# pratyushkumar211/industrial_nnmpc_2021

Hardware: AMD Instinct MI355X
Metric: condensed-QP solves/sec (CDU offline datagen) (higher is better)
Workload: dtype f64; 1 GPU; cdu_offline_data: synthetic CDU-size plant (n=4480 vars, m=8960 box rows, n_aug=284), 100000 sampled x0 per GPU per step, whole sequences u* written out; batch_per_gpu=100000, total_batch=100000, method=auto, parallelism=dp1 (sharded samples, 1 RCCL gather of the first moves pe...

## Files before the change

include/nnmpc.h:

```cpp
#ifndef NNMPC_H
#define NNMPC_H
#include <stdint.h>
#ifdef __cplusplus
extern "C" {
#endif

#define NNMPC_OK 0
#define NNMPC_EINVAL (-1)
#define NNMPC_EHIP (-2)
#define NNMPC_ENOMEM (-3)
#define NNMPC_ENOTIMPL (-4)

#define NNMPC_HOST 0
#define NNMPC_DEVICE 1

#define NNMPC_ST_OPTIMAL 0
#define NNMPC_ST_MAXITER 1
#define NNMPC_ST_NUMERIC 2

typedef struct nnmpc_qp nnmpc_qp;
typedef struct nnmpc_nn nnmpc_nn;

typedef struct {
  int32_t max_batch;
  int32_t nb;
  int32_t max_ipm_iters;
  int32_t max_polish_rounds;
  int32_t max_refine;
  int32_t max_rounds;
  int32_t sub_steps;
  int32_t stale_max_changes;
  int32_t stale_cg_limit;
  int32_t method;
  int32_t asm_max_active;
  int32_t asm_max_rounds;
  int32_t asm_f32_rounds;
  int32_t seg_max;
  int32_t asm_tail_batch;
  int32_t asm_predict_iters;
  float ipm_tol;
  double refine_tol;
  double bound_tol;
} nnmpc_qp_opts;

typedef struct {
  int64_t problems;
  int64_t rounds;
  int64_t factorizations;
  int64_t ipm_iterations;
  int64_t panel_launches;
  double panel_ms;
  double diag_ms;
  double trsv_ms;
  double total_ms;
  double panel_flops;
  int64_t trsv_solves;
  int64_t asm_solved;
  int64_t asm_rounds;
  int64_t asm_gemm_launches;
  double asm_gemm_ms;
  double asm_gemm_flops;
  double asm_lambda_ms;
  double asm_update_ms;
  double asm_lambda_flops;
  double asm_lambda_bytes;
  double asm_e1max;
  double asm_e2max;
  int64_t asm_full_checks;
  double asm_lambda32_ms;
  double asm_lambda64_ms;
  double asm_lambda32_flops;
  int64_t asm_lambda32_launches, asm_lambda64_launches;
  int64_t asm_far_passes;
  double asm_side_ms;
  int64_t asm_small_passes;
  int64_t asm_predict_launches;
  double asm_predict_ms;
  double asm_predict_flops;
} nnmpc_qp_stats;

const char* nnmpc_last_error(void);

int nnmpc_qp_create(nnmpc_qp** out, int32_t n, int32_t nu, int32_t n_aug, const double* P,
                    const double* tq, const double* Kunc, const nnmpc_qp_opts* opts);
int nnmpc_qp_destroy(nnmpc_qp* h);

int nnmpc_qp_solve_batch(nnmpc_qp* h, int32_t B, const double* x0, const double* lb,
                         const double* ub, double* u, uint32_t* active, int32_t* status,
                         int32_t* iters, int32_t ptr_kind);

int nnmpc_qp_solve_batch_warm(nnmpc_qp* h, int32_t B, const double* x0, const double* lb,
                              const double* ub, const uint8_t* guess, double* u, uint32_t* active,
                              int32_t* status, int32_t* iters, int32_t ptr_kind);

#define NNMPC_OUT_SEQUENCE 0
#define NNMPC_OUT_FIRST_MOVE 1
int nnmpc_qp_solve_batch_ex(nnmpc_qp* h, int32_t B, const double* x0, const double* lb,
                            const double* ub, const uint8_t* guess, double* u, uint32_t* active,
                            int32_t* status, int32_t* iters, int32_t ptr_kind, int32_t out_kind);

int nnmpc_qp_set_inverse(nnmpc_qp* h, const double* Hinv, const double* Kunc);

int nnmpc_qp_set_farfield(nnmpc_qp* h, int32_t W, int32_t r, const double* U, const double* Vx, const double* Vl);
int nnmpc_qp_farfield_missing(nnmpc_qp* h, int32_t* W);

int nnmpc_qp_first_moves(const double* u, int64_t ldu, const double* us, int32_t B, int32_t nu, double* out);
int nnmpc_qp_dims(nnmpc_qp* h, int32_t* n, int32_t* nu, int32_t* n_aug);
int nnmpc_qp_set_profiling(nnmpc_qp* h, int32_t on);
int nnmpc_qp_get_stats(nnmpc_qp* h, nnmpc_qp_stats* out, int32_t reset);

int nnmpc_qp_debug_factor_solve(nnmpc_qp* h, int32_t B, const float* dvec, const float* mask,
                                const float* rhs, float* sol);

int nnmpc_nn_create(nnmpc_nn** out, int32_t nlayers, const int32_t* dims,
                    const double* const* W, const double* const* b, int32_t nx, int32_t nu,
                    int32_t with_uprev, const double* xscale, const double* ulb,
                    const double* uub, int32_t use_bf16, int32_t max_batch);
int nnmpc_nn_destroy(nnmpc_nn* h);
int nnmpc_nn_forward(nnmpc_nn* h, int32_t B, const double* x, const double* uprev,
                     const double* xs, const double* us, double* u, int32_t ptr_kind);
int nnmpc_nn_last_ms(nnmpc_nn* h, double* gemm_ms, double* total_ms);
int nnmpc_nn_last_hidden_ms(nnmpc_nn* h, double* hidden_ms, int32_t* launches);

typedef struct nnmpc_chain nnmpc_chain;
int nnmpc_chain_create(nnmpc_chain** out, nnmpc_qp* qp, int32_t nc, int32_t nx, int32_t nu, int32_t nd,
                       const double* A, const double* B, const double* Bd, const double* ulb,
                       const double* uub, const double* x0, const double* uprev0);
int nnmpc_chain_destroy(nnmpc_chain* c);
int nnmpc_chain_run(nnmpc_chain* c, int32_t T, const double* xs, const double* us, const double* d,
                    double* x_rec, double* uprev_rec, double* u_rec, int32_t* status,
                    int32_t warm_start, int32_t ptr_kind);
int nnmpc_chain_reset(nnmpc_chain* c);
int nnmpc_chain_last_ms(nnmpc_chain* c, double* total_ms, double* solve_ms);

typedef struct nnmpc_ts nnmpc_ts;
int nnmpc_ts_create(nnmpc_ts** out, int32_t nu, int32_t nz, const double* Pr, const double* E,
                    const double* lb, const double* ub);
int nnmpc_ts_destroy(nnmpc_ts* h);
int nnmpc_ts_solve_batch(nnmpc_ts* h, int32_t B, const double* q, const double* e, double* us,
                         double* lam_eq, uint8_t* active, int32_t* status, int32_t ptr_kind);

typedef struct nnmpc_cl nnmpc_cl;
#define NNMPC_CL_MPC 0
#define NNMPC_CL_NN 1
#define NNMPC_CL_SATDLQR 2
#define NNMPC_CL_US 3
typedef struct {
  int32_t nx, nu, ny, nd, nz;
  const double *A, *B, *C, *Bp;
  const double *Aaug, *Baug, *Caug, *L;
  const double *tb, *Qb, *Qy, *q0, *Cd, *Eb, *Xb, *Xu;
  const double *Qaug, *Raug, *Maug;
  const double *ulb, *uub, *x0, *xhat0, *uprev0;
} nnmpc_cl_model;
typedef struct {
  int32_t kind;
  nnmpc_qp* qp;
  int32_t nlayers;
  const int32_t* dims;
  const double* const* W;
  const double* const* b;
  int32_t with_uprev;
  const double* xscale;
  const double* Kaug;
} nnmpc_cl_slot;
int nnmpc_cl_create(nnmpc_cl** out, const nnmpc_cl_model* m, nnmpc_ts* ts, int32_t nslots, const nnmpc_cl_slot* slots,
                    int32_t nb, const int32_t* inst_slot);
int nnmpc_cl_destroy(nnmpc_cl* h);
int nnmpc_cl_run(nnmpc_cl* h, int32_t T, int32_t nscen, const double* setpoints, const double* dist, const int32_t* scen,
                 const double* v, const double* sigma, const double* y0, double* y_rec, double* x_rec, double* xhat_rec, double* u_rec,
                 double* xs_rec, double* us_rec, double* avg_rec, int32_t* ts_status, int32_t* reg_status, int32_t ptr_kind);
int nnmpc_cl_reset(nnmpc_cl* h);
int nnmpc_cl_last_ms(nnmpc_cl* h, double* total_ms, double* phase_ms, double* slot_step_ms);
#define NNMPC_CL_PLANT_LINEAR 0
#define NNMPC_CL_PLANT_CSTRS_FLASH 1
#define NNMPC_CSTRS_NPAR 51
int nnmpc_cl_set_plant(nnmpc_cl* h, int32_t kind, const double* par, int32_t npar, double sample_time, int32_t substeps);
int nnmpc_cl_last_plant_ms(nnmpc_cl* h, double* plant_ms);
int nnmpc_cstrs_flow(int32_t nb, const double* par, int32_t npar, double sample_time, int32_t substeps, const double* x,
                     const double* u, const double* p, double* x_out, int32_t ptr_kind);

int nnmpc_device_count(void);
int nnmpc_set_device(int32_t dev);
int nnmpc_device_synchronize(void);
int nnmpc_dev_mem_info(uint64_t* free_bytes, uint64_t* total_bytes);
int nnmpc_dev_malloc(void** out, uint64_t bytes);
int nnmpc_dev_free(void* p);
int nnmpc_dev_memset(void* p, int32_t value, uint64_t bytes);
int nnmpc_memcpy_h2d(void* dst, const void* src, uint64_t bytes);
int nnmpc_memcpy_d2h(void* dst, const void* src, uint64_t bytes);
int nnmpc_memcpy_d2d(void* dst, const void* src, uint64_t bytes);
int nnmpc_host_alloc_pinned(void** out, uint64_t bytes);
int nnmpc_host_free_pinned(void* p);

typedef struct nnmpc_comm nnmpc_comm;
int nnmpc_comm_unique_id(void* id128);
int nnmpc_comm_init(nnmpc_comm** out, const void* id128, int32_t rank, int32_t world);
int nnmpc_comm_destroy(nnmpc_comm* c);
int nnmpc_comm_rank(nnmpc_comm* c);
int nnmpc_comm_world(nnmpc_comm* c);
int nnmpc_comm_gather_rows(nnmpc_comm* c, const double* send, const int64_t* rows, int32_t row_doubles,
                           double* recv, int32_t root);
int nnmpc_comm_allreduce_max(nnmpc_comm* c, double* value);
int nnmpc_comm_barrier(nnmpc_comm* c);

#ifdef __cplusplus
}
#endif
#endif
```

industrial_nnmpc_2021_amd/_lib.py:

```python
import ctypes as C
import os

_HERE = os.path.dirname(os.path.abspath(__file__))
LIB_PATH = os.path.join(_HERE, "libnnmpc_hip.so")

HOST, DEVICE = 0, 1
ST_OPTIMAL, ST_MAXITER, ST_NUMERIC = 0, 1, 2
OUT_SEQUENCE, OUT_FIRST_MOVE = 0, 1
EINVAL, EHIP, ENOMEM, ENOTIMPL = -1, -2, -3, -4


class QpOpts(C.Structure):
    _fields_ = [("max_batch", C.c_int32), ("nb", C.c_int32), ("max_ipm_iters", C.c_int32),
                ("max_polish_rounds", C.c_int32), ("max_refine", C.c_int32),
                ("max_rounds", C.c_int32), ("sub_steps", C.c_int32), ("stale_max_changes", C.c_int32),
                ("stale_cg_limit", C.c_int32), ("method", C.c_int32), ("asm_max_active", C.c_int32),
                ("asm_max_rounds", C.c_int32), ("asm_f32_rounds", C.c_int32), ("seg_max", C.c_int32), ("asm_tail_batch", C.c_int32), ("asm_predict_iters", C.c_int32), ("ipm_tol", C.c_float), ("refine_tol", C.c_double),
                ("bound_tol", C.c_double)]


class QpStats(C.Structure):
    _fields_ = [("problems", C.c_int64), ("rounds", C.c_int64), ("factorizations", C.c_int64),
                ("ipm_iterations", C.c_int64), ("panel_launches", C.c_int64),
                ("panel_ms", C.c_double), ("diag_ms", C.c_double), ("trsv_ms", C.c_double),
                ("total_ms", C.c_double), ("panel_flops", C.c_double), ("trsv_solves", C.c_int64), ("asm_solved", C.c_int64),
                ("asm_rounds", C.c_int64), ("asm_gemm_launches", C.c_int64), ("asm_gemm_ms", C.c_double),
                ("asm_gemm_flops", C.c_double), ("asm_lambda_ms", C.c_double), ("asm_update_ms", C.c_double), ("asm_lambda_flops", C.c_double),
                ("asm_lambda_bytes", C.c_double), ("asm_e1max", C.c_double),
                ("asm_e2max", C.c_double), ("asm_full_checks", C.c_int64), ("asm_lambda32_ms", C.c_double),
                ("asm_lambda64_ms", C.c_double), ("asm_lambda32_flops", C.c_double),
                ("asm_lambda32_launches", C.c_int64), ("asm_lambda64_launches", C.c_int64), ("asm_far_passes", C.c_int64), ("asm_side_ms", C.c_double),
                ("asm_small_passes", C.c_int64), ("asm_predict_launches", C.c_int64), ("asm_predict_ms", C.c_double),
                ("asm_predict_flops", C.c_double)]


CL_MPC, CL_NN, CL_SATDLQR, CL_US = 0, 1, 2, 3
CL_PLANT_LINEAR, CL_PLANT_CSTRS_FLASH, CSTRS_NPAR = 0, 1, 51


class ClModel(C.Structure):
    _fields_ = [(k, C.c_int32) for k in ("nx", "nu", "ny", "nd", "nz")] + \
               [(k, C.c_void_p) for k in ("A", "B", "C", "Bp", "Aaug", "Baug", "Caug", "L", "tb", "Qb", "Qy", "q0", "Cd",
                                          "Eb", "Xb", "Xu", "Qaug", "Raug", "Maug", "ulb", "uub", "x0", "xhat0", "uprev0")]


class ClSlot(C.Structure):
    _fields_ = [("kind", C.c_int32), ("qp", C.c_void_p), ("nlayers", C.c_int32), ("dims", C.c_void_p), ("W", C.c_void_p),
                ("b", C.c_void_p), ("with_uprev", C.c_int32), ("xscale", C.c_void_p), ("Kaug", C.c_void_p)]


EXPORTS = ["nnmpc_last_error", "nnmpc_qp_create", "nnmpc_qp_destroy", "nnmpc_qp_solve_batch",
           "nnmpc_qp_solve_batch_warm", "nnmpc_qp_solve_batch_ex", "nnmpc_qp_set_inverse", "nnmpc_qp_dims",
           "nnmpc_qp_first_moves", "nnmpc_qp_set_farfield", "nnmpc_qp_farfield_missing",
           "nnmpc_qp_set_profiling", "nnmpc_qp_get_stats", "nnmpc_qp_debug_factor_solve",
           "nnmpc_nn_create", "nnmpc_nn_destroy", "nnmpc_nn_forward", "nnmpc_nn_last_ms", "nnmpc_nn_last_hidden_ms",
           "nnmpc_chain_create", "nnmpc_chain_destroy", "nnmpc_chain_run", "nnmpc_chain_reset", "nnmpc_chain_last_ms",
           "nnmpc_ts_create", "nnmpc_ts_destroy", "nnmpc_ts_solve_batch",
           "nnmpc_cl_create", "nnmpc_cl_destroy", "nnmpc_cl_run", "nnmpc_cl_reset", "nnmpc_cl_last_ms",
           "nnmpc_cl_set_plant", "nnmpc_cl_last_plant_ms", "nnmpc_cstrs_flow",
           "nnmpc_device_count", "nnmpc_set_device", "nnmpc_device_synchronize", "nnmpc_dev_mem_info",
           "nnmpc_dev_malloc", "nnmpc_dev_free", "nnmpc_dev_memset", "nnmpc_memcpy_h2d", "nnmpc_memcpy_d2h",
           "nnmpc_memcpy_d2d", "nnmpc_host_alloc_pinned", "nnmpc_host_free_pinned",
           "nnmpc_comm_unique_id", "nnmpc_comm_init", "nnmpc_comm_destroy", "nnmpc_comm_rank", "nnmpc_comm_world",
           "nnmpc_comm_gather_rows", "nnmpc_comm_allreduce_max", "nnmpc_comm_barrier"]

_lib = None


class NnmpcError(RuntimeError):
    pass


def load():
    global _lib
    if _lib is not None:
        return _lib
    if not os.path.exists(LIB_PATH):
        raise NnmpcError(
            f"{LIB_PATH} not found: build it with `python -c 'import __graft_entry__ as g; g.build()'` "
            "(hipcc --offload-arch=gfx950).  There is no CPU fallback.")
    lib = C.CDLL(LIB_PATH)
    vp, i32, dp = C.c_void_p, C.c_int32, C.c_void_p
    lib.nnmpc_last_error.restype = C.c_char_p
    lib.nnmpc_last_error.argtypes = []
    lib.nnmpc_qp_create.restype = i32
    lib.nnmpc_qp_create.argtypes = [C.POINTER(vp), i32, i32, i32, dp, dp, dp, C.POINTER(QpOpts)]
    lib.nnmpc_qp_destroy.restype = i32
    lib.nnmpc_qp_destroy.argtypes = [vp]
    lib.nnmpc_qp_solve_batch.restype = i32
    lib.nnmpc_qp_solve_batch.argtypes = [vp, i32, dp, dp, dp, dp, dp, dp, dp, i32]
    lib.nnmpc_qp_solve_batch_warm.restype = i32
    lib.nnmpc_qp_solve_batch_warm.argtypes = [vp, i32, dp, dp, dp, dp, dp, dp, dp, dp, i32]
    lib.nnmpc_qp_set_inverse.restype = i32
    lib.nnmpc_qp_set_inverse.argtypes = [vp, dp, dp]
    lib.nnmpc_qp_set_farfield.restype = i32
    lib.nnmpc_qp_set_farfield.argtypes = [vp, i32, i32, dp, dp, dp]
    lib.nnmpc_qp_farfield_missing.restype = i32
    lib.nnmpc_qp_farfield_missing.argtypes = [vp, C.POINTER(i32)]
    lib.nnmpc_qp_set_profiling.restype = i32
    lib.nnmpc_qp_set_profiling.argtypes = [vp, i32]
    lib.nnmpc_qp_get_stats.restype = i32
    lib.nnmpc_qp_get_stats.argtypes = [vp, C.POINTER(QpStats), i32]
    lib.nnmpc_qp_debug_factor_solve.restype = i32
    lib.nnmpc_qp_debug_factor_solve.argtypes = [vp, i32, dp, dp, dp, dp]
    lib.nnmpc_nn_create.restype = i32
    lib.nnmpc_nn_create.argtypes = [C.POINTER(vp), i32, C.POINTER(i32), C.POINTER(dp), C.POINTER(dp),
                                    i32, i32, i32, dp, dp, dp, i32, i32]
    lib.nnmpc_nn_destroy.restype = i32
    lib.nnmpc_nn_destroy.argtypes = [vp]
    lib.nnmpc_nn_forward.restype = i32
    lib.nnmpc_nn_forward.argtypes = [vp, i32, dp, dp, dp, dp, dp, i32]
    lib.nnmpc_nn_last_ms.restype = i32
    lib.nnmpc_nn_last_ms.argtypes = [vp, C.POINTER(C.c_double), C.POINTER(C.c_double)]
    lib.nnmpc_nn_last_hidden_ms.restype = i32
    lib.nnmpc_nn_last_hidden_ms.argtypes = [vp, C.POINTER(C.c_double), C.POINTER(C.c_int32)]
    u64 = C.c_uint64
    lib.nnmpc_qp_solve_batch_ex.restype = i32
    lib.nnmpc_qp_solve_batch_ex.argtypes = [vp, i32, dp, dp, dp, dp, dp, dp, dp, dp, i32, i32]
    lib.nnmpc_qp_first_moves.restype = i32
    lib.nnmpc_qp_first_moves.argtypes = [dp, C.c_int64, dp, i32, i32, dp]
    lib.nnmpc_qp_dims.restype = i32
    lib.nnmpc_qp_dims.argtypes = [vp, C.POINTER(i32), C.POINTER(i32), C.POINTER(i32)]
    lib.nnmpc_chain_create.restype = i32
    lib.nnmpc_chain_create.argtypes = [C.POINTER(vp), vp, i32, i32, i32, i32, dp, dp, dp, dp, dp, dp, dp]
    lib.nnmpc_chain_destroy.restype = i32
    lib.nnmpc_chain_destroy.argtypes = [vp]
    lib.nnmpc_chain_run.restype = i32
    lib.nnmpc_chain_run.argtypes = [vp, i32, dp, dp, dp, dp, dp, dp, dp, i32, i32]
    lib.nnmpc_chain_reset.restype = i32
    lib.nnmpc_chain_reset.argtypes = [vp]
    lib.nnmpc_chain_last_ms.restype = i32
    lib.nnmpc_chain_last_ms.argtypes = [vp, C.POINTER(C.c_double), C.POINTER(C.c_double)]
    lib.nnmpc_ts_create.restype = i32
    lib.nnmpc_ts_create.argtypes = [C.POINTER(vp), i32, i32, dp, dp, dp, dp]
    lib.nnmpc_ts_destroy.restype = i32
    lib.nnmpc_ts_destroy.argtypes = [vp]
    lib.nnmpc_ts_solve_batch.restype = i32
    lib.nnmpc_ts_solve_batch.argtypes = [vp, i32, dp, dp, dp, dp, dp, dp, i32]
    lib.nnmpc_cl_create.restype = i32
    lib.nnmpc_cl_create.argtypes = [C.POINTER(vp), C.POINTER(ClModel), vp, i32, C.POINTER(ClSlot), i32, C.POINTER(i32)]
    lib.nnmpc_cl_destroy.restype = i32
    lib.nnmpc_cl_destroy.argtypes = [vp]
    lib.nnmpc_cl_run.restype = i32
    lib.nnmpc_cl_run.argtypes = [vp, i32, i32, dp, dp, dp, dp, dp, dp] + [dp] * 9 + [i32]
    lib.nnmpc_cl_reset.restype = i32
    lib.nnmpc_cl_reset.argtypes = [vp]
    lib.nnmpc_cl_last_ms.restype = i32
    lib.nnmpc_cl_last_ms.argtypes = [vp, C.POINTER(C.c_double), dp, dp]
    lib.nnmpc_cl_set_plant.restype = i32
    lib.nnmpc_cl_set_plant.argtypes = [vp, i32, dp, i32, C.c_double, i32]
    lib.nnmpc_cl_last_plant_ms.restype = i32
    lib.nnmpc_cl_last_plant_ms.argtypes = [vp, C.POINTER(C.c_double)]
    lib.nnmpc_cstrs_flow.restype = i32
    lib.nnmpc_cstrs_flow.argtypes = [i32, dp, i32, C.c_double, i32, dp, dp, dp, dp, i32]
    lib.nnmpc_device_count.restype = i32
    lib.nnmpc_device_count.argtypes = []
    lib.nnmpc_set_device.restype = i32
    lib.nnmpc_set_device.argtypes = [i32]
    lib.nnmpc_device_synchronize.restype = i32
    lib.nnmpc_device_synchronize.argtypes = []
    lib.nnmpc_dev_mem_info.restype = i32
    lib.nnmpc_dev_mem_info.argtypes = [C.POINTER(u64), C.POINTER(u64)]
    lib.nnmpc_dev_malloc.restype = i32
    lib.nnmpc_dev_malloc.argtypes = [C.POINTER(vp), u64]
    lib.nnmpc_dev_free.restype = i32
    lib.nnmpc_dev_free.argtypes = [vp]
    lib.nnmpc_dev_memset.restype = i32
    lib.nnmpc_dev_memset.argtypes = [vp, i32, u64]
    for name in ("nnmpc_memcpy_h2d", "nnmpc_memcpy_d2h", "nnmpc_memcpy_d2d"):
        getattr(lib, name).restype = i32
        getattr(lib, name).argtypes = [vp, vp, u64]
    lib.nnmpc_host_alloc_pinned.restype = i32
    lib.nnmpc_host_alloc_pinned.argtypes = [C.POINTER(vp), u64]
    lib.nnmpc_host_free_pinned.restype = i32
    lib.nnmpc_host_free_pinned.argtypes = [vp]
    lib.nnmpc_comm_unique_id.restype = i32
    lib.nnmpc_comm_unique_id.argtypes = [vp]
    lib.nnmpc_comm_init.restype = i32
    lib.nnmpc_comm_init.argtypes = [C.POINTER(vp), vp, i32, i32]
    lib.nnmpc_comm_destroy.restype = i32
    lib.nnmpc_comm_destroy.argtypes = [vp]
    lib.nnmpc_comm_rank.restype = i32
    lib.nnmpc_comm_rank.argtypes = [vp]
    lib.nnmpc_comm_world.restype = i32
    lib.nnmpc_comm_world.argtypes = [vp]
    lib.nnmpc_comm_gather_rows.restype = i32
    lib.nnmpc_comm_gather_rows.argtypes = [vp, dp, C.POINTER(C.c_int64), i32, dp, i32]
    lib.nnmpc_comm_allreduce_max.restype = i32
    lib.nnmpc_comm_allreduce_max.argtypes = [vp, C.POINTER(C.c_double)]
    lib.nnmpc_comm_barrier.restype = i32
    lib.nnmpc_comm_barrier.argtypes = [vp]
    _lib = lib
    return lib


def check(rc, what):
    if rc != 0:
        msg = load().nnmpc_last_error().decode(errors="replace")
        raise NnmpcError(f"{what} failed (code {rc}): {msg}")


class DeviceArray:

    def __init__(self, shape, dtype):
        import numpy as np
        self.shape = tuple(int(v) for v in (shape if hasattr(shape, "__len__") else (shape,)))
        self.dtype = np.dtype(dtype)
        self.nbytes = int(np.prod(self.shape, dtype=np.int64)) * self.dtype.itemsize
        self._p = C.c_void_p()
        check(load().nnmpc_dev_malloc(C.byref(self._p), self.nbytes), "nnmpc_dev_malloc")

    @classmethod
    def from_host(cls, a):
        import numpy as np
        a = np.ascontiguousarray(a)
        d = cls(a.shape, a.dtype)
        d.upload(a)
        return d

    def data_ptr(self):
        return self._p.value or 0

    def upload(self, a):
        import numpy as np
        a = np.ascontiguousarray(a, dtype=self.dtype)
        if a.nbytes != self.nbytes:
            raise ValueError("upload: size mismatch")
        check(load().nnmpc_memcpy_h2d(self._p, a.ctypes.data_as(C.c_void_p), self.nbytes), "nnmpc_memcpy_h2d")

    def to_host(self, rows=None):
        import numpy as np
        shape = self.shape if rows is None else (int(rows),) + self.shape[1:]
        out = np.empty(shape, self.dtype)
        check(load().nnmpc_memcpy_d2h(out.ctypes.data_as(C.c_void_p), self._p, out.nbytes), "nnmpc_memcpy_d2h")
        return out

    def row_ptr(self, row):
        import numpy as np
        stride = int(np.prod(self.shape[1:], dtype=np.int64)) * self.dtype.itemsize
        return C.c_void_p((self._p.value or 0) + int(row) * stride)

    def free(self):
        if getattr(self, "_p", None) is not None and self._p.value:
            load().nnmpc_dev_free(self._p)
            self._p = C.c_void_p()

    __del__ = free


def set_device(dev):
    check(load().nnmpc_set_device(int(dev)), "nnmpc_set_device")


def synchronize():
    check(load().nnmpc_device_synchronize(), "nnmpc_device_synchronize")


def device_count():
    return int(load().nnmpc_device_count())
```

industrial_nnmpc_2021_amd/csrc/qp_solver.hip:

```cpp
#include <hip/hip_runtime.h>
#include <stdint.h>
#include <stdio.h>
#include <stdarg.h>
#include <string.h>
#include <vector>
#include <algorithm>
#include <cmath>
#include <cstdlib>
#include "../../include/nnmpc.h"
#define ASM_WG_TU (-1)
#include "chol_kernels.h"
#include "gemm_kernels.h"
#include "qp_asm.h"
#include "qp_wide.h"
#include "qp_small.h"
#include "qp_predict.h"
#include "common.h"
static constexpr int ASM_SMALL9_LDS_MAX = 100 * 1024;

using namespace nnmpc;

namespace {

enum { PH_INIT = 0, PH_IPM = 1, PH_POLISH = 2, PH_DONE = 3 };
enum { PS_START = 0, PS_CG = 1, PS_CHECK = 2 };
enum { CNT_ACTIVE = 0, CNT_FACTOR = 1, CNT_IPM = 2, CNT_POLISH = 3, CNT_SOLVE = 4 };

constexpr int POLISH_GRACE = 10;
struct QpDev {
  int n, np, nu, slots;
  int max_ipm, max_polish, max_refine, stale_max_changes, stale_cg_limit;
  float ipm_tol, delta;
  double refine_tol, bound_tol, stat_tol, pscale;
  const float* pdiag;
  float *u, *zu, *zl, *lbv, *ubv, *q, *PU, *rd, *rhs, *sol, *dua, *dvec, *mask, *uunc;
  double *x, *q64, *PX, *r64, *p64, *v64;
  unsigned char* st;
  double *lb64, *ub64;
  const double *q64_all, *lb_all, *ub_all;
  const float* uunc_all;
  const unsigned char* guess_all;
  int *slot_prob, *age, *next_prob;
  int seg_count, max_rounds;
  int *phase, *f_factor, *f_solve, *istep, *ipm_it, *nfac, *prounds, *rcnt, *psub, *fail, *stale;
  int *pninf, *pgrace;
  int* ptie;
  float *mu, *gap, *smu, *qscale;
  double* rz;
  int* counters;
  double* u_out;
  int ldu, nout;
  uint32_t* act_out;
  int* status_out;
  int* iters_out;
  int words;
};

__device__ __forceinline__ float wave_max(float v) {
  for (int o = 32; o > 0; o >>= 1) v = fmaxf(v, __shfl_xor(v, o));
  return v;
}
__device__ __forceinline__ float wave_sum(float v) {
  for (int o = 32; o > 0; o >>= 1) v += __shfl_xor(v, o);
  return v;
}
__device__ __forceinline__ double wave_maxd(double v) {
  for (int o = 32; o > 0; o >>= 1) v = fmax(v, __shfl_xor(v, o));
  return v;
}
__device__ float block_max(float v, float* sh) {
  v = wave_max(v);
  __syncthreads();
  if ((threadIdx.x & 63) == 0) sh[threadIdx.x >> 6] = v;
  __syncthreads();
  return fmaxf(fmaxf(sh[0], sh[1]), fmaxf(sh[2], sh[3]));
}
__device__ float block_sum(float v, float* sh) {
  v = wave_sum(v);
  __syncthreads();
  if ((threadIdx.x & 63) == 0) sh[threadIdx.x >> 6] = v;
  __syncthreads();
  return (sh[0] + sh[1]) + (sh[2] + sh[3]);
}
__device__ double block_maxd(double v, double* sh) {
  v = wave_maxd(v);
  __syncthreads();
  if ((threadIdx.x & 63) == 0) sh[threadIdx.x >> 6] = v;
  __syncthreads();
  return fmax(fmax(sh[0], sh[1]), fmax(sh[2], sh[3]));
}
__device__ double block_sumd(double v, double* sh) {
  for (int o = 32; o > 0; o >>= 1) v += __shfl_xor(v, o);
  __syncthreads();
  if ((threadIdx.x & 63) == 0) sh[threadIdx.x >> 6] = v;
  __syncthreads();
  return (sh[0] + sh[1]) + (sh[2] + sh[3]);
}
__device__ int block_sum_i(int v, int* sh) {
  for (int o = 32; o > 0; o >>= 1) v += __shfl_xor(v, o);
  __syncthreads();
  if ((threadIdx.x & 63) == 0) sh[threadIdx.x >> 6] = v;
  __syncthreads();
  return sh[0] + sh[1] + sh[2] + sh[3];
}

#define SLACK_MIN 1e-12f

__device__ void write_outputs(const QpDev& d, int p, int status);

__global__ __launch_bounds__(256) void refill_k(QpDev d) {
  __shared__ float shf[4];
  __shared__ int s_idx;
  const int p = blockIdx.x, tid = threadIdx.x;
  const size_t o = (size_t)p * d.np;
  if (d.phase[p] != PH_DONE) return;
  if (tid == 0) s_idx = atomicAdd(d.next_prob, 1);
  __syncthreads();
  const int idx = s_idx;
  if (idx >= d.seg_count) {
    if (tid == 0) d.slot_prob[p] = -1;
    return;
  }
  const size_t oi = (size_t)idx * d.np;
  if (tid < d.nu) {
    d.lb64[(size_t)p * d.nu + tid] = d.lb_all[(size_t)idx * d.nu + tid];
    d.ub64[(size_t)p * d.nu + tid] = d.ub_all[(size_t)idx * d.nu + tid];
  }
  float qm = 0.f;
  int invalid = 0;
  for (int r = tid; r < d.np; r += 256) {
    if (r < d.n) {
      const int c = r % d.nu;
      invalid |= !(fabs(d.q64_all[oi + r]) <= 1.79e308);
      const float lb = (float)d.lb_all[(size_t)idx * d.nu + c], ub = (float)d.ub_all[(size_t)idx * d.nu + c];
      const double q64 = d.q64_all[oi + r];
      const float q = (float)(q64 / d.pscale);
      const float w = ub - lb;
      float u0 = d.uunc_all[oi + r];
      u0 = fminf(fmaxf(u0, lb + 0.05f * w), ub - 0.05f * w);
      d.lbv[o + r] = lb; d.ubv[o + r] = ub; d.q[o + r] = q; d.u[o + r] = u0; d.q64[o + r] = q64;
      qm = fmaxf(qm, fabsf(q));
    } else {
      d.lbv[o + r] = -1.f; d.ubv[o + r] = 1.f; d.q[o + r] = 0.f; d.u[o + r] = 0.f; d.q64[o + r] = 0.0;
    }
    d.zu[o + r] = 0.f; d.zl[o + r] = 0.f;
    d.mask[o + r] = 1.f; d.dvec[o + r] = 0.f; d.rhs[o + r] = 0.f; d.sol[o + r] = 0.f;
    d.dua[o + r] = 0.f; d.rd[o + r] = 0.f; d.x[o + r] = 0.0; d.st[o + r] = 0;
    d.r64[o + r] = 0.0; d.p64[o + r] = 0.0; d.v64[o + r] = 0.0;
  }
  qm = block_max(qm, shf);
  {
    invalid |= !(qm <= 3.0e38f);
    if (tid < d.nu) invalid |= !(d.lb_all[(size_t)idx * d.nu + tid] <= d.ub_all[(size_t)idx * d.nu + tid]);
    invalid = __syncthreads_or(invalid);
    if (invalid) {
      const double qnan = __longlong_as_double(0x7ff8000000000000ll);
      for (int r = tid; r < d.np; r += 256) d.x[o + r] = qnan;
      if (tid == 0) { d.slot_prob[p] = idx; d.fail[p] = 1; d.ipm_it[p] = d.nfac[p] = 0; }
      __syncthreads();
      write_outputs(d, p, NNMPC_ST_NUMERIC);
      return;
    }
  }
  const bool warm = d.guess_all != nullptr && d.guess_all[(size_t)idx * d.n] != 255;
  if (warm) {
    for (int r = tid; r < d.n; r += 256) {
      const int c = r % d.nu;
      int s = d.guess_all[(size_t)idx * d.n + r];
      if (s > 2) s = 0;
      const double xv = s == 1 ? d.ub_all[(size_t)idx * d.nu + c]
                      : s == 2 ? d.lb_all[(size_t)idx * d.nu + c] : (double)d.u[o + r];
      d.st[o + r] = (unsigned char)s;
      d.x[o + r] = xv;
      d.v64[o + r] = xv;
    }
  }
  if (tid == 0) {
    d.slot_prob[p] = idx;
    d.age[p] = 0;
    d.qscale[p] = fmaxf(1.f, qm);
    d.phase[p] = warm ? PH_POLISH : PH_INIT;
    d.f_factor[p] = d.f_solve[p] = 0;
    d.ipm_it[p] = d.nfac[p] = d.prounds[p] = d.rcnt[p] = d.psub[p] = d.fail[p] = d.stale[p] = 0;
    d.pninf[p] = 0x7fffffff; d.pgrace[p] = POLISH_GRACE; d.ptie[p] = 0;
    d.mu[p] = d.gap[p] = d.smu[p] = 0.f; d.rz[p] = 0.0;
  }
}
__global__ void reset_slots_k(QpDev d) {
  const int p = blockIdx.x * blockDim.x + threadIdx.x;
  if (p < d.slots) {
    d.phase[p] = PH_DONE; d.slot_prob[p] = -1; d.age[p] = 0;
    d.f_factor[p] = d.f_solve[p] = 0;
  }
  if (p == 0) *d.next_prob = 0;
}

__device__ void write_outputs(const QpDev& d, int p, int status) {
  const int tid = threadIdx.x;
  const size_t o = (size_t)p * d.np;
  const size_t pi = (size_t)d.slot_prob[p];
  for (int r = tid; r < d.nout; r += 256) d.u_out[pi * d.ldu + r] = d.x[o + r];
  const int m = 2 * d.n;
  for (int w = tid; w < d.words; w += 256) {
    uint32_t bits = 0;
    for (int b = 0; b < 32; ++b) {
      const int idx = 32 * w + b;
      if (idx < m) {
        const int k = idx / (2 * d.nu), c = idx % (2 * d.nu);
        const int hit = (c < d.nu) ? (d.st[o + k * d.nu + c] == 1) : (d.st[o + k * d.nu + c - d.nu] == 2);
        bits |= (uint32_t)hit << b;
      }
    }
    if (d.act_out) d.act_out[pi * d.words + w] = bits;
  }
  if (tid == 0) {
    if (d.status_out) d.status_out[pi] = d.fail[p] ? NNMPC_ST_NUMERIC : status;
    if (d.iters_out) { d.iters_out[2 * pi] = d.ipm_it[p]; d.iters_out[2 * pi + 1] = d.nfac[p]; }
  }
}

__device__ int cg_alpha(const QpDev& d, int p, double* shd) {
  const int tid = threadIdx.x;
  const size_t o = (size_t)p * d.np;
  double pap = 0.0;
  for (int r = tid; r < d.n; r += 256)
    if (d.st[o + r] == 0) pap += d.p64[o + r] * d.PX[o + r];
  pap = block_sumd(pap, shd);
  const double rz = d.rz[p];
  const bool ok = (pap > 0.0) && (rz > 0.0);
  const double a = ok ? rz / pap : 0.0;
  double pm = 0.0, xm = 0.0;
  for (int r = tid; r < d.n; r += 256) {
    if (d.st[o + r] == 0) {
      const double pv = d.p64[o + r];
      const double x = d.x[o + r] + a * pv;
      d.x[o + r] = x;
      d.r64[o + r] -= a * d.PX[o + r];
      pm = fmax(pm, fabs(pv));
      xm = fmax(xm, fabs(x));
    } else {
      xm = fmax(xm, fabs(d.x[o + r]));
    }
  }
  pm = block_maxd(pm, shd);
  xm = block_maxd(xm, shd);
  const int rc = d.rcnt[p] + 1;
  const bool nan = !(a == a) || !(xm == xm);
  const bool conv = !ok || nan || (fabs(a) * pm <= d.refine_tol * fmax(1.0, xm)) || rc >= d.max_refine;
  if (conv) {
    for (int r = tid; r < d.n; r += 256) d.v64[o + r] = d.x[o + r];
  } else {
    for (int r = tid; r < d.n; r += 256) d.rhs[o + r] = d.st[o + r] ? 0.f : (float)d.r64[o + r];
  }
  const bool refac = !conv && d.stale[p] && rc >= d.stale_cg_limit;
  if (refac) for (int r = tid; r < d.n; r += 256) d.v64[o + r] = d.x[o + r];
  __syncthreads();
  if (tid == 0) {
    d.rcnt[p] = refac ? 0 : rc;
    if (nan) d.fail[p] = 1;
    if (conv) d.psub[p] = PS_CHECK;
    if (refac) { d.psub[p] = PS_START; d.stale[p] = 0; }
  }
  return (conv || refac) ? 0 : 1;
}
__device__ void cg_beta(const QpDev& d, int p, double* shd) {
  const int tid = threadIdx.x;
  const size_t o = (size_t)p * d.np;
  double rzn = 0.0;
  for (int r = tid; r < d.n; r += 256)
    if (d.st[o + r] == 0) rzn += d.r64[o + r] * (double)d.sol[o + r];
  rzn = block_sumd(rzn, shd);
  const bool first = d.psub[p] == PS_START;
  const double rz = d.rz[p];
  const double beta = (first || !(rz > 0.0)) ? 0.0 : rzn / rz;
  for (int r = tid; r < d.n; r += 256) {
    double pv = 0.0;
    if (d.st[o + r] == 0) pv = (double)d.sol[o + r] + beta * d.p64[o + r];
    d.p64[o + r] = pv;
    d.v64[o + r] = pv;
  }
  __syncthreads();
  if (tid == 0) { d.rz[p] = rzn; d.psub[p] = PS_CG; }
}

__device__ int kkt_check(const QpDev& d, int p, int* shi, double* shd) {
  const int tid = threadIdx.x, n = d.n;
  const size_t o = (size_t)p * d.np;
  int bad = 0;
  double gfree = 0.0;
  for (int r = tid; r < n; r += 256) {
    const int c = r % d.nu;
    const double g = d.PX[o + r] + d.q64[o + r], x = d.x[o + r];
    const double lb = d.lb64[(size_t)p * d.nu + c], ub = d.ub64[(size_t)p * d.nu + c];
    const int s = d.st[o + r];
    if (s == 0) { bad += !(x <= ub + d.bound_tol) || !(x >= lb - d.bound_tol) || !(fabs(g) <= 1.79e308); gfree = fmax(gfree, fabs(g)); }
    else if (s == 1) bad += !(g < 0.0);
    else bad += !(g > 0.0);
  }
  bad = block_sum_i(bad, shi);
  gfree = block_maxd(gfree, shd);
  const int pr = d.prounds[p] + 1;
  if (bad == 0 && pr <= d.max_polish && !d.ptie[p]) {
    int ties = 0;
    for (int r = tid; r < n; r += 256) {
      if (d.st[o + r] != 0) continue;
      const int c = r % d.nu;
      const double x = d.x[o + r];
      const double lb = d.lb64[(size_t)p * d.nu + c], ub = d.ub64[(size_t)p * d.nu + c];
      if (x > ub) { d.st[o + r] = 1; d.x[o + r] = ub; ++ties; }
      else if (x < lb) { d.st[o + r] = 2; d.x[o + r] = lb; ++ties; }
    }
    ties = block_sum_i(ties, shi);
    __syncthreads();
    if (tid == 0) d.ptie[p] = 1;
    if (ties > 0) {
      for (int r = tid; r < n; r += 256) d.v64[o + r] = d.x[o + r];
      if (tid == 0) {
        d.stale[p] = ties <= d.stale_max_changes;
        d.prounds[p] = pr; d.psub[p] = PS_START; d.rcnt[p] = 0;
        d.f_factor[p] = d.f_solve[p] = 0;
      }
      return 0;
    }
  }
  if (bad == 0 || pr > d.max_polish) {
    const double gs = d.pscale * (double)d.qscale[p];
    const int ok = bad == 0 && gfree <= d.stat_tol * gs;
    write_outputs(d, p, ok ? NNMPC_ST_OPTIMAL : NNMPC_ST_MAXITER);
    if (tid == 0) { d.phase[p] = PH_DONE; d.f_factor[p] = d.f_solve[p] = 0; }
    return 1;
  }
  int single = 0, rsel = -1;
  {
    const int best = d.pninf[p], grace = d.pgrace[p];
    __syncthreads();
    if (bad < best) { if (tid == 0) { d.pninf[p] = bad; d.pgrace[p] = POLISH_GRACE; } }
    else if (grace > 0) { if (tid == 0) d.pgrace[p] = grace - 1; }
    else single = 1;
  }
  if (single) {
    double rm = -1e300;
    for (int r = tid; r < n; r += 256) {
      const int c = r % d.nu;
      const double g = d.PX[o + r] + d.q64[o + r], x = d.x[o + r];
      const double lb = d.lb64[(size_t)p * d.nu + c], ub = d.ub64[(size_t)p * d.nu + c];
      const int s = d.st[o + r];
      const bool inf = s == 0 ? ((x > ub + d.bound_tol) || (x < lb - d.bound_tol)) : (s == 1 ? g >= 0.0 : g <= 0.0);
      if (inf && -(double)r > rm) rm = -(double)r;
    }
    rm = block_maxd(rm, shd);
    rsel = rm > -1e299 ? (int)(-rm) : -1;
  }
  for (int r = tid; r < n; r += 256) {
    const int c = r % d.nu;
    const double g = d.PX[o + r] + d.q64[o + r], x = d.x[o + r];
    const double lb = d.lb64[(size_t)p * d.nu + c], ub = d.ub64[(size_t)p * d.nu + c];
    const int s = d.st[o + r];
    double xn = x;
    if (single && r != rsel) { d.v64[o + r] = xn; continue; }
    if (s == 0) {
      if (x > ub + d.bound_tol) { d.st[o + r] = 1; xn = ub; }
      else if (x < lb - d.bound_tol) { d.st[o + r] = 2; xn = lb; }
    } else if ((s == 1 && g >= 0.0) || (s == 2 && g <= 0.0)) {
      d.st[o + r] = 0;
    }
    d.x[o + r] = xn;
    d.v64[o + r] = xn;
  }
  if (tid == 0) {
    d.stale[p] = bad <= d.stale_max_changes;
    d.prounds[p] = pr; d.psub[p] = PS_START; d.rcnt[p] = 0;
    d.f_factor[p] = d.f_solve[p] = 0;
  }
  return 0;
}

__global__ __launch_bounds__(256) void stage_pre_k(QpDev d) {
  __shared__ float shf[4];
  __shared__ int shi[4];
  __shared__ double shd[4];
  const int p = blockIdx.x, tid = threadIdx.x;
  const size_t o = (size_t)p * d.np;
  int ph = d.phase[p];
  if (ph == PH_DONE) return;
  const int n = d.n;
  {
    const int age = d.age[p] + 1;
    __syncthreads();
    if (tid == 0) d.age[p] = age;
    if (age > d.max_rounds) {
      if (ph != PH_POLISH) {
        for (int r = tid; r < n; r += 256) { d.x[o + r] = (double)d.u[o + r]; d.st[o + r] = 0; }
        __syncthreads();
      }
      write_outputs(d, p, NNMPC_ST_MAXITER);
      if (tid == 0) { d.phase[p] = PH_DONE; d.f_factor[p] = d.f_solve[p] = 0; }
      return;
    }
  }

  if (ph == PH_INIT) {
    float s = 0.f;
    for (int r = tid; r < n; r += 256) s += fabsf(d.PU[o + r] + d.q[o + r]);
    s = block_sum(s, shf);
    const float mu0 = 0.1f * s / n + 1e-3f;
    for (int r = tid; r < n; r += 256) {
      const float g = d.PU[o + r] + d.q[o + r];
      const float u = d.u[o + r];
      const float su = fmaxf(d.ubv[o + r] - u, SLACK_MIN), sl = fmaxf(u - d.lbv[o + r], SLACK_MIN);
      d.zu[o + r] = fmaxf(-g, 0.f) + mu0 / su;
      d.zl[o + r] = fmaxf(g, 0.f) + mu0 / sl;
    }
    ph = PH_IPM;
  }

  if (ph == PH_IPM) {
    float rdm = 0.f, gs = 0.f;
    for (int r = tid; r < n; r += 256) {
      const float g = d.PU[o + r] + d.q[o + r];
      const float u = d.u[o + r], zu = d.zu[o + r], zl = d.zl[o + r];
      const float su = fmaxf(d.ubv[o + r] - u, SLACK_MIN), sl = fmaxf(u - d.lbv[o + r], SLACK_MIN);
      const float rdv = g + zu - zl;
      d.rd[o + r] = rdv;
      rdm = fmaxf(rdm, fabsf(rdv));
      gs += su * zu + sl * zl;
    }
    rdm = block_max(rdm, shf);
    gs = block_sum(gs, shf);
    const float mu = gs / (2.f * n);
    const int it = d.ipm_it[p];
    const bool nan = !(rdm == rdm) || !(gs == gs);
    const bool conv = (rdm <= d.ipm_tol * d.qscale[p] && mu <= d.ipm_tol * d.qscale[p]) || it >= d.max_ipm || nan;
    if (!conv) {
      for (int r = tid; r < n; r += 256) {
        const float u = d.u[o + r], zu = d.zu[o + r], zl = d.zl[o + r];
        const float su = fmaxf(d.ubv[o + r] - u, SLACK_MIN), sl = fmaxf(u - d.lbv[o + r], SLACK_MIN);
        d.dvec[o + r] = zu / su + zl / sl + d.delta;
        d.mask[o + r] = 1.f;
        d.rhs[o + r] = -(d.PU[o + r] + d.q[o + r]);
      }
      if (tid == 0) {
        d.phase[p] = PH_IPM;
        d.gap[p] = gs; d.mu[p] = mu;
        d.ipm_it[p] = it + 1; d.nfac[p] += 1;
        d.f_factor[p] = 1; d.f_solve[p] = 1; d.istep[p] = 0;
        atomicAdd(&d.counters[CNT_ACTIVE], 1); atomicAdd(&d.counters[CNT_FACTOR], 1);
        atomicAdd(&d.counters[CNT_IPM], 1); atomicAdd(&d.counters[CNT_SOLVE], 1);
      }
      return;
    }
    for (int r = tid; r < n; r += 256) {
      const float u = d.u[o + r], zu = d.zu[o + r], zl = d.zl[o + r];
      const float su = fmaxf(d.ubv[o + r] - u, SLACK_MIN), sl = fmaxf(u - d.lbv[o + r], SLACK_MIN);
      const int c = r % d.nu;
      int s = 0;
      if (!nan) {
        const float pd = d.pdiag[r];
        const bool au = zu > pd * su, al = zl > pd * sl;
        if (au && al) s = (zu * sl > zl * su) ? 1 : 2; else if (au) s = 1; else if (al) s = 2;
      }
      d.st[o + r] = (unsigned char)s;
      const double xv = s == 1 ? d.ub64[(size_t)p * d.nu + c]
                      : s == 2 ? d.lb64[(size_t)p * d.nu + c]
                               : (nan ? 0.0 : (double)u);
      d.x[o + r] = xv;
      d.v64[o + r] = xv;
    }
    if (tid == 0) {
      if (nan) d.fail[p] = 1;
      d.phase[p] = PH_POLISH; d.psub[p] = PS_START; d.rcnt[p] = 0; d.prounds[p] = 0;
      d.f_factor[p] = d.f_solve[p] = 0;
      atomicAdd(&d.counters[CNT_ACTIVE], 1); atomicAdd(&d.counters[CNT_POLISH], 1);
    }
    return;
  }

  int sub = d.psub[p];
  if (sub == PS_CHECK) {
    if (kkt_check(d, p, shi, shd)) return;
    if (tid == 0) { atomicAdd(&d.counters[CNT_ACTIVE], 1); atomicAdd(&d.counters[CNT_POLISH], 1); }
    return;
  }
  if (sub == PS_START) {
    const int keep = d.stale[p];
    for (int r = tid; r < n; r += 256) {
      const int s = d.st[o + r];
      const double rr = s ? 0.0 : -(d.PX[o + r] + d.q64[o + r]);
      d.r64[o + r] = rr;
      d.rhs[o + r] = (float)rr;
      if (!keep) { d.mask[o + r] = s ? 0.f : 1.f; d.dvec[o + r] = s ? 1.f : d.delta; }
    }
    if (tid == 0) {
      d.f_factor[p] = !keep; d.f_solve[p] = 1;
      if (!keep) { d.nfac[p] += 1; atomicAdd(&d.counters[CNT_FACTOR], 1); }
      atomicAdd(&d.counters[CNT_ACTIVE], 1); atomicAdd(&d.counters[CNT_POLISH], 1);
      atomicAdd(&d.counters[CNT_SOLVE], 1);
    }
    return;
  }
  if (tid == 0) {
    d.f_factor[p] = 0; d.f_solve[p] = 1;
    atomicAdd(&d.counters[CNT_ACTIVE], 1); atomicAdd(&d.counters[CNT_POLISH], 1);
    atomicAdd(&d.counters[CNT_SOLVE], 1);
  }
}

__global__ __launch_bounds__(256) void stage_sub_a_k(QpDev d) {
  __shared__ float shf[4];
  __shared__ double shd[4];
  const int p = blockIdx.x, tid = threadIdx.x;
  const size_t o = (size_t)p * d.np;
  if (!d.f_solve[p]) return;
  const int ph = d.phase[p], n = d.n;
  if (ph == PH_POLISH) { cg_beta(d, p, shd); return; }
  if (ph != PH_IPM) return;
  if (d.istep[p] == 0) {
  float t = 0.f;
  for (int r = tid; r < n; r += 256) {
    const float du = d.sol[o + r], u = d.u[o + r], zu = d.zu[o + r], zl = d.zl[o + r];
    const float su = fmaxf(d.ubv[o + r] - u, SLACK_MIN), sl = fmaxf(u - d.lbv[o + r], SLACK_MIN);
    const float dzu = -zu + zu * du / su, dzl = -zl - zl * du / sl;
    t = fmaxf(t, fmaxf(fmaxf(du / su, -du / sl), fmaxf(-dzu / zu, -dzl / zl)));
  }
  t = block_max(t, shf);
  const float a = t > 0.f ? fminf(1.f, 1.f / t) : 1.f;
  float ga = 0.f;
  for (int r = tid; r < n; r += 256) {
    const float du = d.sol[o + r], u = d.u[o + r], zu = d.zu[o + r], zl = d.zl[o + r];
    const float su = fmaxf(d.ubv[o + r] - u, SLACK_MIN), sl = fmaxf(u - d.lbv[o + r], SLACK_MIN);
    const float dzu = -zu + zu * du / su, dzl = -zl - zl * du / sl;
    ga += (su - a * du) * (zu + a * dzu) + (sl + a * du) * (zl + a * dzl);
  }
  ga = block_sum(ga, shf);
  float sg = ga / d.gap[p];
  sg = fminf(1.f, fmaxf(0.f, sg));
  const float smu = sg * sg * sg * d.mu[p];
  for (int r = tid; r < n; r += 256) {
    const float du = d.sol[o + r], u = d.u[o + r], zu = d.zu[o + r], zl = d.zl[o + r];
    const float su = fmaxf(d.ubv[o + r] - u, SLACK_MIN), sl = fmaxf(u - d.lbv[o + r], SLACK_MIN);
    const float dzu = -zu + zu * du / su, dzl = -zl - zl * du / sl;
    d.rhs[o + r] = -d.rd[o + r] + zu - smu / su - du * dzu / su - zl + smu / sl - du * dzl / sl;
    d.dua[o + r] = du;
  }
  if (tid == 0) { d.smu[p] = smu; d.istep[p] = 1; }
    return;
  }
  const float smu = d.smu[p];
  float t = 0.f;
  for (int r = tid; r < n; r += 256) {
    const float du = d.sol[o + r], da = d.dua[o + r], u = d.u[o + r], zu = d.zu[o + r], zl = d.zl[o + r];
    const float su = fmaxf(d.ubv[o + r] - u, SLACK_MIN), sl = fmaxf(u - d.lbv[o + r], SLACK_MIN);
    const float dzua = -zu + zu * da / su, dzla = -zl - zl * da / sl;
    const float rcu = -su * zu + smu + da * dzua, rcl = -sl * zl + smu - da * dzla;
    const float dzu = (rcu + zu * du) / su, dzl = (rcl - zl * du) / sl;
    t = fmaxf(t, fmaxf(fmaxf(du / su, -du / sl), fmaxf(-dzu / zu, -dzl / zl)));
  }
  t = block_max(t, shf);
  const float a = t > 0.f ? fminf(1.f, 0.99f / t) : 1.f;
  for (int r = tid; r < n; r += 256) {
    const float du = d.sol[o + r], da = d.dua[o + r], u = d.u[o + r], zu = d.zu[o + r], zl = d.zl[o + r];
    const float su = fmaxf(d.ubv[o + r] - u, SLACK_MIN), sl = fmaxf(u - d.lbv[o + r], SLACK_MIN);
    const float dzua = -zu + zu * da / su, dzla = -zl - zl * da / sl;
    const float rcu = -su * zu + smu + da * dzua, rcl = -sl * zl + smu - da * dzla;
    const float dzu = (rcu + zu * du) / su, dzl = (rcl - zl * du) / sl;
    d.u[o + r] = u + a * du;
    d.zu[o + r] = fmaxf(zu + a * dzu, 1e-30f);
    d.zl[o + r] = fmaxf(zl + a * dzl, 1e-30f);
  }
  if (tid == 0) d.f_solve[p] = 0;
}

__global__ __launch_bounds__(256) void stage_sub_b_k(QpDev d) {
  __shared__ int shi[4];
  __shared__ double shd[4];
  const int p = blockIdx.x, tid = threadIdx.x;
  if (d.phase[p] != PH_POLISH) return;
  const int sub = d.psub[p];
  if (sub == PS_CG && d.f_solve[p]) {
    const int go = cg_alpha(d, p, shd);
    if (tid == 0) d.f_solve[p] = go;
  } else if (sub == PS_CHECK) {
    kkt_check(d, p, shi, shd);
  }
}

__global__ void f64_to_f32_k(float* dst, const double* src, size_t count) {
  size_t i = (size_t)blockIdx.x * blockDim.x + threadIdx.x;
  const size_t stride = (size_t)gridDim.x * blockDim.x;
  for (; i < count; i += stride) dst[i] = (float)src[i];
}
__global__ void pad_x0_k(double* d64, float* d32, const double* src, int nprob, int n_aug, int ka,
                         int rows) {
  size_t i = (size_t)blockIdx.x * blockDim.x + threadIdx.x;
  const size_t total = (size_t)rows * ka;
  const size_t stride = (size_t)gridDim.x * blockDim.x;
  for (; i < total; i += stride) {
    const int p = (int)(i / ka), k = (int)(i % ka);
    const double v = (p < nprob && k < n_aug) ? src[(size_t)p * n_aug + k] : 0.0;
    d64[i] = v;
    d32[i] = (float)v;
  }
}

}

struct nnmpc_qp {
  int device;
  int n, np, nu, n_aug, ka, NB, T, tiles, slots, words;
  nnmpc_qp_opts opts;
  bool have_kunc;
  float* Pt;
  float* P32;
  double* P64;
  double* tq64;
  float* Kunc32;
  float* pdiag;
  double pscale;
  float* L;
  float* Y;
  float* Dacc;
  unsigned long long* trsv_count;
  QpDev d;
  bool have_inverse;
  double* H64;
  double* Kunc64;
  double *asm_xunc, *asm_x, *asm_lam, *asm_xh, *asm_scratch, *asm_xhw;
  int *asm_rowprob, *asm_wflag;
  unsigned char* asm_wmark;
  unsigned char* asm_st;
  int *asm_state, *asm_rounds, *asm_counters, *asm_biglist, *asm_status, *asm_binlist, *asm_idxg, *asm_mg, *asm_row, *asm_lrank, *asm_ctot;
  unsigned char *asm_prec, *asm_redo, *asm_alpha, *asm_rowk;
  float *asm_lam32, *asm_xh32, *H32;
  int *asm_ninf, *asm_hi, *asm_kblk;
  double tqmax;
  int asm_pool;
  double asm_e1max, asm_e2max;
  struct Far { int W, r, rp; double *U, *Vx, *Vl, *cu; int* kt; double ksum; double efar; };
  std::vector<Far> far;
  std::vector<int> far_missing;
  double p_inf = 0.0;
  double *asm_tnorm = nullptr, *asm_tslack = nullptr;
  struct PredWin { pu32x4* Hf = nullptr; double L = 0.0; int W = 0; };
  PredWin pred[2];
  int* pred_cnt = nullptr;
  double* asm_work;
  int seg_max;
  double* x0_64;
  float* x0_32;
  double* q64_all;
  float* uunc_all;
  double *lb_d, *ub_d;
  double* in_stage;
  hipStream_t stream;
  hipStream_t stream2 = nullptr;
  hipStream_t stream3 = nullptr, stream4 = nullptr;
  int asm_tail_budget = 50000;
  hipEvent_t ev_fork = nullptr, ev_join = nullptr, ev_join3 = nullptr, ev_join4 = nullptr;
  int* pin_cnt = nullptr;
  int* pin_st = nullptr;
  bool profiling;
  bool gemm_error = false;
  std::vector<hipEvent_t> ev_pool;
  size_t ev_used;
  struct EvRec { int kind; size_t e0, e1; double flops; };
  std::vector<EvRec> ev_recs;
  nnmpc_qp_stats stats;
  std::vector<void*> allocs;
  struct Scratch { void* p = nullptr; size_t cap = 0; };
  enum { SC_U = 0, SC_ACT, SC_ST, SC_IT, SC_GUESS, SC_FB_GUESS, SC_FB_LIST, SC_FB_X0, SC_FB_LB, SC_FB_UB, SC_FB_U, SC_FB_ACT, SC_FB_ST, SC_FB_IT, SC_COUNT };
  Scratch sc[SC_COUNT];
  int ldu, nout;
};

namespace {

template <class T>
int dev_alloc(nnmpc_qp* h, T** p, size_t count) {
  void* q = nullptr;
  hipError_t e = hipMalloc(&q, count * sizeof(T));
  if (e != hipSuccess) { set_error("hipMalloc(%zu bytes): %s", count * sizeof(T), hipGetErrorString(e)); return NNMPC_ENOMEM; }
  e = hipMemset(q, 0, count * sizeof(T));
  if (e != hipSuccess) { set_error("hipMemset: %s", hipGetErrorString(e)); return NNMPC_EHIP; }
  h->allocs.push_back(q);
  *p = (T*)q;
  return 0;
}

template <class T>
int scratch_get(nnmpc_qp* h, int which, T** out, size_t bytes) {
  nnmpc_qp::Scratch& s = h->sc[which];
  if (s.cap < bytes) {
    if (s.p) { hipFree(s.p); s.p = nullptr; s.cap = 0; }
    const size_t want = bytes + bytes / 4 + 256;
    const hipError_t e = hipMalloc(&s.p, want);
    if (e != hipSuccess) { s.p = nullptr; set_error("hipMalloc(%zu bytes of scratch): %s", want, hipGetErrorString(e)); return NNMPC_ENOMEM; }
    s.cap = want;
  }
  *out = (T*)s.p;
  return 0;
}

size_t ev_get(nnmpc_qp* h) {
  if (h->ev_used == h->ev_pool.size()) {
    hipEvent_t e;
    hipEventCreate(&e);
    h->ev_pool.push_back(e);
  }
  return h->ev_used++;
}
struct EvScope {
  nnmpc_qp* h; int kind; double flops; size_t e0; hipStream_t st;
  EvScope(nnmpc_qp* h_, int kind_, double flops_, hipStream_t st_ = nullptr) : h(h_), kind(kind_), flops(flops_), e0(0), st(st_ ? st_ : h_->stream) {
    if (h->profiling) { e0 = ev_get(h); hipEventRecord(h->ev_pool[e0], st); }
  }
  ~EvScope() {
    if (h->profiling) {
      size_t e1 = ev_get(h);
      hipEventRecord(h->ev_pool[e1], st);
      h->ev_recs.push_back({kind, e0, e1, flops});
    }
  }
};
void ev_collect(nnmpc_qp* h) {
  for (auto& r : h->ev_recs) {
    float ms = 0.f;
    hipEventElapsedTime(&ms, h->ev_pool[r.e0], h->ev_pool[r.e1]);
    if (r.kind == 0) { h->stats.panel_ms += ms; h->stats.panel_launches += 1; h->stats.panel_flops += r.flops; }
    else if (r.kind == 1) h->stats.diag_ms += ms;
    else if (r.kind == 2) h->stats.trsv_ms += ms;
    else if (r.kind == 3) h->stats.total_ms += ms;
    else if (r.kind == 4) h->stats.asm_lambda_ms += ms;
    else if (r.kind == 5) { h->stats.asm_gemm_ms += ms; h->stats.asm_gemm_flops += r.flops; h->stats.asm_gemm_launches += 1; }
    else if (r.kind == 6) h->stats.asm_update_ms += ms;
    else if (r.kind == 7) { h->stats.asm_lambda32_ms += ms; h->stats.asm_lambda32_launches += 1; }
    else if (r.kind == 8) { h->stats.asm_lambda64_ms += ms; h->stats.asm_lambda64_launches += 1; }
    else if (r.kind == 9) h->stats.asm_side_ms += ms;
    else if (r.kind == 10) { h->stats.asm_predict_ms += ms; h->stats.asm_predict_flops += r.flops; }
  }
  h->ev_recs.clear();
  h->ev_used = 0;
}

template <int NB>
void launch_gemm32(hipStream_t s, float* C, size_t ldc, const float* A, size_t lda, const float* B,
                   size_t ldb, int M, int N, int K) {
  dim3 grid(N / NB, M / NB);
  hipLaunchKernelGGL((gemm_nt_f32_k<NB, false, false>), grid, dim3(256), TileCfg<NB>::LDS_FLOATS * 4, s,
                     C, ldc, A, lda, B, ldb, K, (const float*)nullptr);
}
void gemm32(nnmpc_qp* h, float* C, size_t ldc, const float* A, size_t lda, const float* B, size_t ldb,
            int M, int N, int K) {
  if (N % 128 == 0 && M % 128 == 0) launch_gemm32<128>(h->stream, C, ldc, A, lda, B, ldb, M, N, K);
  else launch_gemm32<64>(h->stream, C, ldc, A, lda, B, ldb, M, N, K);
}
void gemm64(nnmpc_qp* h, double* C, size_t ldc, const double* A, size_t lda, const double* B,
            size_t ldb, int M, int N, int K, const int* rowphase = nullptr, int want = 0,
            const int* kdyn = nullptr, const int* mdyn = nullptr, bool kblocks = false, const int* rowmap = nullptr) {
  static const bool small64 = getenv("NNMPC_NO_SMALL_GEMM") == nullptr;
  const bool few = small64 && !rowmap && (M / 128) * (N / 128) < 200;
  if (M % 128 == 0 && N % 128 == 0 && K % G64_KC == 0 && !few) {
    const int ntm = M / 128, ntn = N / 128;
    hipLaunchKernelGGL(gemm_nt_f64_t128_k, dim3(g64_grid(ntm, ntn)), dim3(256), G64_LDS, h->stream, C, ldc, A, lda, B, ldb, K, ntm, ntn,
                       rowphase, want, kdyn, kblocks ? 2 : 0, mdyn, rowmap);
    return;
  }
  if (rowmap) {
    set_error("gemm64: rowmap with a shape off the 128 x 128 / K %% 16 grid (M = %d, N = %d, K = %d)", M, N, K);
    h->gemm_error = true;
    return;
  }
  dim3 grid(N / 64, M / 64);
  hipLaunchKernelGGL(gemm_nt_f64_k, grid, dim3(256), 0, h->stream, C, ldc, A, lda, B, ldb, K, rowphase, want, kdyn, mdyn, kblocks ? 1 : 0);
}

template <int NB>
int set_lds_attrs() {
  hipError_t e;
  e = hipFuncSetAttribute((const void*)chol_diag_k<NB>, hipFuncAttributeMaxDynamicSharedMemorySize, chol_diag_lds_bytes<NB>());
  if (e != hipSuccess) return -1;
  e = hipFuncSetAttribute((const void*)chol_panel_k<NB>, hipFuncAttributeMaxDynamicSharedMemorySize, chol_panel_lds_bytes<NB>());
  if (e != hipSuccess) return -1;
  e = hipFuncSetAttribute((const void*)trsv_k<NB>, hipFuncAttributeMaxDynamicSharedMemorySize, 96 * 1024);
  if (e != hipSuccess) return -1;
  e = hipFuncSetAttribute((const void*)gemm_nt_f32_k<NB, false, false>, hipFuncAttributeMaxDynamicSharedMemorySize, TileCfg<NB>::LDS_FLOATS * 4);
  if (e != hipSuccess) return -1;
  return 0;
}

template <int NB>
void factor_all(nnmpc_qp* h, int nslots, int nfactor) {
  CholArgs a;
  a.n = h->n; a.np = h->np; a.T = h->T; a.tiles = h->tiles;
  a.Pt = h->Pt; a.L = h->L; a.Y = h->Y; a.Dacc = h->Dacc; a.dvec = h->d.dvec; a.mask = h->d.mask;
  a.flag = h->d.f_factor; a.fail = h->d.fail;
  const double nb = NB;
  for (int j = 0; j < h->T; ++j) {
    {
      EvScope es(h, 1, 0.0);
      hipLaunchKernelGGL((chol_diag_k<NB>), dim3(nslots), dim3(256), chol_diag_lds_bytes<NB>(), h->stream, a, j);
    }
    const int below = h->T - 1 - j;
    if (below > 0) {
      const double fl = (double)nfactor * below * (2.0 * nb * nb * (j * nb) + nb * nb * nb + nb * nb * nb);
      EvScope es(h, 0, fl);
      hipLaunchKernelGGL((chol_panel_k<NB>), dim3(below, nslots), dim3(256), chol_panel_lds_bytes<NB>(), h->stream, a, j);
    }
  }
}
template <int NB>
void solve_all(nnmpc_qp* h, int nslots, const int* flag) {
  TrsvArgs a;
  a.n = h->n; a.np = h->np; a.T = h->T; a.tiles = h->tiles;
  a.L = h->L; a.Y = h->Y; a.rhs = h->d.rhs; a.sol = h->d.sol; a.flag = flag; a.count = h->trsv_count;
  EvScope es(h, 2, 0.0);
  hipLaunchKernelGGL((trsv_k<NB>), dim3(nslots), dim3(256), (h->np + 5 * NB) * 4, h->stream, a);
}
void factor_dispatch(nnmpc_qp* h, int nslots, int nfactor) {
  if (h->NB == 128) factor_all<128>(h, nslots, nfactor); else factor_all<64>(h, nslots, nfactor);
}
void solve_dispatch(nnmpc_qp* h, int nslots, const int* flag) {
  if (h->NB == 128) solve_all<128>(h, nslots, flag); else solve_all<64>(h, nslots, flag);
}

#define HIPCHK(x) do { hipError_t e_ = (x); if (e_ != hipSuccess) { set_error("%s: %s", #x, hipGetErrorString(e_)); return NNMPC_EHIP; } } while (0)

int solve_segment(nnmpc_qp* h, int nprob, const double* x0_dev, const double* lb_dev, const double* ub_dev,
                  const unsigned char* guess_dev, double* u_dev, uint32_t* act_dev, int32_t* st_dev, int32_t* it_dev) {
  QpDev& d = h->d;
  hipStream_t s = h->stream;
  const int rows = h->slots;
  const int segp = ((nprob + 127) / 128) * 128;
  hipLaunchKernelGGL(pad_x0_k, dim3(512), dim3(256), 0, s, h->x0_64, h->x0_32, x0_dev, nprob, h->n_aug, h->ka, segp);
  gemm64(h, h->q64_all, h->np, h->x0_64, h->ka, h->tq64, h->ka, segp, h->np, h->ka);
  if (h->have_kunc) gemm32(h, h->uunc_all, h->np, h->x0_32, h->ka, h->Kunc32, h->ka, segp, h->np, h->ka);
  else HIPCHK(hipMemsetAsync(h->uunc_all, 0, (size_t)segp * h->np * sizeof(float), s));
  d.q64_all = h->q64_all; d.uunc_all = h->uunc_all; d.lb_all = lb_dev; d.ub_all = ub_dev;
  d.seg_count = nprob;
  d.guess_all = guess_dev;
  d.u_out = u_dev; d.act_out = act_dev; d.status_out = st_dev; d.iters_out = it_dev;
  d.ldu = h->ldu; d.nout = h->nout;
  hipLaunchKernelGGL(reset_slots_k, dim3((rows + 255) / 256), dim3(256), 0, s, d);

  int cnt[8];
  bool any_ipm = true, any_polish = guess_dev != nullptr;
  int issued = 0;
  const int hard_cap = 1000000;
  for (int round = 0; round < hard_cap; ++round) {
    HIPCHK(hipMemsetAsync(d.counters, 0, 8 * sizeof(int), s));
    if (issued < nprob) {
      hipLaunchKernelGGL(refill_k, dim3(rows), dim3(256), 0, s, d);
      any_ipm = true;
      if (guess_dev) any_polish = true;
    }
    if (any_ipm) gemm32(h, d.PU, h->np, d.u, h->np, h->P32, h->np, rows, h->np, h->np);
    if (any_polish) gemm64(h, d.PX, h->np, d.v64, h->np, h->P64, h->np, rows, h->np, h->np, d.phase, PH_POLISH);
    hipLaunchKernelGGL(stage_pre_k, dim3(rows), dim3(256), 0, s, d);
    HIPCHK(hipMemcpyAsync(cnt, d.counters, 8 * sizeof(int), hipMemcpyDeviceToHost, s));
    HIPCHK(hipMemcpyAsync(&issued, d.next_prob, sizeof(int), hipMemcpyDeviceToHost, s));
    HIPCHK(stream_sync(s));
    if (cnt[CNT_ACTIVE] == 0 && issued >= nprob) break;
    any_ipm = cnt[CNT_IPM] > 0;
    any_polish = cnt[CNT_POLISH] > 0;
    h->stats.rounds += 1;
    h->stats.factorizations += cnt[CNT_FACTOR];
    h->stats.ipm_iterations += cnt[CNT_IPM];
    if (cnt[CNT_FACTOR] > 0) factor_dispatch(h, rows, cnt[CNT_FACTOR]);
    if (cnt[CNT_SOLVE] > 0) {
      const int nsub = cnt[CNT_POLISH] > 0 ? h->opts.sub_steps : 2;
      for (int k = 0; k < nsub; ++k) {
        solve_dispatch(h, rows, d.f_solve);
        hipLaunchKernelGGL(stage_sub_a_k, dim3(rows), dim3(256), 0, s, d);
        if (cnt[CNT_POLISH] > 0) {
          gemm64(h, d.PX, h->np, d.v64, h->np, h->P64, h->np, rows, h->np, h->np, d.phase, PH_POLISH);
          hipLaunchKernelGGL(stage_sub_b_k, dim3(rows), dim3(256), 0, s, d);
        }
      }
    }
  }
  HIPCHK(stream_sync(s));
  HIPCHK(hipGetLastError());
  h->stats.problems += nprob;
  return 0;
}


template <int NT>
int build_predictor(nnmpc_qp* h, const std::vector<double>& hh, int np, nnmpc_qp::PredWin& pw) {
  constexpr int W = PredCfg<NT>::W, KS = PredCfg<NT>::KS;
  pw.L = 0.0; pw.W = W;
  std::vector<double> dg(W);
  for (int j = 0; j < W; ++j) { dg[j] = hh[(size_t)j * np + j]; if (!(dg[j] > 0.0)) return 0; }
  std::vector<double> v(W, 1.0), u(W), isd(W);
  for (int j = 0; j < W; ++j) isd[j] = 1.0 / std::sqrt(dg[j]);
  double lam = 0.0;
  for (int itp = 0; itp < 200; ++itp) {
    double nv = 0.0;
    for (int i = 0; i < W; ++i) nv += v[i] * v[i];
    nv = std::sqrt(nv);
    for (int i = 0; i < W; ++i) v[i] *= isd[i] / nv;
    for (int i = 0; i < W; ++i) {
      double sacc = 0.0;
      const double* hr = &hh[(size_t)i * np];
      for (int j = 0; j < W; ++j) sacc += hr[j] * v[j];
      u[i] = sacc * isd[i];
    }
    double num = 0.0;
    for (int i = 0; i < W; ++i) num += u[i] * v[i] / isd[i];
    const bool conv = std::fabs(num - lam) <= 1e-6 * std::fabs(num);
    lam = num;
    v = u;
    if (conv && itp > 8) break;
  }
  if (!(lam > 0.0)) return 0;
  const double L = 1.05 * lam;
  std::vector<unsigned short> hf((size_t)W * W);
  auto bf = [](double x) { float f = (float)x; unsigned u32; memcpy(&u32, &f, 4); return (unsigned short)((u32 + 0x7fffu + ((u32 >> 16) & 1u)) >> 16); };
  for (int jt = 0; jt < W / 16; ++jt)
    for (int ks = 0; ks < KS; ++ks)
      for (int lane = 0; lane < 64; ++lane) {
        const int li = lane & 15, lq = lane >> 4;
        for (int e = 0; e < 8; ++e) {
          const int k = 32 * ks + 8 * lq + e;
          hf[pred_frag_index<NT>(jt, ks, lane) * 8 + e] = bf(hh[(size_t)(16 * jt + li) * np + k] / (L * dg[k]));
        }
      }
  if (!pw.Hf) { int rc = dev_alloc(h, (unsigned short**)&pw.Hf, hf.size()); if (rc) return rc; }
  HIPCHK(hipMemcpy(pw.Hf, hf.data(), hf.size() * 2, hipMemcpyHostToDevice));
  pw.L = L;
  return 0;
}

int solve_segment_asm(nnmpc_qp* h, int nprob, const double* x0_dev, const double* lb_dev, const double* ub_dev,
                      const unsigned char* guess_dev, double* u_dev, uint32_t* act_dev, int32_t* st_dev, int32_t* it_dev) {
  hipStream_t s = h->stream;
  const int segp = ((nprob + 127) / 128) * 128;
  hipLaunchKernelGGL(pad_x0_k, dim3(512), dim3(256), 0, s, h->x0_64, h->x0_32, x0_dev, nprob, h->n_aug, h->ka, segp);
  static const bool no_fuse = getenv("NNMPC_NO_FUSED_WIDE") != nullptr;
  static const bool no_lazy = getenv("NNMPC_NO_LAZY_XUNC") != nullptr;
  const bool tail_only = h->opts.asm_tail_batch >= 0 && nprob <= std::min(std::min(h->asm_pool, 256), h->opts.asm_tail_batch ? h->opts.asm_tail_batch : 256);
  const bool small = getenv("NNMPC_NO_SMALL") == nullptr && (size_t)h->np * h->np * 8 <= (4u << 20) && h->n <= ASM_SM_NMAX && h->np % 4 == 0;
  const bool lazy = h->np % 128 == 0 && !no_fuse && !no_lazy && !tail_only && !small && (uint64_t)h->seg_max * h->ka * 8 < (1ull << 32);
  const int winit = std::min(h->n, std::max(512, ((h->n / 8 + 127) / 128) * 128));
  int Wx = h->np;
  if (lazy) Wx = std::min(h->np, guess_dev ? 512 : ((winit + 127) / 128) * 128);

  {
    EvScope es(h, 5, 2.0 * Wx * (double)h->ka * nprob);
    gemm64(h, h->asm_xunc, h->np, h->x0_64, h->ka, h->Kunc64, h->ka, segp, Wx, h->ka);
  }
  AsmDev a;
  a.Kunc = h->Kunc64; a.Wx = Wx; a.winit = winit;
  a.ffU = a.ffVx = a.ffVl = a.ffcu = nullptr; a.ffk = nullptr; a.ffr = a.ffW = 0; a.T = h->asm_xhw; a.tnorm = h->asm_tnorm; a.tslack = h->asm_tslack;
  a.ff_skip = 0; a.ff_err = 0.0; a.ff_efar = 0.0;
  static const bool no_far = getenv("NNMPC_NO_FARFIELD") != nullptr;
  int wide_far_rp = 0, fft_prev = 0;
  double wide_far_ksum = 0.0;
  a.n = h->n; a.np = h->np; a.nu = h->nu; a.nseg = nprob;
  a.max_active = h->opts.asm_max_active; a.max_rounds = h->opts.asm_max_rounds;
  a.bound_tol = h->opts.bound_tol; a.stat_tol = 1e-8; a.pscale = h->pscale;
  a.e1max = h->asm_e1max; a.e2max = h->asm_e2max; a.x0 = h->x0_64; a.ka = h->ka;
  a.H = h->H64; a.lb = lb_dev; a.ub = ub_dev; a.xunc = h->asm_xunc; a.q64 = h->q64_all;
  a.x = h->asm_x; a.lam = h->asm_lam; a.xh = h->asm_xh; a.px = h->asm_xh;
  a.st = h->asm_st; a.guess = guess_dev; a.state = h->asm_state; a.rounds = h->asm_rounds; a.counters = h->asm_counters;
  a.biglist = h->asm_biglist; a.binlist = h->asm_binlist; a.idxg = h->asm_idxg; a.mg = h->asm_mg; a.row = h->asm_row; a.tqmax = h->tqmax; a.lrank = h->asm_lrank; a.ctot = h->asm_ctot; a.prec = h->asm_prec; a.redo = h->asm_redo; a.rowk = h->asm_rowk; a.lam32 = h->asm_lam32; a.H32 = h->H32; a.xh32 = h->asm_xh32; a.alpha = h->asm_alpha; a.ninf_best = h->asm_ninf; a.hi = h->asm_hi; a.kblk = h->asm_kblk; a.nkblk = 2 * (h->seg_max / 64 + 2); a.kref = 0; a.use_f32 = h->opts.asm_f32_rounds >= 0; a.xhw = h->asm_xhw; a.rowprob = h->asm_rowprob; a.wrows = 0; a.wmark = h->asm_wmark; a.wflag = h->asm_wflag; a.W = h->np; a.scratch = h->asm_scratch; a.work = h->asm_work;
  a.u_out = u_dev; a.ldu = h->ldu; a.nout = h->nout; a.act_out = act_dev; a.status_out = h->asm_status; a.iters_out = it_dev; a.words = h->words;
  a.nseg = nprob;
  { static const int tgi = getenv("NNMPC_TAIL_GI") ? 1 : 0; a.tail_gi = tgi; }
  { static const int wg = getenv("NNMPC_NO_WG") ? 0 : 1; a.use_wg = wg; }
  { static const int rfn = getenv("NNMPC_REFINE") ? atoi(getenv("NNMPC_REFINE")) : 1; a.refine = 0; a.refine_later = rfn && a.use_f32;
    static const double rtol = getenv("NNMPC_REFINE_TOL") ? atof(getenv("NNMPC_REFINE_TOL")) : ASM_REFINE_TOL; a.refine_tol = rtol; }
  { static const int e64 = getenv("NNMPC_EARLY64") ? atoi(getenv("NNMPC_EARLY64")) : 4; a.early64 = e64; }
  if (!guess_dev) HIPCHK(hipMemsetAsync(h->asm_st, 0, (size_t)nprob * h->n, s));
  a.pred_w = 0; a.pred_f64 = 0;
  double pred_flops_per_it = 0.0;
  {
    static const int env_it = getenv("NNMPC_PRED_ITERS") ? atoi(getenv("NNMPC_PRED_ITERS")) : -1;
    const int iters_req = env_it >= 0 ? (env_it == 0 ? -1 : std::min(env_it, (int)PRED_MAXIT)) : h->opts.asm_predict_iters;
    const int iters = iters_req == 0 ? (int)PRED_MAXIT : iters_req;
    if (iters > 0 && h->pred[0].L > 0.0 && !guess_dev && !small && !tail_only && Wx >= PRED_W) {
      PredArgs pa;
      { static const int f10 = getenv("NNMPC_PRED_FACTOR") ? atoi(getenv("NNMPC_PRED_FACTOR")) : 3; pa.fac10 = f10; }
      pa.iters = iters; pa.adaptive = iters_req == 0; pa.itsum = h->profiling ? h->pred_cnt + 1 : nullptr;
      if (h->profiling) HIPCHK(hipMemsetAsync(h->pred_cnt + 1, 0, 4, s));
      double t = 1.0;
      for (int k = 0; k < iters; ++k) { const double tn = 0.5 * (1.0 + std::sqrt(1.0 + 4.0 * t * t)); pa.beta[k] = (float)((t - 1.0) / tn); t = tn; }
      for (int k = iters; k < PRED_MAXIT; ++k) pa.beta[k] = 0.f;
      int wide = 0;
      static const int force_w = getenv("NNMPC_PRED_WIDE") ? atoi(getenv("NNMPC_PRED_WIDE")) : -1;
      if (h->pred[1].L > 0.0 && lazy) {
        if (force_w >= 0) wide = force_w;
        else {
          HIPCHK(hipMemsetAsync(h->pred_cnt, 0, 4, s));
          hipLaunchKernelGGL(asm_extent_k, dim3((nprob + 63) / 64), dim3(256), 0, s, a, PRED_W - PRED_W / 4, PRED_W, h->pred_cnt);
          HIPCHK(hipMemcpyAsync(h->pin_cnt, h->pred_cnt, 4, hipMemcpyDeviceToHost, s));
          HIPCHK(stream_sync(s));
          wide = h->pin_cnt[0] * 4 > nprob;
          h->pin_cnt[0] = 0;
        }
      }
      if (wide && Wx < PRED_W2) {
        EvScope es(h, 5, 2.0 * (PRED_W2 - Wx) * (double)h->ka * nprob);
        gemm64(h, h->asm_xunc + Wx, h->np, h->x0_64, h->ka, h->Kunc64 + (size_t)Wx * h->ka, h->ka, segp, PRED_W2 - Wx, h->ka);
        Wx = PRED_W2; a.Wx = Wx;
      }
      const bool nu4 = h->nu % 4 == 0;
      const int W = wide ? PRED_W2 : PRED_W, MR = (wide || !nu4) ? 32 : 64;
      pa.Hf = h->pred[wide].Hf;
      pred_flops_per_it = 2.0 * W * (double)W * MR;
      h->stats.asm_predict_launches += 1;
      EvScope es(h, 10, 0.0);
      if (wide) hipLaunchKernelGGL((asm_predict_k<8, 2>), dim3((nprob + 31) / 32), dim3(64 * PRED_NW), (pred_lds_bytes<8, 2>(h->nu)), s, a, pa);
      else if (nu4) hipLaunchKernelGGL((asm_predict_k<4, 4>), dim3((nprob + 63) / 64), dim3(64 * PRED_NW), (pred_lds_bytes<4, 4>(h->nu)), s, a, pa);
      else hipLaunchKernelGGL((asm_predict_k<4, 2, false>), dim3((nprob + 31) / 32), dim3(64 * PRED_NW), (pred_lds_bytes<4, 2>(h->nu)), s, a, pa);
      a.pred_w = W;
      { static const int pf = getenv("NNMPC_PRED_F64") ? atoi(getenv("NNMPC_PRED_F64")) : 0; a.pred_f64 = pf; }
    }
  }
  hipLaunchKernelGGL(asm_init_k, dim3((segp + 3) / 4), dim3(256), 0, s, a, segp);
  const int lds_big = (a.max_active + ASM_TS) * 8;
  int* cnt = h->pin_cnt;
  memset(cnt, 0, ASM_NCNT * sizeof(int));
  int rounds = 0;
  int prev_rows = 0;
  int kprev = 0, wide_cols = 0, fused_c0 = -1;
  HIPCHK(hipMemsetAsync(h->asm_counters, 0, ASM_NCNT * sizeof(int), s));
  if (small) {
    EvScope es(h, 4, 0.0);
    static const int g0 = getenv("NNMPC_SMALL_GRACE") ? atoi(getenv("NNMPC_SMALL_GRACE")) : ASM_SM_GRACE;
    hipLaunchKernelGGL((asm_small_k<2, 3, 4>), dim3(nprob), dim3(64), asm_small_lds_bytes(2, h->n, h->nu), s, a, a.max_rounds, g0);
    hipLaunchKernelGGL((asm_small_k<7, 1, 8>), dim3(nprob), dim3(64), asm_small_lds_bytes(7, h->n, h->nu), s, a, a.max_rounds, g0);
    if (asm_small_lds_bytes(9, h->n, h->nu) <= ASM_SMALL9_LDS_MAX)
      hipLaunchKernelGGL((asm_small_k<9, 1, 8>), dim3(nprob), dim3(64), asm_small_lds_bytes(9, h->n, h->nu), s, a, a.max_rounds, g0);
    h->stats.asm_rounds += 1;
    h->stats.asm_small_passes += 1;
    static const bool trace = getenv("NNMPC_TRACE_ROUNDS") != nullptr;
    if (trace) {
      std::vector<int> rd(nprob), mg(nprob), stt(nprob);
      HIPCHK(stream_sync(s));
      hipMemcpy(rd.data(), h->asm_rounds, nprob * sizeof(int), hipMemcpyDeviceToHost);
      hipMemcpy(mg.data(), h->asm_mg, nprob * sizeof(int), hipMemcpyDeviceToHost);
      hipMemcpy(stt.data(), h->asm_state, nprob * sizeof(int), hipMemcpyDeviceToHost);
      long sum = 0, sm = 0, big = 0, bigit = 0, left = 0; int mx = 0, mm = 0, mxbig = 0, hist[8] = {0};
      for (int i = 0; i < nprob; ++i) {
        sum += rd[i]; mx = std::max(mx, rd[i]); sm += mg[i]; mm = std::max(mm, mg[i]); left += stt[i] == ASM_RUN;
        if (mg[i] > 32) { ++big; bigit += rd[i]; mxbig = std::max(mxbig, rd[i]); }
        hist[std::min(7, rd[i] / 8)]++;
      }
      fprintf(stderr, "asm small: %d problems, iterations mean %.2f max %d, final sets mean %.1f max %d; sets > 32: %ld (iterations mean %.1f max %d); handed on %ld; iterations/8 histogram",
              nprob, (double)sum / nprob, mx, (double)sm / nprob, mm, big, big ? (double)bigit / big : 0.0, mxbig, left);
      for (int b = 0; b < 8; ++b) fprintf(stderr, " %d", hist[b]);
      fprintf(stderr, "\n");
#ifdef ASM_SM_PROF
      unsigned long long tp[2][8];
      hipMemcpyFromSymbol(tp, HIP_SYMBOL(asm_small_prof), sizeof tp);
      for (int k = 0; k < 2; ++k)
        fprintf(stderr, "  small instance %d clock sums: list %llu, rhs + solve %llu, x window %llu, signs %llu, exchange / loop %llu; iterations %llu\n", k, tp[k][0], tp[k][1], tp[k][2], tp[k][3], tp[k][5], tp[k][6]);
      memset(tp, 0, sizeof tp); hipMemcpyToSymbol(HIP_SYMBOL(asm_small_prof), tp, sizeof tp);
#endif
    }
  }
  static const bool trace_tail = getenv("NNMPC_TRACE_ROUNDS") != nullptr;
  const bool defer_cnt = tail_only && !trace_tail;
  if (tail_only) {
    EvScope es(h, 4, 0.0);
    hipLaunchKernelGGL(asm_taillist_k, dim3((nprob + 255) / 256), dim3(256), 0, s, a);
    const int lds_tail = (a.max_active + ASM_TS + ASM_TAIL_AREA) * 8 + ((h->n + 15) / 16) * 16 + ASM_TAIL_EXTRA;
    hipLaunchKernelGGL(asm_tail_k, dim3(nprob), dim3(256), lds_tail, s, a, h->asm_tail_budget);
    if (!defer_cnt) {
      HIPCHK(hipMemcpyAsync(cnt, h->asm_counters, ASM_NCNT * sizeof(int), hipMemcpyDeviceToHost, s));
      HIPCHK(stream_sync(s));
    }
    h->stats.asm_rounds += 1;
    if (trace_tail) {
      std::vector<int> rd(nprob), mg(nprob);
      hipMemcpy(rd.data(), h->asm_rounds, nprob * sizeof(int), hipMemcpyDeviceToHost);
      hipMemcpy(mg.data(), h->asm_mg, nprob * sizeof(int), hipMemcpyDeviceToHost);
      long sum = 0, sm = 0; int mx = 0, mm = 0;
      for (int i = 0; i < nprob; ++i) { sum += rd[i]; mx = std::max(mx, rd[i]); sm += mg[i]; mm = std::max(mm, mg[i]); }
      fprintf(stderr, "asm tail only: %d problems, iterations mean %.2f max %d, active bounds mean %.1f max %d\n", nprob, (double)sum / nprob, mx, (double)sm / nprob, mm);
    }
  }
  for (; !tail_only && rounds < 2 * a.max_rounds + 2; ++rounds) {
    if (prev_rows) {
      {
        EvScope es(h, 5, 0.0);
        const int c0 = (a.W < h->np && (h->np - a.W) % 128 == 0) ? a.W : 0;
        fused_c0 = ((h->np - c0) % 128 == 0 && !no_fuse) ? c0 : -1;
        const int ntm = (prev_rows + 127) / 128, ntn = (h->np - c0) / 128;
        a.wrows = prev_rows;
        const nnmpc_qp::Far* ff = nullptr;
        if (lazy && fused_c0 > 0 && !no_far) {
          for (const auto& f : h->far) if (f.W == c0) ff = &f;
          if (!ff && h->far_missing.size() < 16 && std::find(h->far_missing.begin(), h->far_missing.end(), c0) == h->far_missing.end())
            h->far_missing.push_back(c0);
        }
        a.ff_err = 0.0; a.ff_efar = 0.0; a.ff_skip = 0; wide_far_rp = 0;
        if (ff) {
          a.ffU = ff->U; a.ffVx = ff->Vx; a.ffVl = ff->Vl; a.ffcu = ff->cu; a.ffk = ff->kt; a.ffr = ff->rp; a.ffW = ff->W;
          a.ff_err = h->p_inf * ff->efar; a.ff_efar = ff->efar;
          a.ff_skip = h->nout <= c0 && h->nout < h->n;
          wide_far_rp = ff->rp; wide_far_ksum = ff->ksum;
          h->stats.asm_far_passes += 1;
          hipLaunchKernelGGL(asm_wide_t_k, dim3(g64_grid(ntm, ff->rp / 128)), dim3(256), G64_LDS, s, a, ntm, ff->rp / 128);
          if (a.ff_skip) hipLaunchKernelGGL(asm_wide_tnorm_k, dim3((ntm * 128 + 3) / 4), dim3(256), 0, s, a, ntm);
          hipLaunchKernelGGL(asm_wide_gemm_k<WIDE_FAR>, dim3(g64_grid(ntm, ntn)), dim3(256), G64_LDS, s, a, c0, ntm, ntn);
        } else if (fused_c0 >= 0 && lazy) {
          hipLaunchKernelGGL(asm_wide_gemm_k<WIDE_LAZY>, dim3(g64_grid(ntm, ntn)), dim3(256), G64_LDS, s, a, c0, ntm, ntn);
        } else if (fused_c0 >= 0) {
          hipLaunchKernelGGL(asm_wide_gemm_k<WIDE_XUNC>, dim3(g64_grid(ntm, ntn)), dim3(256), G64_LDS, s, a, c0, ntm, ntn);
        } else {
          gemm64(h, h->asm_xhw + c0, h->np, h->asm_lam, h->np, h->H64 + (size_t)c0 * h->np, h->np, ((prev_rows + 127) / 128) * 128,
                 h->np - c0, h->np, nullptr, 0, h->asm_kblk, nullptr, true);
        }
        wide_cols = h->np - c0;
      }
      EvScope es(h, 6, 0.0);
      hipLaunchKernelGGL(asm_wide_k, dim3((prev_rows + 3) / 4), dim3(256), 0, s, a, fused_c0);
    }
    a.kref = kprev;
    if (!a.pred_w) a.refine_later = 0;
    a.refine = a.refine_later && rounds >= 1;
    {
      EvScope es(h, 6, 0.0);
      hipLaunchKernelGGL(asm_count_k, dim3((nprob + 3) / 4), dim3(256), 0, s, a);
      hipLaunchKernelGGL(asm_bins_a_k, dim3((nprob + 1023) / 1024), dim3(1024), 0, s, a);
      hipLaunchKernelGGL(asm_bins_b_k, dim3((nprob + 1023) / 1024), dim3(1024), 0, s, a);
    }
    HIPCHK(hipMemcpyAsync(cnt, h->asm_counters, ASM_NCNT * sizeof(int), hipMemcpyDeviceToHost, s));
    HIPCHK(stream_sync(s));
    const int n64 = cnt[2], n32 = cnt[ASM_CNT_ROWS32], nrun = n64 + n32;
    if (h->profiling)
    {
        const double nw = cnt[ASM_CNT_WIDE + 1], ksum = cnt[ASM_CNT_WKSUM];
        if (wide_far_rp) {
          const double chunks = cnt[ASM_CNT_FFTILES] - fft_prev;
          h->stats.asm_gemm_flops += 2.0 * wide_far_rp * (ksum + nw * h->ka) +
                                     (a.ff_skip ? 2.0 * G64_KC * 128.0 * 128.0 * chunks : 2.0 * 128.0 * wide_far_ksum * nw);
        } else {
          h->stats.asm_gemm_flops += 2.0 * wide_cols * (ksum + (lazy ? nw * h->ka : 0.0));
        }
        fft_prev = cnt[ASM_CNT_FFTILES];
    }
    kprev = cnt[3];
    {
      static const bool trace = getenv("NNMPC_TRACE_ROUNDS") != nullptr;
      if (trace) {
        fprintf(stderr, "asm round %d: fp64 %d f32 %d last-active %d wide-checked %d big %d big32 %d | fp64 classes", rounds, n64, n32, cnt[3],
                cnt[ASM_CNT_WIDE + 1], cnt[1], cnt[ASM_CNT_BIG32] + cnt[ASM_CNT_BIG32B]);
        for (int b = 0; b < ASM_NBIN; ++b) fprintf(stderr, " %d", cnt[4 + b]);
        fprintf(stderr, " | f32 classes");
        for (int b = 0; b < ASM_NBIN; ++b) fprintf(stderr, " %d", cnt[ASM_CNT_F32 + b]);
        fprintf(stderr, "\n");
      }
    }
    if (nrun == 0) break;
    static const int tail_max = getenv("NNMPC_TAIL_MAX") ? atoi(getenv("NNMPC_TAIL_MAX")) : 256;
    if (nrun <= std::min(h->asm_pool, tail_max) && (rounds >= (a.pred_w ? 2 : 6) || small)) {
      EvScope es(h, 4, 0.0);
      hipLaunchKernelGGL(asm_taillist_k, dim3((nprob + 255) / 256), dim3(256), 0, s, a);
      if (Wx < h->np) {
        gemm64(h, h->asm_xunc + Wx, h->np, h->x0_64, h->ka, h->Kunc64 + (size_t)Wx * h->ka, h->ka, ((nrun + 127) / 128) * 128, h->np - Wx, h->ka,
               nullptr, 0, nullptr, h->asm_counters + ASM_CNT_TAIL, false, h->asm_biglist);
        a.Wx = h->np;
      }
      const int lds_tail = (a.max_active + ASM_TS + ASM_TAIL_AREA) * 8 + ((h->n + 15) / 16) * 16 + ASM_TAIL_EXTRA;
      hipLaunchKernelGGL(asm_tail_k, dim3(nrun), dim3(256), lds_tail, s, a, h->asm_tail_budget);
      HIPCHK(hipMemcpyAsync(cnt, h->asm_counters, ASM_NCNT * sizeof(int), hipMemcpyDeviceToHost, s));
      HIPCHK(stream_sync(s));
      {
        static const bool trace = getenv("NNMPC_TRACE_ROUNDS") != nullptr;
        if (trace) {
          std::vector<int> rd(nprob), bl(nrun);
          hipMemcpy(rd.data(), h->asm_rounds, nprob * sizeof(int), hipMemcpyDeviceToHost);
          hipMemcpy(bl.data(), h->asm_biglist, nrun * sizeof(int), hipMemcpyDeviceToHost);
          long sum = 0; int mx = 0;
          for (int i = 0; i < nrun; ++i) { const int r = rd[bl[i]] - rounds; sum += r; mx = std::max(mx, r); }
          fprintf(stderr, "asm tail after round %d: %d problems, iterations mean %.1f max %d\n", rounds, nrun, (double)sum / nrun, mx);
#ifdef ASM_TAIL_PROF
          unsigned long long tp[8];
          hipMemcpyFromSymbol(tp, HIP_SYMBOL(asm_tail_prof), sizeof tp);
          fprintf(stderr, "  tail clock sums (all workgroups): count/factor/solve %llu, substitutions %llu, x loop %llu, tests %llu, exchange %llu; iterations on the dense factor %llu, on a fresh factorisation %llu\n",
                  tp[0], tp[1], tp[2], tp[3], tp[4], tp[5], tp[6]);
          memset(tp, 0, sizeof tp); hipMemcpyToSymbol(HIP_SYMBOL(asm_tail_prof), tp, sizeof tp);
#endif
        }
      }
      h->stats.asm_rounds += 1;
      rounds = 0;
      break;
    }
    h->stats.asm_rounds += 1;
    a.W = std::min(h->np, ((cnt[3] + 1 + h->nu + 127) / 128) * 128);
    if (a.W > Wx) {
      EvScope es(h, 5, 2.0 * (a.W - Wx) * (double)h->ka * nprob);
      gemm64(h, h->asm_xunc + Wx, h->np, h->x0_64, h->ka, h->Kunc64 + (size_t)Wx * h->ka, h->ka, segp, a.W - Wx, h->ka);
      Wx = a.W; a.Wx = Wx;
    }
    {
      EvScope es(h, 4, 0.0);
      const int nreg2_wg = (cnt[4 + 6] + 1) / 2 + (cnt[4 + 7] + 1) / 2;
      const int nreg32b_wg = (cnt[ASM_CNT_F32 + 6] + 3) / 4 + (cnt[ASM_CNT_F32 + 7] + 3) / 4;
      const int nwg64 = a.use_wg ? cnt[ASM_CNT_BIG64] : 0;
      const int nwg32 = a.use_wg ? cnt[ASM_CNT_BIG32] : 0;
      const int nwg32b = a.use_wg ? cnt[ASM_CNT_BIG32B] : 0;
      const int nwg64r = a.use_wg ? cnt[ASM_CNT_BIG64R] : 0;
      int nbig = cnt[1] + cnt[ASM_CNT_BIG32] + nreg2_wg + nreg32b_wg + nwg64 + nwg32b + nwg64r, nreg_wg = 0, nreg32_wg = 0;
      for (int b = 0; b < ASM_NREG; ++b) { nreg_wg += (cnt[4 + b] + 3) / 4; nreg32_wg += (cnt[ASM_CNT_F32 + b] + 3) / 4; }
      const bool side4 = cnt[1] > 0, side2 = nwg64 + nwg32 + nwg32b + nwg64r > 0 || (cnt[ASM_CNT_BIG32] && !a.use_wg), side3 = nreg2_wg + nreg32b_wg > 0;
      if (nbig) {
        HIPCHK(hipEventRecord(h->ev_fork, s));
        if (side4) {
          HIPCHK(hipStreamWaitEvent(h->stream4, h->ev_fork, 0));
          { EvScope e9(h, 9, 0.0, h->stream4); hipLaunchKernelGGL((asm_lambda_tile_k<1>), dim3(std::min(cnt[1], h->asm_pool)), dim3(256), lds_big, h->stream4, a, 0); }
          HIPCHK(hipEventRecord(h->ev_join4, h->stream4));
        }
        if (side2) {
          HIPCHK(hipStreamWaitEvent(h->stream2, h->ev_fork, 0));
          EvScope e9(h, 9, 0.0, h->stream2);
          if (nwg64) hipLaunchKernelGGL(asm_lambda_wg64_k, dim3(nwg64), dim3(256), asm_wg_lds_bytes<double>(), h->stream2, a);
          if (nwg64r) hipLaunchKernelGGL(asm_lambda_wg64r_k, dim3(nwg64r), dim3(512), (asm_wg_lds_bytes_refine<float, ASM_WG_MB8>()), h->stream2, a);
          if (nwg32b) hipLaunchKernelGGL(asm_lambda_wg32b_k, dim3(nwg32b), dim3(512), (asm_wg_lds_bytes<float, ASM_WG_MB8>()), h->stream2, a);
          if (nwg32) hipLaunchKernelGGL(asm_lambda_wg32_k, dim3(nwg32), dim3(256), asm_wg_lds_bytes<float>(), h->stream2, a);
          if (cnt[ASM_CNT_BIG32] && !a.use_wg) hipLaunchKernelGGL(asm_lambda_tile32_k, dim3(std::min(cnt[ASM_CNT_BIG32], 4096)), dim3(512), ASM_TILE32_LDS, h->stream2, a);
          HIPCHK(hipEventRecord(h->ev_join, h->stream2));
        }
        if (side3) {
          HIPCHK(hipStreamWaitEvent(h->stream3, h->ev_fork, 0));
          EvScope e9(h, 9, 0.0, h->stream3);
          if (nreg2_wg && a.use_wg) hipLaunchKernelGGL(asm_lambda_wg64s_k, dim3(cnt[4 + 6] + cnt[4 + 7]), dim3(128), asm_wg_lds_bytes<double>(), h->stream3, a);
          else if (nreg2_wg) hipLaunchKernelGGL(asm_lambda_reg2_k, dim3(nreg2_wg), dim3(128), ASM_REG2_LDS, h->stream3, a);
          if (nreg32b_wg) hipLaunchKernelGGL(asm_lambda_reg32b_k, dim3(nreg32b_wg), dim3(256), ASM_REG32B_LDS, h->stream3, a);
          HIPCHK(hipEventRecord(h->ev_join3, h->stream3));
        }
      }
      if (nreg_wg) { EvScope e8(h, 8, 0.0); hipLaunchKernelGGL(asm_lambda_reg_k, dim3(nreg_wg), dim3(256), ASM_REG_LDS, s, a); }
      if (nreg32_wg) { EvScope e7(h, 7, 0.0); hipLaunchKernelGGL(asm_lambda_reg32_k, dim3(nreg32_wg), dim3(256), ASM_REG32_LDS, s, a); }
      if (side2) HIPCHK(hipStreamWaitEvent(s, h->ev_join, 0));
      if (side3) HIPCHK(hipStreamWaitEvent(s, h->ev_join3, 0));
      if (side4) HIPCHK(hipStreamWaitEvent(s, h->ev_join4, 0));
    }
    {
      EvScope es(h, 5, 2.0 * a.W * (double)cnt[0]);
      if (n64)
        gemm64(h, h->asm_xh, h->np, h->asm_lam, h->np, h->H64, h->np, ((n64 + 127) / 128) * 128, a.W, h->np, nullptr, 0,
               h->asm_kblk, nullptr, true);
      if (n32 && a.W % 128 == 0)
        hipLaunchKernelGGL((gemm_nt_f32_kdyn_k<128>), dim3(a.W / 128, (n32 + 127) / 128), dim3(256), TileCfg<128>::LDS_FLOATS * 4, s,
                           h->asm_xh32, (size_t)h->np, h->asm_lam32, (size_t)h->np, h->H32, (size_t)h->np, h->np, h->asm_kblk + a.nkblk / 2, 2);
      else if (n32)
        hipLaunchKernelGGL((gemm_nt_f32_kdyn_k<64>), dim3(a.W / 64, (n32 + 63) / 64), dim3(256), TileCfg<64>::LDS_FLOATS * 4, s,
                           h->asm_xh32, (size_t)h->np, h->asm_lam32, (size_t)h->np, h->H32, (size_t)h->np, h->np, h->asm_kblk + a.nkblk / 2, 1);
    }
    {
      EvScope es(h, 6, 0.0);
      if (n64) HIPCHK(hipMemsetAsync(h->asm_rowprob, 0xFF, (size_t)((n64 + 127) / 128) * 128 * sizeof(int), s));
      hipLaunchKernelGGL(asm_update_k, dim3((nprob + 3) / 4), dim3(256), 0, s, a);
    }
    prev_rows = a.W < h->n ? n64 : 0;
  }
  if (rounds >= 2 * a.max_rounds + 2) {
    HIPCHK(hipMemcpyAsync(cnt, h->asm_counters, ASM_NCNT * sizeof(int), hipMemcpyDeviceToHost, s));
    HIPCHK(stream_sync(s));
  }
  if (h->gemm_error) { h->gemm_error = false; return NNMPC_EINVAL; }
  if (!defer_cnt) h->stats.asm_full_checks += cnt[ASM_CNT_DONE];
  if (defer_cnt || cnt[ASM_CNT_DONE] > 0) {
    gemm64(h, h->q64_all, h->np, h->x0_64, h->ka, h->tq64, h->ka, segp, h->np, h->ka, h->asm_state, ASM_DONE);
    gemm64(h, h->asm_xh, h->np, h->asm_x, h->np, h->P64, h->np, segp, h->np, h->np, h->asm_state, ASM_DONE);
  }
  hipLaunchKernelGGL(asm_certify_k, dim3(nprob), dim3(256), 0, s, a, h->pscale);
  int* st = h->pin_st;
  HIPCHK(hipMemcpyAsync(st, h->asm_status, (size_t)nprob * sizeof(int), hipMemcpyDeviceToHost, s));
  int* pin_its = h->pin_cnt + ASM_NCNT;
  if (h->profiling && pred_flops_per_it > 0.0) HIPCHK(hipMemcpyAsync(pin_its, h->pred_cnt + 1, 4, hipMemcpyDeviceToHost, s));
  if (defer_cnt) HIPCHK(hipMemcpyAsync(cnt, h->asm_counters, ASM_NCNT * sizeof(int), hipMemcpyDeviceToHost, s));
  HIPCHK(stream_sync(s));
  if (defer_cnt) h->stats.asm_full_checks += cnt[ASM_CNT_DONE];
  if (h->profiling && pred_flops_per_it > 0.0) h->stats.asm_predict_flops += pred_flops_per_it * (double)*pin_its;
  HIPCHK(hipGetLastError());
  std::vector<int> fb;
  int ninvalid = 0;
  for (int p = 0; p < nprob; ++p) { if (st[p] == 3) fb.push_back(p); else if (st[p] != 0) ++ninvalid; }
  h->stats.asm_solved += nprob - (int64_t)fb.size() - ninvalid;
  if (st_dev) HIPCHK(hipMemcpyAsync(st_dev, h->asm_status, (size_t)nprob * sizeof(int), hipMemcpyDeviceToDevice, s));
  if (fb.empty()) { h->stats.problems += nprob; return 0; }
  if (h->opts.method == 2) {
    for (int p = 0; p < nprob; ++p) st[p] = st[p] == 3 ? NNMPC_ST_MAXITER : st[p];
    if (st_dev) HIPCHK(hipMemcpy(st_dev, st, (size_t)nprob * sizeof(int), hipMemcpyHostToDevice));
    h->stats.problems += nprob;
    return 0;
  }
  const int cntf = (int)fb.size();
  int* list = nullptr; double *x0c = nullptr, *lbc = nullptr, *ubc = nullptr, *uc = nullptr;
  uint32_t* actc = nullptr; int *stc = nullptr, *itc = nullptr;
  unsigned char* guessc = nullptr;
  int rc = 0;
  if (!rc) rc = scratch_get(h, nnmpc_qp::SC_FB_GUESS, &guessc, (size_t)cntf * h->n);
  if (!rc) rc = scratch_get(h, nnmpc_qp::SC_FB_LIST, &list, cntf * sizeof(int));
  if (!rc) rc = scratch_get(h, nnmpc_qp::SC_FB_X0, &x0c, (size_t)cntf * h->n_aug * 8);
  if (!rc) rc = scratch_get(h, nnmpc_qp::SC_FB_LB, &lbc, (size_t)cntf * h->nu * 8);
  if (!rc) rc = scratch_get(h, nnmpc_qp::SC_FB_UB, &ubc, (size_t)cntf * h->nu * 8);
  if (!rc) rc = scratch_get(h, nnmpc_qp::SC_FB_U, &uc, (size_t)cntf * h->n * 8);
  if (!rc) rc = scratch_get(h, nnmpc_qp::SC_FB_ACT, &actc, (size_t)cntf * h->words * 4);
  if (!rc) rc = scratch_get(h, nnmpc_qp::SC_FB_ST, &stc, (size_t)cntf * 4);
  if (!rc) rc = scratch_get(h, nnmpc_qp::SC_FB_IT, &itc, (size_t)cntf * 8);
  if (rc) return rc;
  HIPCHK(hipMemcpy(list, fb.data(), cntf * sizeof(int), hipMemcpyHostToDevice));
  hipLaunchKernelGGL(asm_gather_k, dim3(cntf), dim3(128), 0, s, x0c, lbc, ubc, x0_dev, lb_dev, ub_dev, list, cntf, h->n_aug, h->nu);
  hipLaunchKernelGGL(asm_gather_guess_k, dim3(cntf), dim3(128), 0, s, guessc, h->asm_st, h->asm_state, list, cntf, h->n);
  const int ldu_caller = h->ldu, nout_caller = h->nout;
  h->ldu = h->n; h->nout = h->n;
  for (int b0 = 0; b0 < cntf && !rc; b0 += h->seg_max) {
    const int nb = std::min(h->seg_max, cntf - b0);
    rc = solve_segment(h, nb, x0c + (size_t)b0 * h->n_aug, lbc + (size_t)b0 * h->nu, ubc + (size_t)b0 * h->nu, guessc + (size_t)b0 * h->n,
                       uc + (size_t)b0 * h->n, actc + (size_t)b0 * h->words, stc + b0, itc + 2 * (size_t)b0);
  }
  h->ldu = ldu_caller; h->nout = nout_caller;
  if (!rc) {
    hipLaunchKernelGGL(asm_scatter_k, dim3(cntf), dim3(128), 0, s, u_dev, act_dev, st_dev, it_dev, uc, actc, stc, itc,
                       list, cntf, h->n, h->words, h->ldu, h->nout);
    HIPCHK(stream_sync(s));
  }
  h->stats.problems += nprob - cntf;
  return rc;
}

}

hipStream_t nnmpc_qp_stream_internal(nnmpc_qp* h) { return h->stream; }

extern "C" {

int nnmpc_qp_create(nnmpc_qp** out, int32_t n, int32_t nu, int32_t n_aug, const double* P,
                    const double* tq, const double* Kunc, const nnmpc_qp_opts* opts) {
  if (!out || !P || !tq || n <= 0 || nu <= 0 || nu > 256 || n_aug <= 0 || n % nu != 0) {
    set_error("nnmpc_qp_create: bad arguments (n=%d nu=%d n_aug=%d)", n, nu, n_aug);
    return NNMPC_EINVAL;
  }
  int ndev = 0;
  if (hipGetDeviceCount(&ndev) != hipSuccess || ndev == 0) {
    set_error("nnmpc_qp_create: no HIP device available (this library has no CPU fallback)");
    return NNMPC_EHIP;
  }
  nnmpc_qp* h = new nnmpc_qp();
  memset(&h->stats, 0, sizeof(h->stats));
  memset(&h->d, 0, sizeof(h->d));
  h->profiling = false; h->ev_used = 0; h->have_inverse = false;
  h->ldu = n; h->nout = n;
  if (opts) h->opts = *opts; else memset(&h->opts, 0, sizeof(h->opts));
  nnmpc_qp_opts& o = h->opts;
  if (o.max_batch <= 0) o.max_batch = 1024;
  if (o.nb == 0) o.nb = (n <= 1024) ? 64 : 128;
  if (o.nb != 64 && o.nb != 128) { set_error("nb must be 64 or 128"); delete h; return NNMPC_EINVAL; }
  if (o.max_ipm_iters <= 0) o.max_ipm_iters = 40;
  if (o.max_polish_rounds <= 0) o.max_polish_rounds = 150;
  if (o.max_refine <= 0) o.max_refine = 60;
  if (o.max_rounds <= 0) o.max_rounds = 1000;
  if (o.sub_steps <= 0) o.sub_steps = 8;
  if (o.stale_max_changes == 0) o.stale_max_changes = 4;
  if (o.stale_cg_limit <= 0) o.stale_cg_limit = 16;
  if (o.asm_max_active <= 0) o.asm_max_active = 768;
  if (o.asm_max_active > 768) o.asm_max_active = 768;
  o.asm_max_active = std::max(16, (o.asm_max_active / 16) * 16);
  h->asm_tail_budget = o.asm_max_rounds <= 0 ? 50000 : o.asm_max_rounds;
  if (o.asm_max_rounds <= 0) o.asm_max_rounds = 200;
  if (o.asm_predict_iters > PRED_MAXIT) o.asm_predict_iters = PRED_MAXIT;
  if (o.sub_steps < 2) o.sub_steps = 2;
  if (o.ipm_tol <= 0.f) o.ipm_tol = 1e-2f;
  if (o.refine_tol <= 0.0) o.refine_tol = 1e-10;
  if (o.bound_tol <= 0.0) o.bound_tol = 1e-9;
  hipGetDevice(&h->device);
  h->n = n; h->nu = nu; h->n_aug = n_aug;
  h->NB = o.nb;
  h->np = ((n + h->NB - 1) / h->NB) * h->NB;
  h->T = h->np / h->NB;
  h->tiles = h->T * (h->T + 1) / 2;
  h->ka = ((n_aug + 31) / 32) * 32;
  h->slots = ((o.max_batch + 127) / 128) * 128;
  h->words = (2 * n + 31) / 32;
  h->have_kunc = Kunc != nullptr;
  if ((size_t)(h->np + 5 * h->NB) * 4 > 96 * 1024) { set_error("n too large for the LDS-resident solve vector"); delete h; return NNMPC_EINVAL; }
  if (hipStreamCreate(&h->stream) != hipSuccess) { set_error("hipStreamCreate failed"); delete h; return NNMPC_EHIP; }
  if (hipStreamCreate(&h->stream2) != hipSuccess || hipStreamCreate(&h->stream3) != hipSuccess || hipStreamCreate(&h->stream4) != hipSuccess ||
      hipEventCreateWithFlags(&h->ev_fork, hipEventDisableTiming) != hipSuccess ||
      hipEventCreateWithFlags(&h->ev_join3, hipEventDisableTiming) != hipSuccess || hipEventCreateWithFlags(&h->ev_join4, hipEventDisableTiming) != hipSuccess ||
      hipEventCreateWithFlags(&h->ev_join, hipEventDisableTiming) != hipSuccess) {
    set_error("hipStreamCreate / hipEventCreate failed"); nnmpc_qp_destroy(h); return NNMPC_EHIP;
  }
  {
    hipError_t e = hipSuccess;
    if (e == hipSuccess) e = hipFuncSetAttribute((const void*)asm_lambda_reg_k, hipFuncAttributeMaxDynamicSharedMemorySize, ASM_REG_LDS);
    if (e == hipSuccess) e = hipFuncSetAttribute((const void*)asm_lambda_reg2_k, hipFuncAttributeMaxDynamicSharedMemorySize, ASM_REG2_LDS);
    if (e == hipSuccess) e = hipFuncSetAttribute((const void*)asm_lambda_reg32_k, hipFuncAttributeMaxDynamicSharedMemorySize, ASM_REG32_LDS);
    if (e == hipSuccess) e = hipFuncSetAttribute((const void*)asm_tail_k, hipFuncAttributeMaxDynamicSharedMemorySize, 150 * 1024);
    if (e == hipSuccess) e = hipFuncSetAttribute((const void*)asm_lambda_reg32b_k, hipFuncAttributeMaxDynamicSharedMemorySize, ASM_REG32B_LDS);
    if (e == hipSuccess) e = hipFuncSetAttribute((const void*)asm_lambda_tile32_k, hipFuncAttributeMaxDynamicSharedMemorySize, ASM_TILE32_LDS);
    if (e == hipSuccess) e = hipFuncSetAttribute((const void*)gemm_nt_f64_t128_k, hipFuncAttributeMaxDynamicSharedMemorySize, G64_LDS);
    if (e == hipSuccess) e = hipFuncSetAttribute((const void*)asm_wide_gemm_k<WIDE_XUNC>, hipFuncAttributeMaxDynamicSharedMemorySize, G64_LDS);
    if (e == hipSuccess) e = hipFuncSetAttribute((const void*)asm_wide_gemm_k<WIDE_LAZY>, hipFuncAttributeMaxDynamicSharedMemorySize, G64_LDS);
    if (e == hipSuccess) e = hipFuncSetAttribute((const void*)asm_wide_gemm_k<WIDE_FAR>, hipFuncAttributeMaxDynamicSharedMemorySize, G64_LDS);
    if (e == hipSuccess) e = hipFuncSetAttribute((const void*)asm_wide_t_k, hipFuncAttributeMaxDynamicSharedMemorySize, G64_LDS);
    if (e == hipSuccess) e = hipFuncSetAttribute((const void*)asm_small_k<9, 1, 8>, hipFuncAttributeMaxDynamicSharedMemorySize, ASM_SMALL9_LDS_MAX);
    if (e == hipSuccess) e = hipFuncSetAttribute((const void*)gemm_nt_f32_kdyn_k<128>, hipFuncAttributeMaxDynamicSharedMemorySize, TileCfg<128>::LDS_FLOATS * 4);
    if (e != hipSuccess) { set_error("hipFuncSetAttribute(MaxDynamicSharedMemorySize) failed"); nnmpc_qp_destroy(h); return NNMPC_EHIP; }
  }
  if (set_lds_attrs<128>() != 0 || set_lds_attrs<64>() != 0) {
    set_error("hipFuncSetAttribute(MaxDynamicSharedMemorySize) failed"); nnmpc_qp_destroy(h); return NNMPC_EHIP;
  }

  const int np = h->np, NB = h->NB, ka = h->ka, S = h->slots;
  const size_t nb2 = (size_t)NB * NB;
  int rc = 0;
#define A_(ptr, cnt) if (!rc) rc = dev_alloc(h, &(ptr), (size_t)(cnt))
  A_(h->Pt, h->tiles * nb2); A_(h->P32, (size_t)np * np); A_(h->P64, (size_t)np * np);
  A_(h->tq64, (size_t)np * ka); A_(h->Kunc32, (size_t)np * ka); A_(h->pdiag, np);
  A_(h->L, (size_t)S * h->tiles * nb2); A_(h->Y, (size_t)S * h->T * nb2); A_(h->Dacc, (size_t)S * h->T * nb2); A_(h->trsv_count, 1);
  QpDev& d = h->d;
  const size_t V = (size_t)S * np;
  A_(d.u, V); A_(d.zu, V); A_(d.zl, V); A_(d.lbv, V); A_(d.ubv, V); A_(d.q, V); A_(d.PU, V);
  A_(d.rd, V); A_(d.rhs, V); A_(d.sol, V); A_(d.dua, V); A_(d.dvec, V); A_(d.mask, V); A_(d.uunc, V);
  A_(d.x, V); A_(d.q64, V); A_(d.PX, V); A_(d.r64, V); A_(d.p64, V); A_(d.v64, V); A_(d.st, V);
  A_(d.phase, S); A_(d.f_factor, S); A_(d.f_solve, S); A_(d.istep, S); A_(d.ipm_it, S);
  A_(d.nfac, S); A_(d.prounds, S); A_(d.pninf, S); A_(d.pgrace, S); A_(d.ptie, S); A_(d.rcnt, S); A_(d.psub, S); A_(d.fail, S); A_(d.stale, S); A_(d.rz, S);
  A_(d.mu, S); A_(d.gap, S); A_(d.smu, S); A_(d.qscale, S); A_(d.counters, 8);
  {
    size_t free_b = 0, total_b = 0;
    if (hipMemGetInfo(&free_b, &total_b) != hipSuccess) free_b = (size_t)12e9;
    long long cap = (long long)(0.25 * (double)free_b / (12.0 * np + 88.0 * np + n + 4.0 * o.asm_max_active + 64.0));
    if (o.seg_max > 0) cap = std::min<long long>(cap, o.seg_max);
    cap = std::max<long long>(cap, S);
    cap = std::min<long long>(cap, 1 << 20);
    h->seg_max = (int)((cap / 128) * 128);
  }
  const size_t G = h->seg_max;
  A_(h->x0_64, G * ka); A_(h->x0_32, G * ka);
  A_(h->q64_all, G * np); A_(h->uunc_all, G * np);
  A_(h->lb_d, G * nu); A_(h->ub_d, G * nu);
  A_(h->in_stage, G * n_aug);
  if (!rc && hipHostMalloc((void**)&h->pin_cnt, (ASM_NCNT + 4) * sizeof(int)) != hipSuccess) { set_error("nnmpc_qp_create: hipHostMalloc failed"); rc = NNMPC_EHIP; }
  if (!rc && hipHostMalloc((void**)&h->pin_st, G * sizeof(int)) != hipSuccess) { set_error("nnmpc_qp_create: hipHostMalloc failed"); rc = NNMPC_EHIP; }
  A_(d.lb64, (size_t)S * nu); A_(d.ub64, (size_t)S * nu);
  A_(d.slot_prob, S); A_(d.age, S); A_(d.next_prob, 1);
  h->asm_pool = h->seg_max >= 4096 ? (getenv("NNMPC_TAIL_MAX") && atoi(getenv("NNMPC_TAIL_MAX")) > 1024 ? 2048 : 1024) : 256;
  A_(h->H64, (size_t)np * np); A_(h->Kunc64, (size_t)np * ka); A_(h->H32, (size_t)np * np);
  A_(h->asm_xunc, G * np); A_(h->asm_x, G * np); A_(h->asm_lam, G * np); A_(h->asm_xh, G * np);
  A_(h->asm_xhw, (G + 256) * np); A_(h->asm_rowprob, G + 256); A_(h->asm_wflag, G); A_(h->asm_wmark, G);
  A_(h->asm_tnorm, G + 128 * (ASM_NKG + 1)); A_(h->asm_tslack, G + 128 * (ASM_NKG + 1));
  A_(h->asm_st, G * n); A_(h->asm_state, G); A_(h->asm_rounds, G); A_(h->asm_counters, ASM_NCNT);
  A_(h->asm_biglist, G); A_(h->asm_status, G); A_(h->asm_binlist, (size_t)(ASM_NLIST + 4) * G);
  A_(h->asm_idxg, G * o.asm_max_active); A_(h->asm_mg, G); A_(h->asm_row, G); A_(h->asm_lrank, G); A_(h->asm_ctot, ((G + 1023) / 1024) * ASM_NSCAN); A_(h->asm_prec, G); A_(h->asm_redo, G); A_(h->asm_rowk, G); A_(h->asm_lam32, G * np); A_(h->asm_xh32, G * np); A_(h->asm_alpha, G); A_(h->asm_ninf, G); A_(h->asm_hi, G); A_(h->asm_kblk, 2 * (G / 64 + 2)); A_(h->asm_work, 3 * G);
  A_(h->asm_scratch, (size_t)h->asm_pool * ((size_t)(o.asm_max_active / 16) * (o.asm_max_active / 16 + 1) / 2 * ASM_TS));
#undef A_
  if (rc) { nnmpc_qp_destroy(h); return rc; }
  d.n = n; d.np = np; d.nu = nu; d.slots = S; d.words = h->words;
  d.max_ipm = o.max_ipm_iters; d.max_polish = o.max_polish_rounds; d.max_refine = o.max_refine;
  d.max_rounds = o.max_rounds; d.stale_max_changes = o.stale_max_changes; d.stale_cg_limit = o.stale_cg_limit;
  d.ipm_tol = o.ipm_tol; d.refine_tol = o.refine_tol; d.bound_tol = o.bound_tol; d.stat_tol = 1e-8;

  std::vector<float> pt(h->tiles * nb2, 0.f), p32((size_t)np * np, 0.f), k32((size_t)np * ka, 0.f), pdg(np, 1.f);
  std::vector<double> p64((size_t)np * np, 0.0), t64((size_t)np * ka, 0.0);
  {
    std::vector<double> dg(n);
    for (int r = 0; r < n; ++r) dg[r] = P[(size_t)r * n + r];
    std::nth_element(dg.begin(), dg.begin() + n / 2, dg.end());
    h->pscale = dg[n / 2];
    if (!(h->pscale > 0.0)) { set_error("P has a non-positive diagonal"); nnmpc_qp_destroy(h); return NNMPC_EINVAL; }
  }
  const double ips = 1.0 / h->pscale;
  float pdmax = 0.f;
  for (int r = 0; r < n; ++r) {
    pdg[r] = (float)(P[(size_t)r * n + r] * ips);
    pdmax = std::max(pdmax, pdg[r]);
    for (int c = 0; c <= r; ++c) {
      const double v = P[(size_t)r * n + c];
      p64[(size_t)r * np + c] = v; p64[(size_t)c * np + r] = v;
      p32[(size_t)r * np + c] = (float)(v * ips); p32[(size_t)c * np + r] = (float)(v * ips);
    }
  }
  d.pscale = h->pscale;
  for (int r = 0; r < n; ++r) {
    double rs = 0.0;
    for (int c = 0; c < n; ++c) rs += std::fabs(p64[(size_t)r * np + c]);
    h->p_inf = std::max(h->p_inf, rs);
  }
  d.delta = 16.f * 5.96e-8f * pdmax;
  d.pdiag = h->pdiag;
  for (int i = 0; i < h->T; ++i)
    for (int j = 0; j <= i; ++j) {
      float* t = pt.data() + ((size_t)i * (i + 1) / 2 + j) * nb2;
      for (int r = 0; r < NB; ++r)
        for (int c = 0; c < NB; ++c) {
          const int gr = i * NB + r, gc = j * NB + c;
          float v = 0.f;
          if (gr < n && gc < n) v = (float)((gc <= gr ? P[(size_t)gr * n + gc] : P[(size_t)gc * n + gr]) * ips);
          else if (gr == gc) v = 1.f;
          t[(size_t)r * NB + c] = v;
        }
    }
  h->tqmax = 0.0;
  for (int r = 0; r < n; ++r)
    for (int k = 0; k < n_aug; ++k) {
      t64[(size_t)r * ka + k] = tq[(size_t)r * n_aug + k];
      h->tqmax = std::max(h->tqmax, std::fabs(tq[(size_t)r * n_aug + k]));
      if (Kunc) k32[(size_t)r * ka + k] = (float)Kunc[(size_t)r * n_aug + k];
    }
  hipError_t e = hipSuccess;
  if (e == hipSuccess) e = hipMemcpy(h->Pt, pt.data(), pt.size() * 4, hipMemcpyHostToDevice);
  if (e == hipSuccess) e = hipMemcpy(h->P32, p32.data(), p32.size() * 4, hipMemcpyHostToDevice);
  if (e == hipSuccess) e = hipMemcpy(h->P64, p64.data(), p64.size() * 8, hipMemcpyHostToDevice);
  if (e == hipSuccess) e = hipMemcpy(h->tq64, t64.data(), t64.size() * 8, hipMemcpyHostToDevice);
  if (e == hipSuccess) e = hipMemcpy(h->Kunc32, k32.data(), k32.size() * 4, hipMemcpyHostToDevice);
  if (e == hipSuccess) e = hipMemcpy(h->pdiag, pdg.data(), pdg.size() * 4, hipMemcpyHostToDevice);
  if (e != hipSuccess) { set_error("upload of P/tq failed: %s", hipGetErrorString(e)); nnmpc_qp_destroy(h); return NNMPC_EHIP; }
  *out = h;
  return NNMPC_OK;
}

int nnmpc_qp_destroy(nnmpc_qp* h) {
  if (!h) return NNMPC_OK;
  hipDeviceSynchronize();
  for (void* p : h->allocs) hipFree(p);
  for (auto& g : h->far) { hipFree(g.U); hipFree(g.Vx); hipFree(g.Vl); hipFree(g.cu); hipFree(g.kt); }
  for (auto& sc : h->sc) if (sc.p) hipFree(sc.p);
  for (hipEvent_t e : h->ev_pool) hipEventDestroy(e);
  if (h->ev_fork) hipEventDestroy(h->ev_fork);
  if (h->ev_join) hipEventDestroy(h->ev_join);
  if (h->ev_join3) hipEventDestroy(h->ev_join3);
  if (h->ev_join4) hipEventDestroy(h->ev_join4);
  if (h->pin_cnt) hipHostFree(h->pin_cnt);
  if (h->pin_st) hipHostFree(h->pin_st);
  if (h->stream2) hipStreamDestroy(h->stream2);
  if (h->stream3) hipStreamDestroy(h->stream3);
  if (h->stream4) hipStreamDestroy(h->stream4);
  if (h->stream) hipStreamDestroy(h->stream);
  delete h;
  return NNMPC_OK;
}

int nnmpc_qp_set_inverse(nnmpc_qp* h, const double* Hinv, const double* Kunc) {
  if (!h || !Hinv || !Kunc) { set_error("nnmpc_qp_set_inverse: bad arguments"); return NNMPC_EINVAL; }
  HIPCHK(hipSetDevice(h->device));
  const int n = h->n, np = h->np, ka = h->ka, n_aug = h->n_aug;
  if ((uint64_t)np * np * 8 >= (1ull << 32)) {
    set_error("nnmpc_qp_set_inverse: n = %d is too large for the active-set pass (n < 23168)", n);
    return NNMPC_EINVAL;
  }
  std::vector<double> hh((size_t)np * np, 0.0), kk((size_t)np * ka, 0.0);
  for (int r = 0; r < n; ++r) {
    for (int c = 0; c < n; ++c) hh[(size_t)r * np + c] = 0.5 * (Hinv[(size_t)r * n + c] + Hinv[(size_t)c * n + r]);
    for (int k = 0; k < n_aug; ++k) kk[(size_t)r * ka + k] = Kunc[(size_t)r * n_aug + k];
  }
  HIPCHK(hipMemcpy(h->H64, hh.data(), hh.size() * 8, hipMemcpyHostToDevice));
  {
    std::vector<float> h32(hh.size());
    for (size_t i = 0; i < hh.size(); ++i) h32[i] = (float)hh[i];
    HIPCHK(hipMemcpy(h->H32, h32.data(), h32.size() * 4, hipMemcpyHostToDevice));
  }
  HIPCHK(hipMemcpy(h->Kunc64, kk.data(), kk.size() * 8, hipMemcpyHostToDevice));
  h->pred[0].L = h->pred[1].L = 0.0;
  if (h->nu <= 64 && h->nu >= 4 && h->opts.asm_predict_iters >= 0) {
    if (np >= PRED_W && n >= PRED_W) {
      const int rc = build_predictor<4>(h, hh, np, h->pred[0]);
      if (rc) return rc;
      if (!h->pred_cnt) { const int rc2 = dev_alloc(h, &h->pred_cnt, 4); if (rc2) return rc2; }
      HIPCHK(hipFuncSetAttribute((const void*)asm_predict_k<4, 4>, hipFuncAttributeMaxDynamicSharedMemorySize, pred_lds_bytes<4, 4>(h->nu)));
      HIPCHK(hipFuncSetAttribute((const void*)asm_predict_k<4, 2, false>, hipFuncAttributeMaxDynamicSharedMemorySize, pred_lds_bytes<4, 2>(h->nu)));
    }
    if (np >= PRED_W2 && n >= PRED_W2 && h->pred[0].L > 0.0 && h->nu % 4 == 0) {
      const int rc = build_predictor<8>(h, hh, np, h->pred[1]);
      if (rc) return rc;
      HIPCHK(hipFuncSetAttribute((const void*)asm_predict_k<8, 2>, hipFuncAttributeMaxDynamicSharedMemorySize, pred_lds_bytes<8, 2>(h->nu)));
    }
  }
  {
    const int kap = ((n_aug + 63) / 64) * 64;
    double *tmp = nullptr, *kt = nullptr;
    HIPCHK(hipMalloc((void**)&tmp, (size_t)np * np * 8));
    HIPCHK(hipMalloc((void**)&kt, (size_t)kap * np * 8));
    std::vector<double> ktr((size_t)kap * np, 0.0);
    for (int r = 0; r < n; ++r)
      for (int k = 0; k < n_aug; ++k) ktr[(size_t)k * np + r] = Kunc[(size_t)r * n_aug + k];
    HIPCHK(hipMemcpy(kt, ktr.data(), ktr.size() * 8, hipMemcpyHostToDevice));
    gemm64(h, tmp, np, h->P64, np, h->H64, np, np, np, np);
    HIPCHK(stream_sync(h->stream));
    std::vector<double> c((size_t)np * np);
    HIPCHK(hipMemcpy(c.data(), tmp, c.size() * 8, hipMemcpyDeviceToHost));
    double e2 = 0.0;
    for (int r = 0; r < n; ++r)
      for (int cc = 0; cc < n; ++cc) e2 = std::max(e2, std::fabs(c[(size_t)r * np + cc] - (r == cc ? 1.0 : 0.0)));
    gemm64(h, tmp, kap, h->P64, np, kt, np, np, kap, np);
    HIPCHK(stream_sync(h->stream));
    HIPCHK(hipMemcpy(c.data(), tmp, (size_t)np * kap * 8, hipMemcpyDeviceToHost));
    std::vector<double> tqh((size_t)np * ka);
    HIPCHK(hipMemcpy(tqh.data(), h->tq64, tqh.size() * 8, hipMemcpyDeviceToHost));
    double e1 = 0.0;
    for (int r = 0; r < n; ++r)
      for (int k = 0; k < n_aug; ++k) e1 = std::max(e1, std::fabs(c[(size_t)r * kap + k] + tqh[(size_t)r * ka + k]));
    hipFree(tmp); hipFree(kt);
    h->asm_e1max = e1; h->asm_e2max = e2;
    if (!(e2 < 1e-6) || !(e1 == e1)) {
      set_error("nnmpc_qp_set_inverse: |P Pinv - I|_max = %.3e: the supplied inverse is not usable", e2);
      return NNMPC_EINVAL;
    }
  }
  h->have_inverse = true;
  return NNMPC_OK;
}

int nnmpc_qp_set_farfield(nnmpc_qp* h, int32_t W, int32_t r, const double* U, const double* Vx, const double* Vl) {
  if (!h || !U || !Vx || !Vl || r <= 0) { set_error("nnmpc_qp_set_farfield: bad arguments"); return NNMPC_EINVAL; }
  if (!h->have_inverse) { set_error("nnmpc_qp_set_farfield: needs nnmpc_qp_set_inverse first"); return NNMPC_EINVAL; }
  HIPCHK(hipSetDevice(h->device));
  const int n = h->n, np = h->np, ka = h->ka, n_aug = h->n_aug;
  const int rp = ((r + 127) / 128) * 128;
  if (W <= 0 || W % 128 != 0 || W >= n || np % 128 != 0) { set_error("nnmpc_qp_set_farfield: W = %d must be a multiple of 128 below n = %d (padded %d)", W, n, np); return NNMPC_EINVAL; }
  if ((double)rp * (ka + W + (np - W)) > 0.8 * (double)(ka + W) * (np - W)) {
    set_error("nnmpc_qp_set_farfield: rank %d does not pay against the dense form at W = %d (n = %d, n_aug = %d)", r, W, n, n_aug);
    return NNMPC_EINVAL;
  }
  if (rp > np) { set_error("nnmpc_qp_set_farfield: rank %d too large for the workspace", r); return NNMPC_EINVAL; }
  const int nf = np - W;
  std::vector<double> u((size_t)nf * rp, 0.0), vx((size_t)rp * ka, 0.0), vl((size_t)rp * W, 0.0), cu(nf / 128, 0.0);
  for (int j = 0; j < n - W; ++j)
    for (int i = 0; i < r; ++i) u[(size_t)j * rp + i] = U[(size_t)j * r + i];
  for (int i = 0; i < r; ++i) {
    for (int k = 0; k < n_aug; ++k) vx[(size_t)i * ka + k] = Vx[(size_t)i * n_aug + k];
    for (int k = 0; k < W; ++k) vl[(size_t)i * W + k] = Vl[(size_t)i * W + k];
  }
  {
    double run = 0.0;
    for (int t = nf / 128 - 1; t >= 0; --t) {
      for (int j = 128 * t; j < 128 * (t + 1); ++j) {
        double s2 = 0.0;
        for (int i = 0; i < rp; ++i) s2 += u[(size_t)j * rp + i] * u[(size_t)j * rp + i];
        run = std::max(run, std::sqrt(s2) * (1.0 + 1e-12));
      }
      cu[t] = run;
    }
  }
  std::vector<int> kt(nf / 128, 0);
  double ksum = 0.0;
  for (int t = 0; t < nf / 128; ++t) {
    int last = 0;
    for (int j = 128 * t; j < 128 * (t + 1); ++j)
      for (int i = rp - 1; i >= last; --i)
        if (u[(size_t)j * rp + i] != 0.0) { last = i + 1; break; }
    kt[t] = ((last + G64_KC - 1) / G64_KC) * G64_KC;
    ksum += kt[t];
  }
  nnmpc_qp::Far f;
  f.W = W; f.r = r; f.rp = rp; f.U = f.Vx = f.Vl = f.cu = nullptr; f.kt = nullptr; f.ksum = ksum; f.efar = 0.0;
  unsigned long long* em = nullptr;
  auto release = [&](nnmpc_qp::Far& g) {
    hipFree(g.U); hipFree(g.Vx); hipFree(g.Vl); hipFree(g.cu); hipFree(g.kt);
    g.U = g.Vx = g.Vl = g.cu = nullptr; g.kt = nullptr;
  };
  auto fail = [&](int code) { release(f); if (em) hipFree(em); return code; };
#define FFCHK(x) do { hipError_t e_ = (x); if (e_ != hipSuccess) { set_error("%s: %s", #x, hipGetErrorString(e_)); return fail(e_ == hipErrorOutOfMemory ? NNMPC_ENOMEM : NNMPC_EHIP); } } while (0)
  FFCHK(hipMalloc((void**)&f.U, u.size() * 8));
  FFCHK(hipMalloc((void**)&f.Vx, vx.size() * 8));
  FFCHK(hipMalloc((void**)&f.Vl, vl.size() * 8));
  FFCHK(hipMalloc((void**)&f.cu, cu.size() * 8));
  FFCHK(hipMalloc((void**)&f.kt, kt.size() * sizeof(int)));
  FFCHK(hipMemcpy(f.kt, kt.data(), kt.size() * sizeof(int), hipMemcpyHostToDevice));
  FFCHK(hipMemcpy(f.U, u.data(), u.size() * 8, hipMemcpyHostToDevice));
  FFCHK(hipMemcpy(f.Vx, vx.data(), vx.size() * 8, hipMemcpyHostToDevice));
  FFCHK(hipMemcpy(f.Vl, vl.data(), vl.size() * 8, hipMemcpyHostToDevice));
  FFCHK(hipMemcpy(f.cu, cu.data(), cu.size() * 8, hipMemcpyHostToDevice));
  {
    FFCHK(hipMalloc((void**)&em, 8));
    FFCHK(hipMemset(em, 0, 8));
    hipLaunchKernelGGL(far_verify_k, dim3(nf), dim3(256), rp * sizeof(double), h->stream, f.U, f.Vx, f.Vl, h->Kunc64, h->H64, W, rp, ka, np, em);
    unsigned long long bits = 0;
    FFCHK(hipMemcpyAsync(&bits, em, 8, hipMemcpyDeviceToHost, h->stream));
    FFCHK(stream_sync(h->stream));
    hipFree(em); em = nullptr;
    double e;
    memcpy(&e, &bits, 8);
    f.efar = e;
    if (!(e < 1e-9)) { set_error("nnmpc_qp_set_farfield: max |U V' - M| = %.3e: the factors are not usable", e); return fail(NNMPC_EINVAL); }
  }
#undef FFCHK
  h->far_missing.erase(std::remove(h->far_missing.begin(), h->far_missing.end(), W), h->far_missing.end());
  for (auto& g : h->far) if (g.W == W) { HIPCHK(stream_sync(h->stream)); release(g); g = f; return NNMPC_OK; }
  h->far.push_back(f);
  return NNMPC_OK;
}

int nnmpc_qp_farfield_missing(nnmpc_qp* h, int32_t* W) {
  if (!h || !W) { set_error("nnmpc_qp_farfield_missing: bad arguments"); return NNMPC_EINVAL; }
  *W = 0;
  if (!h->far_missing.empty()) { *W = h->far_missing.back(); h->far_missing.pop_back(); }
  return NNMPC_OK;
}

int nnmpc_qp_dims(nnmpc_qp* h, int32_t* n, int32_t* nu, int32_t* n_aug) {
  if (!h) { set_error("nnmpc_qp_dims: null handle"); return NNMPC_EINVAL; }
  if (n) *n = h->n;
  if (nu) *nu = h->nu;
  if (n_aug) *n_aug = h->n_aug;
  return NNMPC_OK;
}

int nnmpc_qp_set_profiling(nnmpc_qp* h, int32_t on) {
  if (!h) return NNMPC_EINVAL;
  h->profiling = on != 0;
  return NNMPC_OK;
}

int nnmpc_qp_get_stats(nnmpc_qp* h, nnmpc_qp_stats* out, int32_t reset) {
  if (!h || !out) return NNMPC_EINVAL;
  *out = h->stats;
  out->asm_e1max = h->asm_e1max; out->asm_e2max = h->asm_e2max;
  {
    std::vector<double> w(3 * (size_t)h->seg_max, 0.0);
    hipMemcpy(w.data(), h->asm_work, w.size() * sizeof(double), hipMemcpyDeviceToHost);
    double f = 0.0, b = 0.0, f32 = 0.0;
    for (size_t i = 0; i < w.size(); i += 3) { f += w[i]; b += w[i + 1]; f32 += w[i + 2]; }
    out->asm_lambda_flops = f; out->asm_lambda_bytes = b; out->asm_lambda32_flops = f32;
    if (reset) hipMemset(h->asm_work, 0, w.size() * sizeof(double));
  }
  {
    unsigned long long c = 0;
    hipMemcpy(&c, h->trsv_count, sizeof(c), hipMemcpyDeviceToHost);
    out->trsv_solves = (int64_t)c;
    if (reset) hipMemset(h->trsv_count, 0, sizeof(c));
  }
  if (reset) memset(&h->stats, 0, sizeof(h->stats));
  return NNMPC_OK;
}

int nnmpc_qp_solve_batch(nnmpc_qp* h, int32_t B, const double* x0, const double* lb, const double* ub,
                         double* u, uint32_t* active, int32_t* status, int32_t* iters, int32_t ptr_kind) {
  return nnmpc_qp_solve_batch_ex(h, B, x0, lb, ub, nullptr, u, active, status, iters, ptr_kind, NNMPC_OUT_SEQUENCE);
}

int nnmpc_qp_solve_batch_warm(nnmpc_qp* h, int32_t B, const double* x0, const double* lb, const double* ub,
                              const uint8_t* guess, double* u, uint32_t* active, int32_t* status,
                              int32_t* iters, int32_t ptr_kind) {
  return nnmpc_qp_solve_batch_ex(h, B, x0, lb, ub, guess, u, active, status, iters, ptr_kind, NNMPC_OUT_SEQUENCE);
}

int nnmpc_qp_solve_batch_ex(nnmpc_qp* h, int32_t B, const double* x0, const double* lb, const double* ub,
                            const uint8_t* guess, double* u, uint32_t* active, int32_t* status,
                            int32_t* iters, int32_t ptr_kind, int32_t out_kind) {
  if (!h || B < 0 || !x0 || !lb || !ub || !u) { set_error("nnmpc_qp_solve_batch: bad arguments"); return NNMPC_EINVAL; }
  if (out_kind != NNMPC_OUT_SEQUENCE && out_kind != NNMPC_OUT_FIRST_MOVE) { set_error("nnmpc_qp_solve_batch_ex: bad out_kind %d", out_kind); return NNMPC_EINVAL; }
  if (B == 0) return NNMPC_OK;
  HIPCHK(hipSetDevice(h->device));
  const int G = h->seg_max;
  const int ncol = out_kind == NNMPC_OUT_FIRST_MOVE ? h->nu : h->n;
  h->ldu = ncol; h->nout = ncol;
  size_t e_tot0 = 0;
  if (h->profiling) { e_tot0 = ev_get(h); hipEventRecord(h->ev_pool[e_tot0], h->stream); }
  double* u_stage = nullptr; uint32_t* a_stage = nullptr; int32_t* s_stage = nullptr; int32_t* i_stage = nullptr;
  unsigned char* g_stage = nullptr;
  const int gmax = std::min(G, (int)B);
  int rc = 0;
  if (ptr_kind == NNMPC_HOST) {
    if (!rc) rc = scratch_get(h, nnmpc_qp::SC_U, &u_stage, (size_t)gmax * ncol * sizeof(double));
    if (!rc && active) rc = scratch_get(h, nnmpc_qp::SC_ACT, &a_stage, (size_t)gmax * h->words * sizeof(uint32_t));
    if (!rc && status) rc = scratch_get(h, nnmpc_qp::SC_ST, &s_stage, (size_t)gmax * sizeof(int32_t));
    if (!rc && iters) rc = scratch_get(h, nnmpc_qp::SC_IT, &i_stage, (size_t)gmax * 2 * sizeof(int32_t));
    if (!rc && guess) rc = scratch_get(h, nnmpc_qp::SC_GUESS, &g_stage, (size_t)gmax * h->n);
  }
  hipError_t he = hipSuccess;
#define STEP_(x) do { if (!rc && he == hipSuccess) { he = (x); if (he != hipSuccess) { set_error("%s: %s", #x, hipGetErrorString(he)); rc = NNMPC_EHIP; } } } while (0)
  for (int b0 = 0; b0 < B && !rc; b0 += G) {
    const int nb = std::min(G, B - b0);
    const double *x0d, *lbd, *ubd;
    double* ud; uint32_t* ad; int32_t* sd; int32_t* idv;
    const unsigned char* gd = nullptr;
    if (ptr_kind == NNMPC_HOST) {
      if (guess) { STEP_(hipMemcpyAsync(g_stage, guess + (size_t)b0 * h->n, (size_t)nb * h->n, hipMemcpyHostToDevice, h->stream)); gd = g_stage; }
      STEP_(hipMemcpyAsync(h->in_stage, x0 + (size_t)b0 * h->n_aug, (size_t)nb * h->n_aug * 8, hipMemcpyHostToDevice, h->stream));
      STEP_(hipMemcpyAsync(h->lb_d, lb + (size_t)b0 * h->nu, (size_t)nb * h->nu * 8, hipMemcpyHostToDevice, h->stream));
      STEP_(hipMemcpyAsync(h->ub_d, ub + (size_t)b0 * h->nu, (size_t)nb * h->nu * 8, hipMemcpyHostToDevice, h->stream));
      x0d = h->in_stage; lbd = h->lb_d; ubd = h->ub_d;
      ud = u_stage; ad = active ? a_stage : nullptr; sd = status ? s_stage : nullptr; idv = iters ? i_stage : nullptr;
    } else {
      x0d = x0 + (size_t)b0 * h->n_aug; lbd = lb + (size_t)b0 * h->nu; ubd = ub + (size_t)b0 * h->nu;
      if (guess) gd = guess + (size_t)b0 * h->n;
      ud = u + (size_t)b0 * ncol;
      ad = active ? active + (size_t)b0 * h->words : nullptr;
      sd = status ? status + b0 : nullptr;
      idv = iters ? iters + 2 * (size_t)b0 : nullptr;
    }
    if (rc) break;
    if (h->have_inverse && h->opts.method != 1) rc = solve_segment_asm(h, nb, x0d, lbd, ubd, gd, ud, ad, sd, idv);
    else rc = solve_segment(h, nb, x0d, lbd, ubd, gd, ud, ad, sd, idv);
    if (!rc && ptr_kind == NNMPC_HOST) {
      STEP_(hipMemcpy(u + (size_t)b0 * ncol, u_stage, (size_t)nb * ncol * 8, hipMemcpyDeviceToHost));
      if (active) STEP_(hipMemcpy(active + (size_t)b0 * h->words, a_stage, (size_t)nb * h->words * 4, hipMemcpyDeviceToHost));
      if (status) STEP_(hipMemcpy(status + b0, s_stage, (size_t)nb * 4, hipMemcpyDeviceToHost));
      if (iters) STEP_(hipMemcpy(iters + 2 * (size_t)b0, i_stage, (size_t)nb * 8, hipMemcpyDeviceToHost));
    }
  }
#undef STEP_
  if (h->profiling) {
    size_t e1 = ev_get(h);
    hipEventRecord(h->ev_pool[e1], h->stream);
    stream_sync(h->stream);
    h->ev_recs.push_back({3, e_tot0, e1, 0.0});
    ev_collect(h);
  }
  return rc;
}

int nnmpc_qp_debug_factor_solve(nnmpc_qp* h, int32_t B, const float* dvec, const float* mask,
                                const float* rhs, float* sol) {
  if (!h || B <= 0 || B > h->slots || !dvec || !mask || !rhs || !sol) { set_error("debug_factor_solve: bad arguments"); return NNMPC_EINVAL; }
  HIPCHK(hipSetDevice(h->device));
  QpDev& d = h->d;
  const int rows = h->slots;
  std::vector<float> dv((size_t)rows * h->np, 0.f), mk((size_t)rows * h->np, 1.f), rh((size_t)rows * h->np, 0.f);
  std::vector<int> fl(rows, 0);
  for (int p = 0; p < B; ++p) {
    fl[p] = 1;
    for (int r = 0; r < h->n; ++r) {
      dv[(size_t)p * h->np + r] = dvec[(size_t)p * h->n + r];
      mk[(size_t)p * h->np + r] = mask[(size_t)p * h->n + r];
      rh[(size_t)p * h->np + r] = rhs[(size_t)p * h->n + r];
    }
  }
  HIPCHK(hipMemcpy(d.dvec, dv.data(), dv.size() * 4, hipMemcpyHostToDevice));
  HIPCHK(hipMemcpy(d.mask, mk.data(), mk.size() * 4, hipMemcpyHostToDevice));
  HIPCHK(hipMemcpy(d.rhs, rh.data(), rh.size() * 4, hipMemcpyHostToDevice));
  HIPCHK(hipMemcpy(d.f_factor, fl.data(), rows * 4, hipMemcpyHostToDevice));
  HIPCHK(hipMemset(d.fail, 0, rows * 4));
  factor_dispatch(h, rows, B);
  solve_dispatch(h, rows, d.f_factor);
  HIPCHK(stream_sync(h->stream));
  HIPCHK(hipGetLastError());
  std::vector<float> so((size_t)rows * h->np);
  HIPCHK(hipMemcpy(so.data(), d.sol, so.size() * 4, hipMemcpyDeviceToHost));
  for (int p = 0; p < B; ++p)
    for (int r = 0; r < h->n; ++r) sol[(size_t)p * h->n + r] = so[(size_t)p * h->np + r];
  if (h->profiling) { stream_sync(h->stream); ev_collect(h); }
  return NNMPC_OK;
}

}
```

industrial_nnmpc_2021_amd/qp.py:

```python
import ctypes as C
import numpy as np

from . import _lib


def _ptr(a):
    if a is None:
        return None, None
    if hasattr(a, "data_ptr"):
        return C.c_void_p(a.data_ptr()), _lib.DEVICE
    return a.ctypes.data_as(C.c_void_p), _lib.HOST


def _staircase(U0, tol, block=128, chunk=16):
    import scipy.linalg as sla
    nf, r = U0.shape
    nb = -(-nf // block)
    Rs = [None] * nb
    below = np.zeros((0, r))
    for j in range(nb - 1, -1, -1):
        below = Rs[j] = sla.qr(np.vstack((U0[j * block:(j + 1) * block], below)), mode="r")[0][:r]
    cur = np.eye(r)
    drops, kj = [], np.zeros(nb, int)
    for j in range(nb):
        if cur.shape[0]:
            _, sv, vt = sla.svd(Rs[j] @ cur.T)
            k = int((sv > tol).sum())
            drops.append(vt[k:] @ cur)
            cur = vt[:k] @ cur
        else:
            drops.append(np.zeros((0, r)))
        kj[j] = cur.shape[0]
    G = np.vstack([cur] + drops[:0:-1])
    if G.shape[0] == 0:
        G = np.eye(1, r)
    kj = np.minimum(-(-kj // chunk) * chunk, G.shape[0])
    U1 = U0 @ G.T
    for j in range(nb):
        U1[j * block:(j + 1) * block, kj[j]:] = 0.0
    return np.ascontiguousarray(U1), G


class BatchedBoxQP:

    def __init__(self, P, tq, nu, *, Kunc="auto", method="auto", farfield="auto", max_batch=1024, nb=0, ipm_tol=0.0,
                 max_rounds=0, max_ipm_iters=0, max_polish_rounds=0, max_refine=0, sub_steps=0, stale_max_changes=0, stale_cg_limit=0, asm_max_active=0,
                 asm_max_rounds=0, asm_f32_rounds=0, seg_max=0, asm_tail_batch=0, asm_predict_iters=0):
        lib = _lib.load()
        P = np.ascontiguousarray(P, dtype=np.float64)
        tq = np.ascontiguousarray(tq, dtype=np.float64)
        n, n_aug = tq.shape
        if P.shape != (n, n) or n % nu:
            raise ValueError("P must be (n, n), tq (n, n_aug), n a multiple of nu")
        meth = {"auto": 0, "pdip": 1, "asm": 2}[method]
        Hinv = None
        if isinstance(Kunc, str) and Kunc == "auto":
            import scipy.linalg as sla
            Ps = np.tril(P) + np.tril(P, -1).T
            cf = sla.cho_factor(Ps, lower=True)
            Kunc = -sla.cho_solve(cf, tq)
            if meth != 1:
                Hinv = sla.cho_solve(cf, np.eye(n))
        elif meth == 2:
            raise ValueError("method='asm' needs Kunc='auto' (the inverse Hessian is built with it)")
        if Kunc is not None:
            Kunc = np.ascontiguousarray(Kunc, dtype=np.float64)
        self.n, self.n_aug, self.nu = n, n_aug, nu
        self.words = (2 * n + 31) // 32
        opts = _lib.QpOpts(max_batch=max_batch, nb=nb, max_ipm_iters=max_ipm_iters,
                           max_polish_rounds=max_polish_rounds, max_refine=max_refine,
                           max_rounds=max_rounds, sub_steps=sub_steps, stale_max_changes=stale_max_changes,
                           stale_cg_limit=stale_cg_limit, method=meth, asm_max_active=asm_max_active,
                           asm_max_rounds=asm_max_rounds, asm_f32_rounds=asm_f32_rounds, seg_max=seg_max, asm_tail_batch=asm_tail_batch,
                           asm_predict_iters=asm_predict_iters,
                           ipm_tol=ipm_tol, refine_tol=0.0, bound_tol=0.0)
        self._h = C.c_void_p()
        kp = Kunc.ctypes.data_as(C.c_void_p) if Kunc is not None else None
        _lib.check(lib.nnmpc_qp_create(C.byref(self._h), n, nu, n_aug,
                                       P.ctypes.data_as(C.c_void_p), tq.ctypes.data_as(C.c_void_p),
                                       kp, C.byref(opts)), "nnmpc_qp_create")
        self._lib = lib
        self.have_inverse = False
        if Hinv is not None:
            Hinv = np.ascontiguousarray(Hinv, dtype=np.float64)
            rc = lib.nnmpc_qp_set_inverse(self._h, Hinv.ctypes.data_as(C.c_void_p), Kunc.ctypes.data_as(C.c_void_p))
            if rc == _lib.EINVAL and meth == 0:
                import warnings
                warnings.warn("BatchedBoxQP: " + lib.nnmpc_last_error().decode(errors="replace") +
                              " -- continuing with the PDIP path only", RuntimeWarning)
            else:
                _lib.check(rc, "nnmpc_qp_set_inverse")
                self.have_inverse = True
        self._ff_wmax = (n // 2 // 128) * 128
        self._ff_src = (np.ascontiguousarray(Hinv[:, :self._ff_wmax]), Kunc) if (self.have_inverse and farfield and self._ff_wmax > 0) else None
        nb_lib = nb if nb else (128 if n > 1024 else 64)
        self._np = -(-n // nb_lib) * nb_lib
        self._ff_done = set()
        self.farfield_info = {}
        if self._ff_src is not None and not isinstance(farfield, str):
            for W in farfield:
                self.prepare_farfield(int(W))

    def close(self):
        if getattr(self, "_h", None) is not None and self._h.value:
            self._lib.nnmpc_qp_destroy(self._h)
            self._h = C.c_void_p()
        self._ff_src = None

    __del__ = close

    def prepare_farfield(self, W, rtol=1e-13):
        if self._ff_src is None or W in self._ff_done:
            return 0
        self._ff_done.add(W)
        self.farfield_info[W] = dict(rank=0, reason="window not on the 128-column grid")
        Hinv, Kunc = self._ff_src
        if W <= 0 or W % 128 or W >= self.n or self._np % 128 or W > self._ff_wmax:
            return 0
        import scipy.linalg as sla
        M = np.hstack((Kunc[W:], -Hinv[W:, :W]))
        U, s, Vt = sla.svd(M, full_matrices=False, lapack_driver="gesdd")
        r = max(1, int((s > rtol * s[0]).sum()))
        rp, nf, k = -(-r // 128) * 128, self.n - W, -(-self.n_aug // 32) * 32 + W
        self.farfield_info[W] = dict(rank=0, numerical_rank=r, sigma_ratio_at_rank=float(s[min(r, s.size - 1)] / s[0]),
                                     reason="the factored form would not pay: numerical rank too large")
        if rp * (k + nf) > 0.8 * k * nf:
            return 0
        Uf, G = _staircase(U[:, :r] * s[:r], rtol * s[0])
        r = G.shape[0]
        Vt = G @ Vt[:G.shape[1]]
        Vx, Vl = np.ascontiguousarray(Vt[:, :self.n_aug]), np.ascontiguousarray(Vt[:, self.n_aug:])
        p = lambda a: a.ctypes.data_as(C.c_void_p)
        rc = self._lib.nnmpc_qp_set_farfield(self._h, W, r, p(Uf), p(Vx), p(Vl))
        if rc == _lib.EINVAL:
            import warnings
            self.farfield_info[W] = dict(rank=0, numerical_rank=r, reason=self._lib.nnmpc_last_error().decode(errors="replace"))
            warnings.warn("BatchedBoxQP.prepare_farfield: " + self.farfield_info[W]["reason"], RuntimeWarning)
            return 0
        _lib.check(rc, "nnmpc_qp_set_farfield")
        kj = [int(np.flatnonzero(np.abs(Uf[j:j + 128]).max(axis=0) > 0).max(initial=-1)) + 1 for j in range(0, Uf.shape[0], 128)]
        self.farfield_info[W] = dict(rank=int(r), staircase_mean_k=float(np.mean(kj)), staircase_max_k=int(max(kj)))
        return r

    def prepare_farfield_windows(self, lo=128, hi=None):
        hi = self.n // 4 if hi is None else hi
        return {W: self.prepare_farfield(W) for W in range(lo, hi + 1, 128)}

    def _farfield_auto(self):
        if self._ff_src is None:
            return
        for _ in range(32):
            W = C.c_int32(0)
            _lib.check(self._lib.nnmpc_qp_farfield_missing(self._h, C.byref(W)), "nnmpc_qp_farfield_missing")
            if not W.value:
                break
            self.prepare_farfield(W.value)

    def solve_batch(self, x0, lb, ub, guess=None, first_move_only=False):
        x0 = np.ascontiguousarray(x0, dtype=np.float64).reshape(-1, self.n_aug)
        B = x0.shape[0]
        lb = np.ascontiguousarray(np.broadcast_to(np.asarray(lb, np.float64).reshape(-1, self.nu), (B, self.nu)))
        ub = np.ascontiguousarray(np.broadcast_to(np.asarray(ub, np.float64).reshape(-1, self.nu), (B, self.nu)))
        u = np.empty((B, self.nu if first_move_only else self.n))
        act = np.zeros((B, self.words), np.uint32)
        status = np.empty(B, np.int32)
        iters = np.empty((B, 2), np.int32)
        gp = None
        if guess is not None:
            guess = np.ascontiguousarray(guess, dtype=np.uint8).reshape(B, self.n)
            gp = guess.ctypes.data_as(C.c_void_p)
        p = lambda a: a.ctypes.data_as(C.c_void_p)
        _lib.check(self._lib.nnmpc_qp_solve_batch_ex(
            self._h, B, p(x0), p(lb), p(ub), gp, p(u), p(act), p(status), p(iters), _lib.HOST,
            _lib.OUT_FIRST_MOVE if first_move_only else _lib.OUT_SEQUENCE), "nnmpc_qp_solve_batch_ex")
        self._farfield_auto()
        bits = np.unpackbits(act.view(np.uint8), axis=1, bitorder="little")[:, :2 * self.n].astype(bool)
        return dict(u=u, active=bits, status=status, ipm_iters=iters[:, 0], factorizations=iters[:, 1])

    def active_to_state(self, active):
        n, nu = self.n, self.nu
        k, c = np.arange(n) // nu, np.arange(n) % nu
        return (active[:, k * 2 * nu + c].astype(np.uint8) + 2 * active[:, k * 2 * nu + nu + c].astype(np.uint8))

    def solve_batch_device(self, B, x0, lb, ub, u, active=None, status=None, iters=None, guess=None,
                           first_move_only=False):
        q = lambda a: (_ptr(a)[0] if a is not None else None)
        _lib.check(self._lib.nnmpc_qp_solve_batch_ex(
            self._h, B, q(x0), q(lb), q(ub), q(guess), q(u), q(active), q(status), q(iters), _lib.DEVICE,
            _lib.OUT_FIRST_MOVE if first_move_only else _lib.OUT_SEQUENCE), "nnmpc_qp_solve_batch_ex")
        self._farfield_auto()

    def set_profiling(self, on=True):
        _lib.check(self._lib.nnmpc_qp_set_profiling(self._h, int(on)), "nnmpc_qp_set_profiling")

    def stats(self, reset=False):
        s = _lib.QpStats()
        _lib.check(self._lib.nnmpc_qp_get_stats(self._h, C.byref(s), int(reset)), "nnmpc_qp_get_stats")
        return {k: getattr(s, k) for k, _ in s._fields_}

    def debug_factor_solve(self, dvec, mask, rhs):
        dvec = np.ascontiguousarray(dvec, np.float32)
        mask = np.ascontiguousarray(mask, np.float32)
        rhs = np.ascontiguousarray(rhs, np.float32)
        B = dvec.shape[0]
        sol = np.empty((B, self.n), np.float32)
        _lib.check(self._lib.nnmpc_qp_debug_factor_solve(
            self._h, B, *(a.ctypes.data_as(C.c_void_p) for a in (dvec, mask, rhs, sol))),
            "nnmpc_qp_debug_factor_solve")
        return sol
```

Before: 7.457 million solves/s.

## Overlap far-field wide-check GEMM pass with next ASM round via double-buffered views

Adds a second set of active-set working buffers (a view with fewer rows) and a second counter block, so the far-field wide check GEMM for one round runs on a side stream while the next round's count/bins/lambda/update work proceeds on the main stream in the alternate view. The pass is joined by event before the wide kernel finishes, and if the new round needs more rows than the small view holds, the pass is finished first and the round is redone in the main view. This is meant to hide the wide far-field GEMM latency behind the next round's work. In exchange it costs extra device memory, more host syncs and branching, and the risk of contention between the concurrent kernels.

```diff
diff --git a/include/nnmpc.h b/include/nnmpc.h
--- a/include/nnmpc.h
+++ b/include/nnmpc.h
@@ -38,6 +38,7 @@
   int32_t seg_max;
   int32_t asm_tail_batch;
   int32_t asm_predict_iters;
+  int32_t asm_overlap;
   float ipm_tol;
   double refine_tol;
   double bound_tol;
@@ -77,6 +78,7 @@
   int64_t asm_predict_launches;
   double asm_predict_ms;
   double asm_predict_flops;
+  int64_t asm_overlapped_passes;
 } nnmpc_qp_stats;
 
 const char* nnmpc_last_error(void);
diff --git a/industrial_nnmpc_2021_amd/_lib.py b/industrial_nnmpc_2021_amd/_lib.py
--- a/industrial_nnmpc_2021_amd/_lib.py
+++ b/industrial_nnmpc_2021_amd/_lib.py
@@ -15,7 +15,7 @@
                 ("max_polish_rounds", C.c_int32), ("max_refine", C.c_int32),
                 ("max_rounds", C.c_int32), ("sub_steps", C.c_int32), ("stale_max_changes", C.c_int32),
                 ("stale_cg_limit", C.c_int32), ("method", C.c_int32), ("asm_max_active", C.c_int32),
-                ("asm_max_rounds", C.c_int32), ("asm_f32_rounds", C.c_int32), ("seg_max", C.c_int32), ("asm_tail_batch", C.c_int32), ("asm_predict_iters", C.c_int32), ("ipm_tol", C.c_float), ("refine_tol", C.c_double),
+                ("asm_max_rounds", C.c_int32), ("asm_f32_rounds", C.c_int32), ("seg_max", C.c_int32), ("asm_tail_batch", C.c_int32), ("asm_predict_iters", C.c_int32), ("asm_overlap", C.c_int32), ("ipm_tol", C.c_float), ("refine_tol", C.c_double),
                 ("bound_tol", C.c_double)]
 
 
@@ -31,7 +31,7 @@
                 ("asm_lambda64_ms", C.c_double), ("asm_lambda32_flops", C.c_double),
                 ("asm_lambda32_launches", C.c_int64), ("asm_lambda64_launches", C.c_int64), ("asm_far_passes", C.c_int64), ("asm_side_ms", C.c_double),
                 ("asm_small_passes", C.c_int64), ("asm_predict_launches", C.c_int64), ("asm_predict_ms", C.c_double),
-                ("asm_predict_flops", C.c_double)]
+                ("asm_predict_flops", C.c_double), ("asm_overlapped_passes", C.c_int64)]
 
 
 CL_MPC, CL_NN, CL_SATDLQR, CL_US = 0, 1, 2, 3
diff --git a/industrial_nnmpc_2021_amd/csrc/qp_solver.hip b/industrial_nnmpc_2021_amd/csrc/qp_solver.hip
--- a/industrial_nnmpc_2021_amd/csrc/qp_solver.hip
+++ b/industrial_nnmpc_2021_amd/csrc/qp_solver.hip
@@ -640,6 +640,13 @@
   std::vector<int> far_missing;
   double p_inf = 0.0;
   double *asm_tnorm = nullptr, *asm_tslack = nullptr;
+  struct AsmView {
+    double *lam = nullptr, *xh = nullptr, *xhw = nullptr, *tnorm = nullptr, *tslack = nullptr;
+    float *lam32 = nullptr, *xh32 = nullptr;
+    int *rowprob = nullptr, *kblk = nullptr, *counters = nullptr;
+    int rows = 0;
+  };
+  AsmView view[2];
   struct PredWin { pu32x4* Hf = nullptr; double L = 0.0; int W = 0; };
   PredWin pred[2];
   int* pred_cnt = nullptr;
@@ -656,6 +663,7 @@
   hipStream_t stream3 = nullptr, stream4 = nullptr;
   int asm_tail_budget = 50000;
   hipEvent_t ev_fork = nullptr, ev_join = nullptr, ev_join3 = nullptr, ev_join4 = nullptr;
+  hipEvent_t ev_wfork = nullptr, ev_wide = nullptr;
   int* pin_cnt = nullptr;
   int* pin_st = nullptr;
   bool profiling;
@@ -953,8 +961,6 @@
   a.ffU = a.ffVx = a.ffVl = a.ffcu = nullptr; a.ffk = nullptr; a.ffr = a.ffW = 0; a.T = h->asm_xhw; a.tnorm = h->asm_tnorm; a.tslack = h->asm_tslack;
   a.ff_skip = 0; a.ff_err = 0.0; a.ff_efar = 0.0;
   static const bool no_far = getenv("NNMPC_NO_FARFIELD") != nullptr;
-  int wide_far_rp = 0, fft_prev = 0;
-  double wide_far_ksum = 0.0;
   a.n = h->n; a.np = h->np; a.nu = h->nu; a.nseg = nprob;
   a.max_active = h->opts.asm_max_active; a.max_rounds = h->opts.asm_max_rounds;
   a.bound_tol = h->opts.bound_tol; a.stat_tol = 1e-8; a.pscale = h->pscale;
@@ -1019,11 +1025,10 @@
   hipLaunchKernelGGL(asm_init_k, dim3((segp + 3) / 4), dim3(256), 0, s, a, segp);
   const int lds_big = (a.max_active + ASM_TS) * 8;
   int* cnt = h->pin_cnt;
-  memset(cnt, 0, ASM_NCNT * sizeof(int));
+  memset(cnt, 0, 2 * ASM_NCNT * sizeof(int));
   int rounds = 0;
-  int prev_rows = 0;
-  int kprev = 0, wide_cols = 0, fused_c0 = -1;
-  HIPCHK(hipMemsetAsync(h->asm_counters, 0, ASM_NCNT * sizeof(int), s));
+  int kprev = 0;
+  HIPCHK(hipMemsetAsync(h->asm_counters, 0, 2 * ASM_NCNT * sizeof(int), s));
   if (small) {
     EvScope es(h, 4, 0.0);
     static const int g0 = getenv("NNMPC_SMALL_GRACE") ? atoi(getenv("NNMPC_SMALL_GRACE")) : ASM_SM_GRACE;
@@ -1067,7 +1072,7 @@
     const int lds_tail = (a.max_active + ASM_TS + ASM_TAIL_AREA) * 8 + ((h->n + 15) / 16) * 16 + ASM_TAIL_EXTRA;
     hipLaunchKernelGGL(asm_tail_k, dim3(nprob), dim3(256), lds_tail, s, a, h->asm_tail_budget);
     if (!defer_cnt) {
-      HIPCHK(hipMemcpyAsync(cnt, h->asm_counters, ASM_NCNT * sizeof(int), hipMemcpyDeviceToHost, s));
+      HIPCHK(hipMemcpyAsync(h->pin_cnt, h->asm_counters, 2 * ASM_NCNT * sizeof(int), hipMemcpyDeviceToHost, s));
       HIPCHK(stream_sync(s));
     }
     h->stats.asm_rounds += 1;
@@ -1080,72 +1085,141 @@
       fprintf(stderr, "asm tail only: %d problems, iterations mean %.2f max %d, active bounds mean %.1f max %d\n", nprob, (double)sum / nprob, mx, (double)sm / nprob, mm);
     }
   }
+  auto set_view = [&](AsmDev& d, int v) {
+    const nnmpc_qp::AsmView& V = h->view[v];
+    d.lam = V.lam; d.xh = V.xh; d.xhw = V.xhw; d.T = V.xhw; d.tnorm = V.tnorm; d.tslack = V.tslack; d.lam32 = V.lam32; d.xh32 = V.xh32;
+    d.rowprob = V.rowprob; d.kblk = V.kblk; d.counters = V.counters;
+  };
+  const char* env_ovl = getenv("NNMPC_OVERLAP");
+  const bool overlap_on = h->opts.asm_overlap >= 0 && h->view[1].rows > 0 && !(env_ovl && atoi(env_ovl) == 0);
+  int vW[2] = {h->np, h->np}, vrows[2] = {0, 0};
+  int pend = -1;
+  bool tail_ran[2] = {false, false};
+  struct WideStat { bool open; int view, far_rp, skip, cols; double far_ksum; } wst = {false, 0, 0, 0, 0, 0.0}, wnext = wst;
+  int fft_prev[2] = {0, 0};
+  auto account = [&](const int* c) {
+    if (!wst.open) return;
+    wst.open = false;
+    if (!h->profiling) return;
+    const double nw = c[ASM_CNT_WIDE + 1], ksum = c[ASM_CNT_WKSUM];
+    if (wst.far_rp) {
+      const int fft = h->pin_cnt[wst.view * ASM_NCNT + ASM_CNT_FFTILES];
+      const double chunks = fft - fft_prev[wst.view];
+      fft_prev[wst.view] = fft;
+      h->stats.asm_gemm_flops += 2.0 * wst.far_rp * (ksum + nw * h->ka) +
+                                 (wst.skip ? 2.0 * G64_KC * 128.0 * 128.0 * chunks : 2.0 * 128.0 * wst.far_ksum * nw);
+    } else {
+      h->stats.asm_gemm_flops += 2.0 * wst.cols * (ksum + (lazy ? nw * h->ka : 0.0));
+    }
+  };
   for (; !tail_only && rounds < 2 * a.max_rounds + 2; ++rounds) {
-    if (prev_rows) {
+    const int pv = pend;
+    bool inflight = false;
+    AsmDev ap = a;
+    int fused_c0 = -1;
+    if (pv >= 0) {
+      const int prev_rows = vrows[pv];
+      set_view(ap, pv);
+      ap.W = vW[pv]; ap.wrows = prev_rows;
+      const int c0 = (ap.W < h->np && (h->np - ap.W) % 128 == 0) ? ap.W : 0;
+      fused_c0 = ((h->np - c0) % 128 == 0 && !no_fuse) ? c0 : -1;
+      const int ntm = (prev_rows + 127) / 128, ntn = (h->np - c0) / 128;
+      const nnmpc_qp::Far* ff = nullptr;
+      if (lazy && fused_c0 > 0 && !no_far) {
+        for (const auto& f : h->far) if (f.W == c0) ff = &f;
+        if (!ff && h->far_missing.size() < 16 && std::find(h->far_missing.begin(), h->far_missing.end(), c0) == h->far_missing.end())
+          h->far_missing.push_back(c0);
+      }
+      const bool ovl = ff && overlap_on && h->view[1 - pv].rows > 0;
+      if (!ovl && wst.open && h->profiling && h->view[1 - pv].rows > 0) {
+        AsmDev af = a;
+        set_view(af, 1 - pv);
+        hipLaunchKernelGGL(asm_bins_a_k, dim3((nprob + 1023) / 1024), dim3(1024), 0, s, af);
+        hipLaunchKernelGGL(asm_bins_b_k, dim3((nprob + 1023) / 1024), dim3(1024), 0, s, af);
+        HIPCHK(hipMemcpyAsync(h->pin_cnt, h->asm_counters, 2 * ASM_NCNT * sizeof(int), hipMemcpyDeviceToHost, s));
+        HIPCHK(stream_sync(s));
+        account(h->pin_cnt + (1 - pv) * ASM_NCNT);
+      }
+      hipStream_t ps = ovl ? h->stream4 : s;
+      if (ovl) {
+        HIPCHK(hipEventRecord(h->ev_wfork, s));
+        HIPCHK(hipStreamWaitEvent(ps, h->ev_wfork, 0));
+      }
+      ap.ff_err = 0.0; ap.ff_efar = 0.0; ap.ff_skip = 0;
+      int far_rp = 0;
+      double far_ksum = 0.0;
       {
-        EvScope es(h, 5, 0.0);
-        const int c0 = (a.W < h->np && (h->np - a.W) % 128 == 0) ? a.W : 0;
-        fused_c0 = ((h->np - c0) % 128 == 0 && !no_fuse) ? c0 : -1;
-        const int ntm = (prev_rows + 127) / 128, ntn = (h->np - c0) / 128;
-        a.wrows = prev_rows;
-        const nnmpc_qp::Far* ff = nullptr;
-        if (lazy && fused_c0 > 0 && !no_far) {
-          for (const auto& f : h->far) if (f.W == c0) ff = &f;
-          if (!ff && h->far_missing.size() < 16 && std::find(h->far_missing.begin(), h->far_missing.end(), c0) == h->far_missing.end())
-            h->far_missing.push_back(c0);
+        EvScope es(h, 5, 0.0, ps);
+        if (ff) {
+          ap.ffU = ff->U; ap.ffVx = ff->Vx; ap.ffVl = ff->Vl; ap.ffcu = ff->cu; ap.ffk = ff->kt; ap.ffr = ff->rp; ap.ffW = ff->W;
+          ap.ff_err = h->p_inf * ff->efar; ap.ff_efar = ff->efar;
+          ap.ff_skip = h->nout <= c0 && h->nout < h->n;
+          far_rp = ff->rp; far_ksum = ff->ksum;
+          h->stats.asm_far_passes += 1;
+          hipLaunchKernelGGL(asm_wide_t_k, dim3(g64_grid(ntm, ff->rp / 128)), dim3(256), G64_LDS, ps, ap, ntm, ff->rp / 128);
+          if (ap.ff_skip) hipLaunchKernelGGL(asm_wide_tnorm_k, dim3((ntm * 128 + 3) / 4), dim3(256), 0, ps, ap, ntm);
+          hipLaunchKernelGGL(asm_wide_gemm_k<WIDE_FAR>, dim3(g64_grid(ntm, ntn)), dim3(256), G64_LDS, ps, ap, c0, ntm, ntn);
+        } else if (fused_c0 >= 0 && lazy) {
+          hipLaunchKernelGGL(asm_wide_gemm_k<WIDE_LAZY>, dim3(g64_grid(ntm, ntn)), dim3(256), G64_LDS, s, ap, c0, ntm, ntn);
+        } else if (fused_c0 >= 0) {
+          hipLaunchKernelGGL(asm_wide_gemm_k<WIDE_XUNC>, dim3(g64_grid(ntm, ntn)), dim3(256), G64_LDS, s, ap, c0, ntm, ntn);
+        } else {
+          gemm64(h, h->view[pv].xhw + c0, h->np, h->view[pv].lam, h->np, h->H64 + (size_t)c0 * h->np, h->np, ((prev_rows + 127) / 128) * 128,
+                 h->np - c0, h->np, nullptr, 0, h->view[pv].kblk, nullptr, true);
         }
-        a.ff_err = 0.0; a.ff_efar = 0.0; a.ff_skip = 0; wide_far_rp = 0;
-        if (ff) {
-          a.ffU = ff->U; a.ffVx = ff->Vx; a.ffVl = ff->Vl; a.ffcu = ff->cu; a.ffk = ff->kt; a.ffr = ff->rp; a.ffW = ff->W;
-          a.ff_err = h->p_inf * ff->efar; a.ff_efar = ff->efar;
-          a.ff_skip = h->nout <= c0 && h->nout < h->n;
-          wide_far_rp = ff->rp; wide_far_ksum = ff->ksum;
-          h->stats.asm_far_passes += 1;
-          hipLaunchKernelGGL(asm_wide_t_k, dim3(g64_grid(ntm, ff->rp / 128)), dim3(256), G64_LDS, s, a, ntm, ff->rp / 128);
-          if (a.ff_skip) hipLaunchKernelGGL(asm_wide_tnorm_k, dim3((ntm * 128 + 3) / 4), dim3(256), 0, s, a, ntm);
-          hipLaunchKernelGGL(asm_wide_gemm_k<WIDE_FAR>, dim3(g64_grid(ntm, ntn)), dim3(256), G64_LDS, s, a, c0, ntm, ntn);
-        } else if (fused_c0 >= 0 && lazy) {
-          hipLaunchKernelGGL(asm_wide_gemm_k<WIDE_LAZY>, dim3(g64_grid(ntm, ntn)), dim3(256), G64_LDS, s, a, c0, ntm, ntn);
-        } else if (fused_c0 >= 0) {
-          hipLaunchKernelGGL(asm_wide_gemm_k<WIDE_XUNC>, dim3(g64_grid(ntm, ntn)), dim3(256), G64_LDS, s, a, c0, ntm, ntn);
-        } else {
-          gemm64(h, h->asm_xhw + c0, h->np, h->asm_lam, h->np, h->H64 + (size_t)c0 * h->np, h->np, ((prev_rows + 127) / 128) * 128,
-                 h->np - c0, h->np, nullptr, 0, h->asm_kblk, nullptr, true);
-        }
-        wide_cols = h->np - c0;
-      }
+      }
+      wnext.view = pv; wnext.far_rp = far_rp; wnext.far_ksum = far_ksum; wnext.skip = ap.ff_skip; wnext.cols = h->np - c0; wnext.open = true;
+      if (ovl) {
+        HIPCHK(hipEventRecord(h->ev_wide, ps));
+        inflight = true;
+      } else {
+        EvScope es(h, 6, 0.0);
+        hipLaunchKernelGGL(asm_wide_k, dim3((prev_rows + 3) / 4), dim3(256), 0, s, ap, fused_c0);
+        wst = wnext;
+      }
+      pend = -1; vrows[pv] = 0;
+    }
+    auto finish_pass = [&]() -> int {
+      HIPCHK(hipStreamWaitEvent(s, h->ev_wide, 0));
       EvScope es(h, 6, 0.0);
-      hipLaunchKernelGGL(asm_wide_k, dim3((prev_rows + 3) / 4), dim3(256), 0, s, a, fused_c0);
-    }
-    a.kref = kprev;
+      hipLaunchKernelGGL(asm_wide_k, dim3((ap.wrows + 3) / 4), dim3(256), 0, s, ap, fused_c0);
+      wst = wnext;
+      inflight = false;
+      return 0;
+    };
     if (!a.pred_w) a.refine_later = 0;
     a.refine = a.refine_later && rounds >= 1;
-    {
-      EvScope es(h, 6, 0.0);
-      hipLaunchKernelGGL(asm_count_k, dim3((nprob + 3) / 4), dim3(256), 0, s, a);
-      hipLaunchKernelGGL(asm_bins_a_k, dim3((nprob + 1023) / 1024), dim3(1024), 0, s, a);
-      hipLaunchKernelGGL(asm_bins_b_k, dim3((nprob + 1023) / 1024), dim3(1024), 0, s, a);
-    }
-    HIPCHK(hipMemcpyAsync(cnt, h->asm_counters, ASM_NCNT * sizeof(int), hipMemcpyDeviceToHost, s));
-    HIPCHK(stream_sync(s));
-    const int n64 = cnt[2], n32 = cnt[ASM_CNT_ROWS32], nrun = n64 + n32;
-    if (h->profiling)
-    {
-        const double nw = cnt[ASM_CNT_WIDE + 1], ksum = cnt[ASM_CNT_WKSUM];
-        if (wide_far_rp) {
-          const double chunks = cnt[ASM_CNT_FFTILES] - fft_prev;
-          h->stats.asm_gemm_flops += 2.0 * wide_far_rp * (ksum + nw * h->ka) +
-                                     (a.ff_skip ? 2.0 * G64_KC * 128.0 * 128.0 * chunks : 2.0 * 128.0 * wide_far_ksum * nw);
-        } else {
-          h->stats.asm_gemm_flops += 2.0 * wide_cols * (ksum + (lazy ? nw * h->ka : 0.0));
-        }
-        fft_prev = cnt[ASM_CNT_FFTILES];
-    }
+    a.kref = kprev;
+    int rv = inflight ? 1 - pv : 0;
+    int n64 = 0, n32 = 0, nrun = 0;
+    for (;;) {
+      set_view(a, rv);
+      cnt = h->pin_cnt + rv * ASM_NCNT;
+      {
+        EvScope es(h, 6, 0.0);
+        hipLaunchKernelGGL(asm_count_k, dim3((nprob + 3) / 4), dim3(256), 0, s, a);
+        hipLaunchKernelGGL(asm_bins_a_k, dim3((nprob + 1023) / 1024), dim3(1024), 0, s, a);
+        hipLaunchKernelGGL(asm_bins_b_k, dim3((nprob + 1023) / 1024), dim3(1024), 0, s, a);
+      }
+      HIPCHK(hipMemcpyAsync(h->pin_cnt, h->asm_counters, 2 * ASM_NCNT * sizeof(int), hipMemcpyDeviceToHost, s));
+      HIPCHK(stream_sync(s));
+      n64 = cnt[2]; n32 = cnt[ASM_CNT_ROWS32]; nrun = n64 + n32;
+      account(cnt);
+      if (inflight && nrun > h->view[rv].rows) {
+        const int rcf = finish_pass();
+        if (rcf) return rcf;
+        rv = 0;
+        a.work = nullptr;
+        continue;
+      }
+      break;
+    }
+    a.work = h->asm_work;
     kprev = cnt[3];
     {
       static const bool trace = getenv("NNMPC_TRACE_ROUNDS") != nullptr;
       if (trace) {
-        fprintf(stderr, "asm round %d: fp64 %d f32 %d last-active %d wide-checked %d big %d big32 %d | fp64 classes", rounds, n64, n32, cnt[3],
+        fprintf(stderr, "asm round %d%s: fp64 %d f32 %d last-active %d wide-checked %d big %d big32 %d | fp64 classes", rounds, inflight ? " (beside the pass)" : "", n64, n32, cnt[3],
                 cnt[ASM_CNT_WIDE + 1], cnt[1], cnt[ASM_CNT_BIG32] + cnt[ASM_CNT_BIG32B]);
         for (int b = 0; b < ASM_NBIN; ++b) fprintf(stderr, " %d", cnt[4 + b]);
         fprintf(stderr, " | f32 classes");
@@ -1153,41 +1227,59 @@
         fprintf(stderr, "\n");
       }
     }
-    if (nrun == 0) break;
+    if (nrun == 0) {
+      if (!inflight) break;
+      const int rcf = finish_pass();
+      if (rcf) return rcf;
+      --rounds;
+      continue;
+    }
+    const nnmpc_qp::AsmView& V = h->view[rv];
     static const int tail_max = getenv("NNMPC_TAIL_MAX") ? atoi(getenv("NNMPC_TAIL_MAX")) : 256;
     if (nrun <= std::min(h->asm_pool, tail_max) && (rounds >= (a.pred_w ? 2 : 6) || small)) {
-      EvScope es(h, 4, 0.0);
-      hipLaunchKernelGGL(asm_taillist_k, dim3((nprob + 255) / 256), dim3(256), 0, s, a);
-      if (Wx < h->np) {
-        gemm64(h, h->asm_xunc + Wx, h->np, h->x0_64, h->ka, h->Kunc64 + (size_t)Wx * h->ka, h->ka, ((nrun + 127) / 128) * 128, h->np - Wx, h->ka,
-               nullptr, 0, nullptr, h->asm_counters + ASM_CNT_TAIL, false, h->asm_biglist);
-        a.Wx = h->np;
-      }
-      const int lds_tail = (a.max_active + ASM_TS + ASM_TAIL_AREA) * 8 + ((h->n + 15) / 16) * 16 + ASM_TAIL_EXTRA;
-      hipLaunchKernelGGL(asm_tail_k, dim3(nrun), dim3(256), lds_tail, s, a, h->asm_tail_budget);
-      HIPCHK(hipMemcpyAsync(cnt, h->asm_counters, ASM_NCNT * sizeof(int), hipMemcpyDeviceToHost, s));
-      HIPCHK(stream_sync(s));
+      static const bool trace = getenv("NNMPC_TRACE_ROUNDS") != nullptr;
       {
-        static const bool trace = getenv("NNMPC_TRACE_ROUNDS") != nullptr;
-        if (trace) {
-          std::vector<int> rd(nprob), bl(nrun);
-          hipMemcpy(rd.data(), h->asm_rounds, nprob * sizeof(int), hipMemcpyDeviceToHost);
-          hipMemcpy(bl.data(), h->asm_biglist, nrun * sizeof(int), hipMemcpyDeviceToHost);
-          long sum = 0; int mx = 0;
-          for (int i = 0; i < nrun; ++i) { const int r = rd[bl[i]] - rounds; sum += r; mx = std::max(mx, r); }
-          fprintf(stderr, "asm tail after round %d: %d problems, iterations mean %.1f max %d\n", rounds, nrun, (double)sum / nrun, mx);
+        EvScope es(h, 4, 0.0);
+        if (tail_ran[rv]) HIPCHK(hipMemsetAsync(V.counters + ASM_CNT_TAIL, 0, sizeof(int), s));
+        hipLaunchKernelGGL(asm_taillist_k, dim3((nprob + 255) / 256), dim3(256), 0, s, a);
+        if (Wx < h->np) {
+          gemm64(h, h->asm_xunc + Wx, h->np, h->x0_64, h->ka, h->Kunc64 + (size_t)Wx * h->ka, h->ka, ((nrun + 127) / 128) * 128, h->np - Wx, h->ka,
+                 nullptr, 0, nullptr, V.counters + ASM_CNT_TAIL, false, h->asm_biglist);
+          a.Wx = h->np;
+        }
+        const int lds_tail = (a.max_active + ASM_TS + ASM_TAIL_AREA) * 8 + ((h->n + 15) / 16) * 16 + ASM_TAIL_EXTRA;
+        hipLaunchKernelGGL(asm_tail_k, dim3(nrun), dim3(256), lds_tail, s, a, h->asm_tail_budget);
+        tail_ran[rv] = true;
+      }
+      if (!inflight || trace) {
+        HIPCHK(hipMemcpyAsync(h->pin_cnt, h->asm_counters, 2 * ASM_NCNT * sizeof(int), hipMemcpyDeviceToHost, s));
+        HIPCHK(stream_sync(s));
+      }
+      if (trace) {
+        std::vector<int> rd(nprob), bl(nrun);
+        hipMemcpy(rd.data(), h->asm_rounds, nprob * sizeof(int), hipMemcpyDeviceToHost);
+        hipMemcpy(bl.data(), h->asm_biglist, nrun * sizeof(int), hipMemcpyDeviceToHost);
+        long sum = 0; int mx = 0;
+        for (int i = 0; i < nrun; ++i) { const int r = rd[bl[i]] - rounds; sum += r; mx = std::max(mx, r); }
+        fprintf(stderr, "asm tail after round %d: %d problems, iterations mean %.1f max %d\n", rounds, nrun, (double)sum / nrun, mx);
 #ifdef ASM_TAIL_PROF
-          unsigned long long tp[8];
-          hipMemcpyFromSymbol(tp, HIP_SYMBOL(asm_tail_prof), sizeof tp);
-          fprintf(stderr, "  tail clock sums (all workgroups): count/factor/solve %llu, substitutions %llu, x loop %llu, tests %llu, exchange %llu; iterations on the dense factor %llu, on a fresh factorisation %llu\n",
-                  tp[0], tp[1], tp[2], tp[3], tp[4], tp[5], tp[6]);
-          memset(tp, 0, sizeof tp); hipMemcpyToSymbol(HIP_SYMBOL(asm_tail_prof), tp, sizeof tp);
+        unsigned long long tp[8];
+        hipMemcpyFromSymbol(tp, HIP_SYMBOL(asm_tail_prof), sizeof tp);
+        fprintf(stderr, "  tail clock sums (all workgroups): count/factor/solve %llu, substitutions %llu, x loop %llu, tests %llu, exchange %llu; iterations on the dense factor %llu, on a fresh factorisation %llu\n",
+                tp[0], tp[1], tp[2], tp[3], tp[4], tp[5], tp[6]);
+        memset(tp, 0, sizeof tp); hipMemcpyToSymbol(HIP_SYMBOL(asm_tail_prof), tp, sizeof tp);
 #endif
-        }
       }
       h->stats.asm_rounds += 1;
-      rounds = 0;
-      break;
+      if (!inflight) {
+        rounds = 0;
+        break;
+      }
+      a.Wx = Wx;
+      const int rcf = finish_pass();
+      if (rcf) return rcf;
+      h->stats.asm_overlapped_passes += 1;
+      continue;
     }
     h->stats.asm_rounds += 1;
     a.W = std::min(h->np, ((cnt[3] + 1 + h->nu + 127) / 128) * 128);
@@ -1207,12 +1299,13 @@
       int nbig = cnt[1] + cnt[ASM_CNT_BIG32] + nreg2_wg + nreg32b_wg + nwg64 + nwg32b + nwg64r, nreg_wg = 0, nreg32_wg = 0;
       for (int b = 0; b < ASM_NREG; ++b) { nreg_wg += (cnt[4 + b] + 3) / 4; nreg32_wg += (cnt[ASM_CNT_F32 + b] + 3) / 4; }
       const bool side4 = cnt[1] > 0, side2 = nwg64 + nwg32 + nwg32b + nwg64r > 0 || (cnt[ASM_CNT_BIG32] && !a.use_wg), side3 = nreg2_wg + nreg32b_wg > 0;
+      hipStream_t st4 = inflight ? h->stream2 : h->stream4;
       if (nbig) {
         HIPCHK(hipEventRecord(h->ev_fork, s));
         if (side4) {
-          HIPCHK(hipStreamWaitEvent(h->stream4, h->ev_fork, 0));
-          { EvScope e9(h, 9, 0.0, h->stream4); hipLaunchKernelGGL((asm_lambda_tile_k<1>), dim3(std::min(cnt[1], h->asm_pool)), dim3(256), lds_big, h->stream4, a, 0); }
-          HIPCHK(hipEventRecord(h->ev_join4, h->stream4));
+          HIPCHK(hipStreamWaitEvent(st4, h->ev_fork, 0));
+          { EvScope e9(h, 9, 0.0, st4); hipLaunchKernelGGL((asm_lambda_tile_k<1>), dim3(std::min(cnt[1], h->asm_pool)), dim3(256), lds_big, st4, a, 0); }
+          HIPCHK(hipEventRecord(h->ev_join4, st4));
         }
         if (side2) {
           HIPCHK(hipStreamWaitEvent(h->stream2, h->ev_fork, 0));
@@ -1242,40 +1335,50 @@
     {
       EvScope es(h, 5, 2.0 * a.W * (double)cnt[0]);
       if (n64)
-        gemm64(h, h->asm_xh, h->np, h->asm_lam, h->np, h->H64, h->np, ((n64 + 127) / 128) * 128, a.W, h->np, nullptr, 0,
-               h->asm_kblk, nullptr, true);
+        gemm64(h, V.xh, h->np, V.lam, h->np, h->H64, h->np, ((n64 + 127) / 128) * 128, a.W, h->np, nullptr, 0,
+               V.kblk, nullptr, true);
       if (n32 && a.W % 128 == 0)
         hipLaunchKernelGGL((gemm_nt_f32_kdyn_k<128>), dim3(a.W / 128, (n32 + 127) / 128), dim3(256), TileCfg<128>::LDS_FLOATS * 4, s,
-                           h->asm_xh32, (size_t)h->np, h->asm_lam32, (size_t)h->np, h->H32, (size_t)h->np, h->np, h->asm_kblk + a.nkblk / 2, 2);
+                           V.xh32, (size_t)h->np, V.lam32, (size_t)h->np, h->H32, (size_t)h->np, h->np, V.kblk + a.nkblk / 2, 2);
       else if (n32)
         hipLaunchKernelGGL((gemm_nt_f32_kdyn_k<64>), dim3(a.W / 64, (n32 + 63) / 64), dim3(256), TileCfg<64>::LDS_FLOATS * 4, s,
-                           h->asm_xh32, (size_t)h->np, h->asm_lam32, (size_t)h->np, h->H32, (size_t)h->np, h->np, h->asm_kblk + a.nkblk / 2, 1);
+                           V.xh32, (size_t)h->np, V.lam32, (size_t)h->np, h->H32, (size_t)h->np, h->np, V.kblk + a.nkblk / 2, 1);
     }
     {
       EvScope es(h, 6, 0.0);
-      if (n64) HIPCHK(hipMemsetAsync(h->asm_rowprob, 0xFF, (size_t)((n64 + 127) / 128) * 128 * sizeof(int), s));
+      if (n64) HIPCHK(hipMemsetAsync(V.rowprob, 0xFF, (size_t)((n64 + 127) / 128) * 128 * sizeof(int), s));
       hipLaunchKernelGGL(asm_update_k, dim3((nprob + 3) / 4), dim3(256), 0, s, a);
     }
-    prev_rows = a.W < h->n ? n64 : 0;
+    vW[rv] = a.W;
+    vrows[rv] = a.W < h->n ? n64 : 0;
+    pend = vrows[rv] ? rv : -1;
+    if (inflight) {
+      const int rcf = finish_pass();
+      if (rcf) return rcf;
+      h->stats.asm_overlapped_passes += 1;
+    }
   }
   if (rounds >= 2 * a.max_rounds + 2) {
-    HIPCHK(hipMemcpyAsync(cnt, h->asm_counters, ASM_NCNT * sizeof(int), hipMemcpyDeviceToHost, s));
+    HIPCHK(hipMemcpyAsync(h->pin_cnt, h->asm_counters, 2 * ASM_NCNT * sizeof(int), hipMemcpyDeviceToHost, s));
     HIPCHK(stream_sync(s));
   }
   if (h->gemm_error) { h->gemm_error = false; return NNMPC_EINVAL; }
-  if (!defer_cnt) h->stats.asm_full_checks += cnt[ASM_CNT_DONE];
-  if (defer_cnt || cnt[ASM_CNT_DONE] > 0) {
+  set_view(a, 0);
+  cnt = h->pin_cnt;
+  auto ndone = [&]() { return h->pin_cnt[ASM_CNT_DONE] + h->pin_cnt[ASM_NCNT + ASM_CNT_DONE]; };
+  if (!defer_cnt) h->stats.asm_full_checks += ndone();
+  if (defer_cnt || ndone() > 0) {
     gemm64(h, h->q64_all, h->np, h->x0_64, h->ka, h->tq64, h->ka, segp, h->np, h->ka, h->asm_state, ASM_DONE);
     gemm64(h, h->asm_xh, h->np, h->asm_x, h->np, h->P64, h->np, segp, h->np, h->np, h->asm_state, ASM_DONE);
   }
   hipLaunchKernelGGL(asm_certify_k, dim3(nprob), dim3(256), 0, s, a, h->pscale);
   int* st = h->pin_st;
   HIPCHK(hipMemcpyAsync(st, h->asm_status, (size_t)nprob * sizeof(int), hipMemcpyDeviceToHost, s));
-  int* pin_its = h->pin_cnt + ASM_NCNT;
+  int* pin_its = h->pin_cnt + 2 * ASM_NCNT;
   if (h->profiling && pred_flops_per_it > 0.0) HIPCHK(hipMemcpyAsync(pin_its, h->pred_cnt + 1, 4, hipMemcpyDeviceToHost, s));
-  if (defer_cnt) HIPCHK(hipMemcpyAsync(cnt, h->asm_counters, ASM_NCNT * sizeof(int), hipMemcpyDeviceToHost, s));
+  if (defer_cnt) HIPCHK(hipMemcpyAsync(h->pin_cnt, h->asm_counters, 2 * ASM_NCNT * sizeof(int), hipMemcpyDeviceToHost, s));
   HIPCHK(stream_sync(s));
-  if (defer_cnt) h->stats.asm_full_checks += cnt[ASM_CNT_DONE];
+  if (defer_cnt) h->stats.asm_full_checks += ndone();
   if (h->profiling && pred_flops_per_it > 0.0) h->stats.asm_predict_flops += pred_flops_per_it * (double)*pin_its;
   HIPCHK(hipGetLastError());
   std::vector<int> fb;
@@ -1384,7 +1487,8 @@
   if (hipStreamCreate(&h->stream2) != hipSuccess || hipStreamCreate(&h->stream3) != hipSuccess || hipStreamCreate(&h->stream4) != hipSuccess ||
       hipEventCreateWithFlags(&h->ev_fork, hipEventDisableTiming) != hipSuccess ||
       hipEventCreateWithFlags(&h->ev_join3, hipEventDisableTiming) != hipSuccess || hipEventCreateWithFlags(&h->ev_join4, hipEventDisableTiming) != hipSuccess ||
-      hipEventCreateWithFlags(&h->ev_join, hipEventDisableTiming) != hipSuccess) {
+      hipEventCreateWithFlags(&h->ev_join, hipEventDisableTiming) != hipSuccess ||
+      hipEventCreateWithFlags(&h->ev_wfork, hipEventDisableTiming) != hipSuccess || hipEventCreateWithFlags(&h->ev_wide, hipEventDisableTiming) != hipSuccess) {
     set_error("hipStreamCreate / hipEventCreate failed"); nnmpc_qp_destroy(h); return NNMPC_EHIP;
   }
   {
@@ -1437,7 +1541,7 @@
   A_(h->q64_all, G * np); A_(h->uunc_all, G * np);
   A_(h->lb_d, G * nu); A_(h->ub_d, G * nu);
   A_(h->in_stage, G * n_aug);
-  if (!rc && hipHostMalloc((void**)&h->pin_cnt, (ASM_NCNT + 4) * sizeof(int)) != hipSuccess) { set_error("nnmpc_qp_create: hipHostMalloc failed"); rc = NNMPC_EHIP; }
+  if (!rc && hipHostMalloc((void**)&h->pin_cnt, (2 * ASM_NCNT + 4) * sizeof(int)) != hipSuccess) { set_error("nnmpc_qp_create: hipHostMalloc failed"); rc = NNMPC_EHIP; }
   if (!rc && hipHostMalloc((void**)&h->pin_st, G * sizeof(int)) != hipSuccess) { set_error("nnmpc_qp_create: hipHostMalloc failed"); rc = NNMPC_EHIP; }
   A_(d.lb64, (size_t)S * nu); A_(d.ub64, (size_t)S * nu);
   A_(d.slot_prob, S); A_(d.age, S); A_(d.next_prob, 1);
@@ -1446,10 +1550,27 @@
   A_(h->asm_xunc, G * np); A_(h->asm_x, G * np); A_(h->asm_lam, G * np); A_(h->asm_xh, G * np);
   A_(h->asm_xhw, (G + 256) * np); A_(h->asm_rowprob, G + 256); A_(h->asm_wflag, G); A_(h->asm_wmark, G);
   A_(h->asm_tnorm, G + 128 * (ASM_NKG + 1)); A_(h->asm_tslack, G + 128 * (ASM_NKG + 1));
-  A_(h->asm_st, G * n); A_(h->asm_state, G); A_(h->asm_rounds, G); A_(h->asm_counters, ASM_NCNT);
+  A_(h->asm_st, G * n); A_(h->asm_state, G); A_(h->asm_rounds, G); A_(h->asm_counters, 2 * ASM_NCNT);
   A_(h->asm_biglist, G); A_(h->asm_status, G); A_(h->asm_binlist, (size_t)(ASM_NLIST + 4) * G);
   A_(h->asm_idxg, G * o.asm_max_active); A_(h->asm_mg, G); A_(h->asm_row, G); A_(h->asm_lrank, G); A_(h->asm_ctot, ((G + 1023) / 1024) * ASM_NSCAN); A_(h->asm_prec, G); A_(h->asm_redo, G); A_(h->asm_rowk, G); A_(h->asm_lam32, G * np); A_(h->asm_xh32, G * np); A_(h->asm_alpha, G); A_(h->asm_ninf, G); A_(h->asm_hi, G); A_(h->asm_kblk, 2 * (G / 64 + 2)); A_(h->asm_work, 3 * G);
   A_(h->asm_scratch, (size_t)h->asm_pool * ((size_t)(o.asm_max_active / 16) * (o.asm_max_active / 16 + 1) / 2 * ASM_TS));
+  {
+    nnmpc_qp::AsmView& v0 = h->view[0];
+    v0.lam = h->asm_lam; v0.xh = h->asm_xh; v0.xhw = h->asm_xhw; v0.tnorm = h->asm_tnorm; v0.tslack = h->asm_tslack;
+    v0.lam32 = h->asm_lam32; v0.xh32 = h->asm_xh32; v0.rowprob = h->asm_rowprob; v0.kblk = h->asm_kblk; v0.counters = h->asm_counters;
+    v0.rows = (int)G;
+    long long R = std::max<long long>(1024, ((long long)G / 32 + 127) / 128 * 128);
+    if (const char* e = getenv("NNMPC_OVERLAP_ROWS")) R = std::max(0, atoi(e) / 128 * 128);
+    R = std::min<long long>(R, (long long)G);
+    if (o.asm_overlap >= 0 && R > 0) {
+      nnmpc_qp::AsmView& v1 = h->view[1];
+      const size_t Rr = (size_t)R;
+      A_(v1.lam, Rr * np); A_(v1.xh, Rr * np); A_(v1.xhw, (Rr + 256) * np); A_(v1.lam32, Rr * np); A_(v1.xh32, Rr * np);
+      A_(v1.tnorm, Rr + 128 * (ASM_NKG + 1)); A_(v1.tslack, Rr + 128 * (ASM_NKG + 1)); A_(v1.rowprob, Rr + 256); A_(v1.kblk, 2 * (G / 64 + 2));
+      v1.counters = h->asm_counters + ASM_NCNT;
+      if (!rc) v1.rows = (int)R;
+    }
+  }
 #undef A_
   if (rc) { nnmpc_qp_destroy(h); return rc; }
   d.n = n; d.np = np; d.nu = nu; d.slots = S; d.words = h->words;
@@ -1527,6 +1648,8 @@
   if (h->ev_join) hipEventDestroy(h->ev_join);
   if (h->ev_join3) hipEventDestroy(h->ev_join3);
   if (h->ev_join4) hipEventDestroy(h->ev_join4);
+  if (h->ev_wfork) hipEventDestroy(h->ev_wfork);
+  if (h->ev_wide) hipEventDestroy(h->ev_wide);
   if (h->pin_cnt) hipHostFree(h->pin_cnt);
   if (h->pin_st) hipHostFree(h->pin_st);
   if (h->stream2) hipStreamDestroy(h->stream2);
diff --git a/industrial_nnmpc_2021_amd/qp.py b/industrial_nnmpc_2021_amd/qp.py
--- a/industrial_nnmpc_2021_amd/qp.py
+++ b/industrial_nnmpc_2021_amd/qp.py
@@ -45,7 +45,7 @@
 
     def __init__(self, P, tq, nu, *, Kunc="auto", method="auto", farfield="auto", max_batch=1024, nb=0, ipm_tol=0.0,
                  max_rounds=0, max_ipm_iters=0, max_polish_rounds=0, max_refine=0, sub_steps=0, stale_max_changes=0, stale_cg_limit=0, asm_max_active=0,
-                 asm_max_rounds=0, asm_f32_rounds=0, seg_max=0, asm_tail_batch=0, asm_predict_iters=0):
+                 asm_max_rounds=0, asm_f32_rounds=0, seg_max=0, asm_tail_batch=0, asm_predict_iters=0, asm_overlap=0):
         lib = _lib.load()
         P = np.ascontiguousarray(P, dtype=np.float64)
         tq = np.ascontiguousarray(tq, dtype=np.float64)
@@ -72,7 +72,7 @@
                            max_rounds=max_rounds, sub_steps=sub_steps, stale_max_changes=stale_max_changes,
                            stale_cg_limit=stale_cg_limit, method=meth, asm_max_active=asm_max_active,
                            asm_max_rounds=asm_max_rounds, asm_f32_rounds=asm_f32_rounds, seg_max=seg_max, asm_tail_batch=asm_tail_batch,
-                           asm_predict_iters=asm_predict_iters,
+                           asm_predict_iters=asm_predict_iters, asm_overlap=asm_overlap,
                            ipm_tol=ipm_tol, refine_tol=0.0, bound_tol=0.0)
         self._h = C.c_void_p()
         kp = Kunc.ctypes.data_as(C.c_void_p) if Kunc is not None else None
```

Result: faster. 7.650 million solves/s (median of 6 runs) (+2.6%).
